# shanjiayao/PTT

Hardware: AMD Instinct MI355X
Metric: tracklet frames/sec (hot path: PointNet++ SA stack + Point-Track-Transformer blocks) (higher is better)
Workload: dtype f32

## Files before the change

include/ptt_hip.h:

```cpp
#ifndef PTT_HIP_H
#define PTT_HIP_H

#include <stddef.h>
#include <stdint.h>

#ifdef __cplusplus
extern "C" {
#endif

#define PTT_ABI_VERSION 31

enum {
    PTT_OK = 0,
    PTT_EINVAL = -1,
    PTT_EUNSUPPORTED = -2,
    PTT_ELAUNCH = -3,
    PTT_EWORKSPACE = -4
};

typedef void* ptt_stream_t;

int ptt_version(void);
const char* ptt_error_name(int code);
const char* ptt_last_error_string(void);

int ptt_fps_f32(const float* xyz, int B, int N, int npoint, int32_t* idx_out,
                ptt_stream_t stream);
int ptt_fps_ws_f32(const float* xyz, int B, int N, int npoint, int32_t* idx_out, float* workspace,
                   size_t workspace_elems, ptt_stream_t stream);

int ptt_ffps_f32(const float* xyz, const float* feat, int64_t feat_sb, int64_t feat_sc, int64_t feat_sn,
                 int B, int N, int C, int npoint, int32_t* idx_out, ptt_stream_t stream);

int ptt_gather_f32(const float* feat, const int32_t* idx, int B, int C, int N, int M,
                   float* out, ptt_stream_t stream);
int ptt_gather_grad_f32(const float* grad_out, const int32_t* idx, int B, int C, int N,
                        int M, float* grad_feat, ptt_stream_t stream);

int ptt_select_centres_f32(const float* xyz, const int32_t* idx, int B, int N, int M, float* new_xyz,
                           int64_t* idx64_out, ptt_stream_t stream);

int ptt_ball_query_f32(const float* new_xyz, const float* xyz, int B, int M, int N,
                       float radius, int nsample, int32_t* idx_out, ptt_stream_t stream);

int ptt_centres_ball_query_f32(const float* xyz, const int32_t* sel, int B, int N, int M, float radius, int nsample,
                               float* new_xyz, int64_t* idx64_out, int32_t* idx_out, ptt_stream_t stream);

int ptt_group_f32(const float* feat, const int32_t* idx, int B, int C, int N, int M,
                  int ns, float* out, ptt_stream_t stream);
int ptt_group_grad_f32(const float* grad_out, const int32_t* idx, int B, int C, int N,
                       int M, int ns, float* grad_feat, ptt_stream_t stream);

size_t ptt_scatter_add_det_workspace(int B, int N, int E);
int ptt_scatter_add_det_f32(const float* src, const int32_t* idx, int B, int C, int N, int E, float* out,
                            void* workspace, size_t workspace_bytes, ptt_stream_t stream);

int ptt_knn_f32(const float* xyz, int B, int N, int k, int32_t* idx_out,
                ptt_stream_t stream);
int ptt_knn_rel_f32(const float* xyz, int B, int N, int k, int32_t* idx_out, float* rel_out,
                    ptt_stream_t stream);

size_t ptt_packed_weight_elems(int Cout, int K);
int ptt_pack_weight_f32(const float* W, int Cout, int K, float* packed,
                        ptt_stream_t stream);
int ptt_pack_weight_rot_f32(const float* W, int Cout, int K, int rot, float* packed,
                            ptt_stream_t stream);

int ptt_linear_f32(const float* X, int rows, int K, int ldx, const float* Wpacked, int Cout,
                   const float* scale, const float* shift, int relu, const float* residual,
                   int ldr, float* out, int ldo, ptt_stream_t stream);

#define PTT_SA_MAX_LAYERS 4

typedef struct ptt_sa_layer {
    const float* Wpacked;
    const float* scale;
    const float* shift;
    int Cin;
    int Cout;
    int relu;
} ptt_sa_layer;

int ptt_rows_mlp_f32(const float* X, int rows, int K, int ldx, const ptt_sa_layer* layers, int n_layers,
                     const float* residual, int ldr, float* out, int ldo, ptt_stream_t stream);

size_t ptt_ball_query_grid_workspace(int B, int N);
int ptt_ball_query_grid_f32(const float* new_xyz, const float* xyz, int B, int M, int N, float radius, int nsample,
                            int32_t* idx_out, void* workspace, size_t workspace_bytes, ptt_stream_t stream);
int ptt_centres_ball_query_grid_f32(const float* xyz, const int32_t* sel, int B, int N, int M, float radius, int nsample,
                                    float* new_xyz, int64_t* idx64_out, int32_t* idx_out, void* workspace, size_t workspace_bytes,
                                    ptt_stream_t stream);
int ptt_fps_ball_knn_f32(const float* xyz, int B, int N, int M, float radius, int nsample, int k, int32_t* inds,
                         int64_t* inds64, float* new_xyz, int32_t* idx, int32_t* knn, float* rel, ptt_stream_t stream);
#define PTT_POINT_JOBS_MAX 4
typedef struct ptt_point_job {
    const float* xyz; const int32_t* centre_sel; const int32_t* point_sel;
    float* new_xyz; int64_t* idx64_out; int32_t* idx_out; float* rel_out;
    int32_t kind, sel_ld, B, Nraw, Npts, M, nsample;
    float radius;
} ptt_point_job;
int ptt_point_jobs_f32(const ptt_point_job* jobs, int n_jobs, ptt_stream_t stream);

#define PTT_ROW_JOBS_MAX 4
typedef struct ptt_row_job {
    const float* X; const float* X2;
    const float* Xmax;
    const float* Wpacked; const float* scale; const float* shift;
    const float* res; const float* res2;
    float* out; float* out2; float* raw;
    const float* rel; const float* w1;
    const float* qkv; const int32_t* knn; const float* pos;
    int32_t rows, K, K1, ldx, ldx2, Cout;
    int32_t act, res_split, ldr, ldr2, out_split, out_col0, ldo, ldo2, ldraw;
    int32_t prologue, epilogue, ldq, q_off, k_off, v_off, ldp, N;
    float sm_scale;
    int32_t col_tiles;
    const int32_t* idx; const float* xyz; const float* centres; const float* wx;
    float radius;
    int32_t ns, M, normalize_xyz, pro_relu;
} ptt_row_job;
int ptt_row_jobs_f32(const ptt_row_job* jobs, int n_jobs, ptt_stream_t stream);

typedef struct ptt_sa_desc {
    const float* xyz;
    const float* new_xyz;
    const int32_t* idx;
    const float* feat;
    int64_t feat_sb, feat_sc, feat_sn;
    float* out;
    int64_t out_sb, out_sc, out_sm;
    int B, N, M, nsample, C;
    float radius;
    int use_xyz;
    int normalize_xyz;
    int n_layers;
    ptt_sa_layer layers[PTT_SA_MAX_LAYERS];
    const float* l0_point_term;
    const float* l0_xyz_weight;
    int l0_channels;
    int l0_relu;
    void* compact_ws;
    size_t compact_ws_bytes;
} ptt_sa_desc;

int ptt_sa_fused_fwd_f32(const ptt_sa_desc* d, ptt_stream_t stream);
size_t ptt_sa_compact_workspace(int B, int M);

typedef struct ptt_xcorr_desc {
    const float* cos_t;
    const float* P;
    const float* w_sim;
    const float* scale0;
    const float* shift0;
    float* out;
    int64_t out_sb, out_sc, out_sn;
    float* sim_out;
    int B, Ns, Nt, C0;
    int n_layers;
    ptt_sa_layer layers[PTT_SA_MAX_LAYERS];
    int32_t split; int64_t out_sh;
    const float* search_feat; const float* templ_feat;
    int64_t s_sb, s_sn, t_sb, t_sn;
    int C; float eps;
} ptt_xcorr_desc;

int ptt_xcorr_fused_fwd_f32(const ptt_xcorr_desc* d, ptt_stream_t stream);

int ptt_cosine_map_f32(const float* search_feat, int64_t s_sb, int64_t s_sn, int64_t s_sc, const float* templ_feat,
                       int64_t t_sb, int64_t t_sn, int64_t t_sc, int B, int Ns, int Nt, int C, float eps,
                       float* cos_t, ptt_stream_t stream);

typedef struct ptt_attn_desc {
    const float* xyz;
    const float* rel;
    const int32_t* knn;
    const float* qkv;
    const float* Wd1p;
    const float* Wd2p;
    const float* bd2;
    const float* Wg1p;
    const float* bg1;
    const float* Wg2p;
    const float* bg2;
    float* res;
    float* attn;
    int B, N, k, D;
    const int32_t* order;
    int heads;
} ptt_attn_desc;

int ptt_pt_attn_pair_f32(const ptt_attn_desc* d, ptt_stream_t stream);
int ptt_spatial_order_f32(const float* xyz, int B, int N, int32_t* order, ptt_stream_t stream);

typedef struct ptt_crop_job {
    const float* points;
    int64_t ld;
    double lo1[3], hi1[3];
    double trans[3];
    double rot[9];
    double lo2[3], hi2[3];
    float* out;
    int32_t* count;
    int32_t n_points;
    int32_t capacity;
    uint8_t* label_out;
    double ltrans[3];
    double lrot[9];
    double llo[3], lhi[3];
    int32_t append;
    int32_t reserved;
} ptt_crop_job;

int ptt_crop_compact_f32(const ptt_crop_job* jobs_device, int n_jobs, ptt_stream_t stream);
#define PTT_CROP_JOBS_BY_VALUE_MAX 8
int ptt_crop_compact_host_f32(const ptt_crop_job* jobs_host, int n_jobs, ptt_stream_t stream);

#define PTT_SCAN_CROP_CHUNK 1024
size_t ptt_crop_scan_workspace(int n_jobs, int max_points);
int ptt_crop_scan_f32(const ptt_crop_job* jobs_device, int n_jobs, int max_points, void* ws, size_t ws_bytes, ptt_stream_t stream);

#define PTT_MAX_SEGMENTS 4
typedef struct ptt_regularize_job {
    const float* seg[PTT_MAX_SEGMENTS];
    const int32_t* seg_count[PTT_MAX_SEGMENTS];
    int32_t seg_capacity[PTT_MAX_SEGMENTS];
// ... 301 lines not shown
```

ptt_amd/_lib.py:

```python
import ctypes
import os
import re
from ctypes import Structure, c_char_p, c_double, c_float, c_int, c_int32, c_int64, c_longlong, c_size_t, c_uint32, c_void_p

from .build import HEADER as HEADER_PATH, LIB as LIB_PATH


def _strip_comments(text):
    return re.sub(r"/\*.*?\*/|//[^\n]*", " ", text, flags=re.S)


def parse_defines(text):
    return {n: int(v) for n, v in re.findall(r"^[ \t]*#[ \t]*define[ \t]+(PTT_\w+)[ \t]+(-?\d+)[ \t]*$", _strip_comments(text), re.M)}


CTYPES = {"int": c_int, "int32_t": c_int32, "uint32_t": c_uint32, "int64_t": c_int64, "long long": c_longlong, "size_t": c_size_t,
          "float": c_float, "double": c_double, "ptt_stream_t": c_void_p}


def _ctype(decl, name, is_return=False):
    words = decl.replace("*", " * ").split()
    if not is_return and len(words) > 1 and words[-1] != "*":
        words.pop()
    if "*" in words:
# ... 67 lines not shown
                ("reg", c_float * 4), ("index", c_uint32), ("epoch", c_uint32), ("capacity", c_int32), ("reserved", c_int32)]


class TrainBatchDesc(Structure):
    _fields_ = [("search_points", c_void_p), ("template_points", c_void_p), ("cls_label", c_void_p), ("reg_label", c_void_p),
                ("src_out", c_void_p), ("idx_search_out", c_void_p), ("idx_template_out", c_void_p), ("info", c_void_p), ("totals", c_void_p),
                ("B", c_int32), ("n_cand", c_int32), ("search_size", c_int32), ("template_size", c_int32), ("min_points", c_int32),
                ("seed_lo", c_uint32), ("seed_hi", c_uint32), ("reserved", c_int32)]


class BnTrainTail(Structure):
    _fields_ = [("gamma", c_void_p), ("beta", c_void_p), ("act_a", c_void_p), ("act_b", c_void_p),
                ("running_mean", c_void_p), ("running_var", c_void_p), ("num_batches_tracked", c_void_p), ("momentum", c_float)]


class BnBwdInput(Structure):
    _fields_ = [("g", c_void_p), ("ldg", c_int), ("arg", c_void_p), ("ns", c_int), ("z", c_void_p), ("ldz", c_int),
                ("k1", c_void_p), ("c0", c_void_p), ("c1", c_void_p), ("mean", c_void_p), ("act_a", c_void_p), ("act_b", c_void_p),
                ("dz_out", c_void_p), ("ldd", c_int)]


class PackJob(Structure):
    _fields_ = [("W", c_void_p), ("out_offset", c_int64), ("stride_out", c_int64), ("stride_k", c_int64),
                ("Cout", c_int32), ("K", c_int32)]


class RowJob(Structure):
    _fields_ = [("X", c_void_p), ("X2", c_void_p), ("Xmax", c_void_p), ("Wpacked", c_void_p), ("scale", c_void_p), ("shift", c_void_p),
                ("res", c_void_p), ("res2", c_void_p), ("out", c_void_p), ("out2", c_void_p), ("raw", c_void_p),
                ("rel", c_void_p), ("w1", c_void_p), ("qkv", c_void_p), ("knn", c_void_p), ("pos", c_void_p),
                ("rows", c_int32), ("K", c_int32), ("K1", c_int32), ("ldx", c_int32), ("ldx2", c_int32), ("Cout", c_int32),
                ("act", c_int32), ("res_split", c_int32), ("ldr", c_int32), ("ldr2", c_int32), ("out_split", c_int32),
                ("out_col0", c_int32), ("ldo", c_int32), ("ldo2", c_int32), ("ldraw", c_int32),
                ("prologue", c_int32), ("epilogue", c_int32), ("ldq", c_int32), ("q_off", c_int32), ("k_off", c_int32),
                ("v_off", c_int32), ("ldp", c_int32), ("N", c_int32), ("sm_scale", c_float), ("col_tiles", c_int32),
                ("idx", c_void_p), ("xyz", c_void_p), ("centres", c_void_p), ("wx", c_void_p), ("radius", c_float),
                ("ns", c_int32), ("M", c_int32), ("normalize_xyz", c_int32), ("pro_relu", c_int32)]


class PointJob(Structure):
    _fields_ = [("xyz", c_void_p), ("centre_sel", c_void_p), ("point_sel", c_void_p), ("new_xyz", c_void_p), ("idx64_out", c_void_p),
                ("idx_out", c_void_p), ("rel_out", c_void_p), ("kind", c_int32), ("sel_ld", c_int32), ("B", c_int32),
                ("Nraw", c_int32), ("Npts", c_int32), ("M", c_int32), ("nsample", c_int32), ("radius", c_float)]


class TrackLossDesc(Structure):
    _fields_ = [("seed_cls", c_void_p), ("cls_label", c_void_p), ("search_inds", c_void_p), ("votes", c_void_p), ("reg_label", c_void_p),
                ("box_data", c_void_p), ("centres", c_void_p), ("pos_weight_seed", c_void_p), ("pos_weight_box", c_void_p),
                ("B", c_int32), ("N", c_int32), ("Ns", c_int32), ("M", c_int32), ("ld_reg", c_int32),
                ("w_seed_cls", c_float), ("w_seed_reg", c_float), ("w_box_cls", c_float), ("w_box_reg", c_float)]


class AdamTensor(Structure):
    _fields_ = [("param", c_void_p), ("grad", c_void_p), ("exp_avg", c_void_p), ("exp_avg_sq", c_void_p), ("n", c_int64)]


class GradJob(Structure):
    _fields_ = [("partial", c_void_p), ("nchunks", c_int32), ("reserved", c_int32)]


class GradSegment(Structure):
    _fields_ = [("dst", c_int64), ("n", c_int32), ("cols", c_int32), ("ld", c_int32), ("job0", c_int32), ("njobs", c_int32), ("out", c_int32),
                ("vec", c_int32), ("reserved", c_int32)]


class AdamHyper(Structure):
    _fields_ = [("beta1", c_float), ("beta2", c_float), ("one_minus_beta1", c_float), ("one_minus_beta2", c_float), ("eps", c_float), ("step_size", c_float), ("bias2_sqrt", c_float),
                ("weight_decay", c_float), ("max_norm", c_float), ("write_clipped", c_int32)]


class SaLayer(Structure):
    _fields_ = [("Wpacked", c_void_p), ("scale", c_void_p), ("shift", c_void_p),
                ("Cin", c_int), ("Cout", c_int), ("relu", c_int)]


class SaDesc(Structure):
    _fields_ = [("xyz", c_void_p), ("new_xyz", c_void_p), ("idx", c_void_p), ("feat", c_void_p),
                ("feat_sb", c_int64), ("feat_sc", c_int64), ("feat_sn", c_int64),
                ("out", c_void_p), ("out_sb", c_int64), ("out_sc", c_int64), ("out_sm", c_int64),
                ("B", c_int), ("N", c_int), ("M", c_int), ("nsample", c_int), ("C", c_int),
                ("radius", c_float), ("use_xyz", c_int), ("normalize_xyz", c_int), ("n_layers", c_int),
                ("layers", SaLayer * PTT_SA_MAX_LAYERS),
                ("l0_point_term", c_void_p), ("l0_xyz_weight", c_void_p), ("l0_channels", c_int), ("l0_relu", c_int),
                ("compact_ws", c_void_p), ("compact_ws_bytes", c_size_t)]


class XcorrDesc(Structure):
    _fields_ = [("cos_t", c_void_p), ("P", c_void_p), ("w_sim", c_void_p), ("scale0", c_void_p), ("shift0", c_void_p),
                ("out", c_void_p), ("out_sb", c_int64), ("out_sc", c_int64), ("out_sn", c_int64),
                ("sim_out", c_void_p),
                ("B", c_int), ("Ns", c_int), ("Nt", c_int), ("C0", c_int),
                ("n_layers", c_int), ("layers", SaLayer * PTT_SA_MAX_LAYERS),
                ("split", c_int32), ("out_sh", c_int64), ("search_feat", c_void_p), ("templ_feat", c_void_p),
                ("s_sb", c_int64), ("s_sn", c_int64), ("t_sb", c_int64), ("t_sn", c_int64), ("C", c_int), ("eps", c_float)]


class AttnDesc(Structure):
    _fields_ = [("xyz", c_void_p), ("rel", c_void_p), ("knn", c_void_p), ("qkv", c_void_p),
                ("Wd1p", c_void_p), ("Wd2p", c_void_p), ("bd2", c_void_p),
                ("Wg1p", c_void_p), ("bg1", c_void_p), ("Wg2p", c_void_p), ("bg2", c_void_p),
                ("res", c_void_p), ("attn", c_void_p),
                ("B", c_int), ("N", c_int), ("k", c_int), ("D", c_int), ("order", c_void_p), ("heads", c_int)]


_lib = None


def lib():
    global _lib
    if _lib is None:
        if not os.path.exists(LIB_PATH):
            raise RuntimeError(
                "ptt_amd: %s is missing — build it with `python -m ptt_amd.build` "
                "(hipcc --offload-arch=gfx950); there is no CPU fallback" % LIB_PATH)
        import torch
        try:
            loaded = ctypes.CDLL(LIB_PATH)
        except OSError as e:
            raise RuntimeError("ptt_amd: cannot load %s: %s" % (LIB_PATH, e))
        for name, (restype, argtypes) in PROTOTYPES.items():
            fn = getattr(loaded, name)
            fn.restype, fn.argtypes = restype, argtypes
        if loaded.ptt_version() != ABI_VERSION:
            raise RuntimeError("ptt_amd: %s has ABI version %d, this package expects %d — rebuild it with "
                               "`python -m ptt_amd.build`" % (LIB_PATH, loaded.ptt_version(), ABI_VERSION))
        _lib = loaded
    return _lib


def check(rc, what):
    if rc != 0:
        l = lib()
        raise RuntimeError("%s failed: %s (%s)" % (what, l.ptt_error_name(rc).decode(),
                                                   l.ptt_last_error_string().decode()))
```

ptt_amd/csrc/common.h:

```cpp
#pragma once
#include <hip/hip_runtime.h>
#include <stdint.h>
#include <stdio.h>
#include "../../include/ptt_hip.h"

namespace ptt {

char* last_error_buf();
int fail(int code, const char* fmt, ...);
int check_launch(const char* what);

static inline hipStream_t as_stream(ptt_stream_t s) { return reinterpret_cast<hipStream_t>(s); }

struct DevSwitches {
    int linear_rt = 1, linear_ct = 1;
    int linear_small = 1;
    int sa_gather1 = 0;
    int sa_stagger = 0;
    int sa_wave = 1;
    int sa_rt = 2;
    int sa_lds = 1;
    int sa_stream = 1;
    int sa_chunk = 2;
    int pair_stagger = 0;
    int pair_lds_pad = 0;
    int sa_lds_chunk = 2;
    int fps_plain = 0;
    int ball_cpw = 0;
    int fps_t = 0;
    int ffps_stream = 0;
    int group_grad_global = 0;
    long long* stamps = nullptr;
};
const DevSwitches& dev_switches();

int set_lds_limit(const void* fn, int bytes);

bool wgrad_stream_ok(int R, int Cout, int Cin, int ldz, int ldx);
int wgrad_stream_rows(int R);
int launch_wgrad_stream(const float* dZ, int ldz, const float* X, int ldx, int R, int Cout, int Cin, int rows, float* partial,
                        const float* x_scale, const float* x_shift, hipStream_t s);

template <int CTRL, int ROW_MASK>
__device__ __forceinline__ int dpp_i32(int v) {
    return __builtin_amdgcn_update_dpp(v, v, CTRL, ROW_MASK, 0xF, false);
}
template <int CTRL, int ROW_MASK>
__device__ __forceinline__ float dpp_f32(float v) {
    return __builtin_bit_cast(float, dpp_i32<CTRL, ROW_MASK>(__builtin_bit_cast(int, v)));
}

__device__ __forceinline__ float wave_max_f32(float v) {
    v = fmaxf(v, dpp_f32<0xB1, 0xF>(v));
    v = fmaxf(v, dpp_f32<0x4E, 0xF>(v));
    v = fmaxf(v, dpp_f32<0x141, 0xF>(v));
    v = fmaxf(v, dpp_f32<0x140, 0xF>(v));
    v = fmaxf(v, dpp_f32<0x142, 0xA>(v));
    v = fmaxf(v, dpp_f32<0x143, 0xC>(v));
    return __builtin_bit_cast(float, __builtin_amdgcn_readlane(__builtin_bit_cast(int, v), 63));
}
__device__ __forceinline__ float wave_max_f32_fused(float v) {
    asm volatile(
        "s_nop 1\n\tv_max_f32_dpp %0, %0, %0 quad_perm:[1,0,3,2] row_mask:0xf bank_mask:0xf\n\t"
        "s_nop 1\n\tv_max_f32_dpp %0, %0, %0 quad_perm:[2,3,0,1] row_mask:0xf bank_mask:0xf\n\t"
        "s_nop 1\n\tv_max_f32_dpp %0, %0, %0 row_half_mirror row_mask:0xf bank_mask:0xf\n\t"
        "s_nop 1\n\tv_max_f32_dpp %0, %0, %0 row_mirror row_mask:0xf bank_mask:0xf\n\t"
        "s_nop 1\n\tv_max_f32_dpp %0, %0, %0 row_bcast:15 row_mask:0xa bank_mask:0xf\n\t"
        "s_nop 1\n\tv_max_f32_dpp %0, %0, %0 row_bcast:31 row_mask:0xc bank_mask:0xf\n\t"
        "s_nop 1"
        : "+v"(v));
    return __builtin_bit_cast(float, __builtin_amdgcn_readlane(__builtin_bit_cast(int, v), 63));
}

__device__ __forceinline__ float wave_min_f32(float v) {
    v = fminf(v, dpp_f32<0xB1, 0xF>(v));
    v = fminf(v, dpp_f32<0x4E, 0xF>(v));
    v = fminf(v, dpp_f32<0x141, 0xF>(v));
    v = fminf(v, dpp_f32<0x140, 0xF>(v));
    v = fminf(v, dpp_f32<0x142, 0xA>(v));
    v = fminf(v, dpp_f32<0x143, 0xC>(v));
    return __builtin_bit_cast(float, __builtin_amdgcn_readlane(__builtin_bit_cast(int, v), 63));
}
__device__ __forceinline__ int wave_min_i32(int v) {
    v = min(v, dpp_i32<0xB1, 0xF>(v));
    v = min(v, dpp_i32<0x4E, 0xF>(v));
    v = min(v, dpp_i32<0x141, 0xF>(v));
    v = min(v, dpp_i32<0x140, 0xF>(v));
    v = min(v, dpp_i32<0x142, 0xA>(v));
    v = min(v, dpp_i32<0x143, 0xC>(v));
    return __builtin_amdgcn_readlane(v, 63);
}

}
```

ptt_amd/csrc/errors.hip:

```cpp
#include <stdarg.h>
#include <stdlib.h>
#include <string.h>
#include <map>
#include <mutex>
#include <utility>
#include "common.h"

namespace ptt {

static thread_local char g_err[512] = "";

char* last_error_buf() { return g_err; }

int fail(int code, const char* fmt, ...) {
    va_list ap;
    va_start(ap, fmt);
    vsnprintf(g_err, sizeof(g_err), fmt, ap);
    va_end(ap);
    return code;
}

int check_launch(const char* what) {
    const hipError_t e = hipGetLastError();
    if (e == hipSuccess) return PTT_OK;
    return fail(PTT_ELAUNCH, "%s: %s", what, hipGetErrorString(e));
}

#ifdef PTT_DEV
static DevSwitches read_switches() {
    DevSwitches d;
    if (const char* e = getenv("PTT_LINEAR_TILE")) { d.linear_rt = (e[0] == '2') ? 2 : 1; d.linear_ct = (e[0] && e[1] == '2') ? 2 : 1; }
    if (getenv("PTT_SA_GATHER1")) d.sa_gather1 = 1;
    if (const char* e = getenv("PTT_SA_STAGGER")) d.sa_stagger = atoi(e);
    if (const char* e = getenv("PTT_SA_WAVE")) d.sa_wave = atoi(e) != 0;
    if (const char* e = getenv("PTT_SA_RT")) d.sa_rt = (atoi(e) == 1) ? 1 : 2;
    if (const char* e = getenv("PTT_SA_STREAM")) d.sa_stream = atoi(e) != 0;
    if (const char* e = getenv("PTT_SA_LDS")) d.sa_lds = atoi(e) != 0;
    if (const char* e = getenv("PTT_SA_CHUNK")) d.sa_chunk = atoi(e);
    if (const char* e = getenv("PTT_PAIR_STAGGER")) d.pair_stagger = atoi(e);
    if (const char* e = getenv("PTT_PAIR_LDS_PAD")) d.pair_lds_pad = atoi(e);
    if (const char* e = getenv("PTT_LINEAR_SMALL")) d.linear_small = atoi(e);
    if (const char* e = getenv("PTT_BALL_CPW")) d.ball_cpw = atoi(e);
    if (const char* e = getenv("PTT_FPS_PLAIN")) d.fps_plain = atoi(e);
    if (const char* e = getenv("PTT_SA_LDS_CHUNK")) d.sa_lds_chunk = atoi(e);
    if (const char* e = getenv("PTT_FPS_T")) d.fps_t = atoi(e);
    if (const char* e = getenv("PTT_FFPS_STREAM")) d.ffps_stream = atoi(e);
    if (getenv("PTT_GROUP_GRAD_GLOBAL")) d.group_grad_global = 1;
    if (const char* e = getenv("PTT_DEBUG_STAMPS")) d.stamps = reinterpret_cast<long long*>(strtoull(e, nullptr, 16));
    return d;
}
const DevSwitches& dev_switches() {
    static thread_local DevSwitches d;
    d = read_switches();
    return d;
}
#else
const DevSwitches& dev_switches() {
    static const DevSwitches d;
    return d;
}
#endif

int set_lds_limit(const void* fn, int bytes) {
    if (bytes <= 48 * 1024) return PTT_OK;
    static std::map<std::pair<const void*, int>, int> table;
    static std::mutex mu;
    int dev = 0;
    if (hipGetDevice(&dev) != hipSuccess) return check_launch("hipGetDevice");
    std::lock_guard<std::mutex> g(mu);
    const auto key = std::make_pair(fn, dev);
    const auto it = table.find(key);
    if (it != table.end() && it->second >= bytes) return PTT_OK;
    if (hipFuncSetAttribute(fn, hipFuncAttributeMaxDynamicSharedMemorySize, bytes) != hipSuccess)
        return check_launch("hipFuncSetAttribute(MaxDynamicSharedMemorySize)");
    table[key] = bytes;
    return PTT_OK;
}

}

extern "C" int ptt_version(void) { return PTT_ABI_VERSION; }

extern "C" const char* ptt_last_error_string(void) { return ptt::last_error_buf(); }

extern "C" const char* ptt_error_name(int code) {
    switch (code) {
        case PTT_OK: return "PTT_OK";
        case PTT_EINVAL: return "PTT_EINVAL";
        case PTT_EUNSUPPORTED: return "PTT_EUNSUPPORTED";
        case PTT_ELAUNCH: return "PTT_ELAUNCH";
        case PTT_EWORKSPACE: return "PTT_EWORKSPACE";
        default: return "PTT_E?";
    }
}
```

ptt_amd/csrc/mfma_ops.hip:

```cpp
#include <math.h>
#include <stdlib.h>
#include <string.h>
#include "common.h"
#include "mfma_common.h"

#ifndef PTT_PAIR_PF
#define PTT_PAIR_PF 1
#endif
#ifndef PTT_GATHER_BATCH
#define PTT_GATHER_BATCH 16
#endif
#ifndef PTT_SA_WAVES
#define PTT_SA_WAVES 2
#endif

namespace ptt {

#ifdef PTT_DEV
#define PTT_STAMP(i) do { if (p.dbg && threadIdx.x == 0 && blockIdx.x < 4096) p.dbg[blockIdx.x * 8 + (i)] = __builtin_readcyclecounter(); } while (0)
#else
#define PTT_STAMP(i) do { } while (0)
#endif

__device__ __forceinline__ void stagger_second_slot(int first_wave_blocks, int quanta) {
// ... 340 lines not shown
                if (gr >= p.rows) continue;
                float y = acc[rt][u][r] * sc + sh;
                if (p.relu) y = fmaxf(y, 0.f);
                if (p.residual) y += p.residual[(size_t)gr * p.ldr + col];
                p.out[(size_t)gr * p.ldo + col] = y;
            }
    }
}

constexpr int LS_PD = 8;
__global__ __launch_bounds__(512, 1) void linear_small_kernel(LinearParams p) {
    extern __shared__ __attribute__((aligned(16))) float smem[];
    const int t = threadIdx.x, lane = t & 63, half = lane >> 5;
    const int w = __builtin_amdgcn_readfirstlane(t >> 6), ks = w >> 2, cw = w & 3;
    const int row0 = blockIdx.x * 32;
    const int ct = blockIdx.y * 4 + cw;
    const bool has_ct = ct < p.NT;
    const int hb = ((p.nkb + 1) / 2 + LS_PD - 1) / LS_PD * LS_PD;
    const int ldk = 2 * hb * 8 + 4;
    float* Xs = smem;
    float* Rs = smem + 32 * ldk;
    {
        const int qpr = 2 * hb * 2;
        for (int e = t; e < 32 * qpr; e += 512) {
            const int r = e / qpr, c = (e - r * qpr) << 2;
            f32x4 v = {0.f, 0.f, 0.f, 0.f};
            if (row0 + r < p.rows && c < p.K) v = *reinterpret_cast<const f32x4*>(p.X + (size_t)(row0 + r) * p.ldx + c);
            *reinterpret_cast<f32x4*>(Xs + r * ldk + c) = v;
        }
    }
    const __amdgpu_buffer_rsrc_t wr = weight_rsrc(p.Wp);
    const int wvoff = ((has_ct ? ct : 0) * 64 + lane) * 16;
    const int wkstep = p.NT * 1024;
    const int kb0 = ks * hb, last = p.nkb - 1;
    f32x4 b[LS_PD];
#pragma unroll
    for (int i = 0; i < LS_PD; ++i) b[i] = weight_load(wr, wvoff, min(kb0 + i, last) * wkstep);
    f32x16 acc;
#pragma unroll
    for (int r = 0; r < 16; ++r) acc[r] = 0.f;
    __syncthreads();
    const float* arow = Xs + (lane & 31) * ldk + 4 * half + kb0 * 8;
    for (int k = 0; k < hb; k += LS_PD) {
#pragma unroll
        for (int i = 0; i < LS_PD; ++i) {
            const f32x4 a = *reinterpret_cast<const f32x4*>(arow + (k + i) * 8);
#pragma unroll
            for (int j = 0; j < 4; ++j) acc = __builtin_amdgcn_mfma_f32_32x32x2f32(a[j], b[i][j], acc, 0, 0, 0);
            b[i] = weight_load(wr, wvoff, min(kb0 + k + i + LS_PD, last) * wkstep);
        }
    }
    if (ks == 1) {
#pragma unroll
        for (int r = 0; r < 16; ++r) Rs[(cw * 16 + r) * 64 + lane] = acc[r];
    }
    __syncthreads();
    if (ks == 1 || !has_ct) return;
    const int col = ct * 32 + (lane & 31);
    if (col >= p.Cout) return;
    const float sc = p.scale ? p.scale[col] : 1.f;
    const float sh = p.shift ? p.shift[col] : 0.f;
#pragma unroll
    for (int r = 0; r < 16; ++r) {
        const int gr = row0 + tile_row(r, half);
        if (gr >= p.rows) continue;
        float y = (acc[r] + Rs[(cw * 16 + r) * 64 + lane]) * sc + sh;
        if (p.relu) y = fmaxf(y, 0.f);
        if (p.residual) y += p.residual[(size_t)gr * p.ldr + col];
        p.out[(size_t)gr * p.ldo + col] = y;
    }
}

struct SaLayerDev { const float* Wp; const float* scale; const float* shift; int Cin, Cout, relu, nkb, NT; };
struct SaParams {
    const float* xyz; const float* new_xyz; const int32_t* idx; const float* feat; float* out;
    long long fsb, fsc, fsn, osb, osc, osm;
    int B, N, M, C, use_xyz, normalize, n_layers, ldk, K0, first_wave, stagger, vec_gather;
    int tiles, chunk;
    int hoist, l0_relu;
    const float* wx;
    float radius;
    long long* dbg;
    int32_t* cws;
    SaLayerDev L[PTT_SA_MAX_LAYERS];
};

struct RowsMlpParams {
    const float* X; const float* residual; float* out;
    int rows, K0, ldx, ldr, ldo, n_layers, ldk, vec_in;
    SaLayerDev L[PTT_SA_MAX_LAYERS];
};

__global__ __launch_bounds__(256, 2) void rows_mlp_kernel(RowsMlpParams p) {
    extern __shared__ __attribute__((aligned(16))) float smem[];
    float* Xs = smem;
    const int t = threadIdx.x, lane = t & 63, w = t >> 6, half = lane >> 5;
    const int row0 = blockIdx.x * 32;
    f32x4 pw[3];
    float psh[3];
    auto prefetch = [&](const SaLayerDev& L) {
        const f32x4* bp = reinterpret_cast<const f32x4*>(L.Wp) + (size_t)w * 64 + lane;
#pragma unroll
        for (int u = 0; u < 3; ++u) {
            psh[u] = 0.f;
            if (w + 4 * u < L.NT) {
                pw[u] = bp[(size_t)u * 4 * 64];
                const int col = (w + 4 * u) * 32 + (lane & 31);
                if (L.shift && !L.scale && col < L.Cout) psh[u] = L.shift[col];
            }
        }
    };
    prefetch(p.L[0]);
    {
        const int Kpad = p.L[0].nkb * 8;
        if (p.vec_in) {
            const int nq = Kpad >> 2;
            for (int e = t; e < 32 * nq; e += 256) {
                const int r = e / nq, c4 = (e - r * nq) * 4;
                f32x4 v = {0.f, 0.f, 0.f, 0.f};
                if (row0 + r < p.rows && c4 < p.K0) v = *reinterpret_cast<const f32x4*>(p.X + (size_t)(row0 + r) * p.ldx + c4);
                *reinterpret_cast<f32x4*>(Xs + r * p.ldk + c4) = v;
            }
        } else {
            for (int e = t; e < 32 * Kpad; e += 256) {
                const int r = e / Kpad, c = e - r * Kpad;
                Xs[r * p.ldk + c] = (row0 + r < p.rows && c < p.K0) ? p.X[(size_t)(row0 + r) * p.ldx + c] : 0.f;
            }
        }
    }
    lds_barrier();
    for (int l = 0; l < p.n_layers; ++l) {
        const SaLayerDev& L = p.L[l];
        const bool last = l == p.n_layers - 1, affine = L.scale != nullptr;
        f32x16 acc[1][3];
#pragma unroll
        for (int u = 0; u < 3; ++u)
#pragma unroll
            for (int r = 0; r < 16; ++r) acc[0][u][r] = psh[u];
        int nvalid = 0;
#pragma unroll
        for (int u = 0; u < 3; ++u)
            if (w + 4 * u < L.NT) nvalid = u + 1;
        if (nvalid) gemm_tiles<1, 3, 0>(Xs, p.ldk, L.nkb, reinterpret_cast<const f32x4*>(L.Wp), L.NT, w, nvalid, lane, acc, pw);
        if (!last) { prefetch(p.L[l + 1]); lds_barrier(); }
#pragma unroll
        for (int u = 0; u < 3; ++u) {
            if (u >= nvalid) break;
            const int col = (w + 4 * u) * 32 + (lane & 31);
            float sc = 1.f, sh = 0.f;
            if (affine && col < L.Cout) { sc = L.scale[col]; sh = L.shift ? L.shift[col] : 0.f; }
#pragma unroll
            for (int r = 0; r < 16; ++r) {
                float y = affine ? acc[0][u][r] * sc + sh : acc[0][u][r];
                if (L.relu) y = fmaxf(y, 0.f);
                const int row = tile_row(r, half);
                if (!last) {
                    Xs[row * p.ldk + col] = (col < L.Cout) ? y : 0.f;
                } else if (col < L.Cout && row0 + row < p.rows) {
                    if (p.residual) y += p.residual[(size_t)(row0 + row) * p.ldr + col];
                    p.out[(size_t)(row0 + row) * p.ldo + col] = y;
                }
            }
        }
        if (!last) lds_barrier();
    }
}
// ... 172 lines not shown
                if (L.relu) m = fmaxf(m, 0.f);
                const int c = centre0 + rt;
                if (half == 0 && rt < ncentres) {
                    const int b = c / p.M, mm = c - b * p.M;
                    p.out[b * p.osb + col * p.osc + mm * p.osm] = m;
                }
            } else {
                float m0 = y[0], m1 = y[8];
#pragma unroll
                for (int r = 1; r < 8; ++r) { m0 = fmaxf(m0, y[r]); m1 = fmaxf(m1, y[8 + r]); }
                m0 = max_halves(m0);
                m1 = max_halves(m1);
                if (L.relu) { m0 = fmaxf(m0, 0.f); m1 = fmaxf(m1, 0.f); }
                if (half == 0) {
                    const int ca = rt * 2, cb = rt * 2 + 1;
                    if (ca < ncentres) {
                        const int c = centre0 + ca; const int b = c / p.M, mm = c - b * p.M;
                        p.out[b * p.osb + col * p.osc + mm * p.osm] = m0;
                    }
                    if (cb < ncentres) {
                        const int c = centre0 + cb; const int b = c / p.M, mm = c - b * p.M;
                        p.out[b * p.osb + col * p.osc + mm * p.osm] = m1;
                    }
                }
            }
        }
    }
    if (!last) lds_barrier();
}

template <int NS, int RT>
__global__ __launch_bounds__(256, PTT_SA_WAVES) void sa_fused_kernel(SaParams p) {
    extern __shared__ __attribute__((aligned(16))) float smem[];
    float* Xs = smem;
    constexpr int CPW = 32 * RT / NS;
    const int t = threadIdx.x, lane = t & 63, w = t >> 6;
    const int total_centres = p.B * p.M;
    const int centre0 = logical_block() * CPW;
    const int ncentres = min(CPW, total_centres - centre0);
    stagger_second_slot(p.first_wave, p.stagger);
    PTT_STAMP(0);

    SaPre pre;
    pre.w[0] = pre.w[1] = f32x4{0.f, 0.f, 0.f, 0.f};
    prefetch_first_block(p.L[0].Wp, p.L[0].scale, p.L[0].shift, p.L[0].NT, w, lane, pre);

    sa_gather_rows<NS, 8 * RT>(p, Xs, w * 8 * RT, centre0, lane);
    lds_barrier();

    PTT_STAMP(1);
    for (int l = 0; l < p.n_layers; ++l) {
        const SaLayerDev& L = p.L[l];
        const bool last = (l == p.n_layers - 1);
        const int ctw = (L.NT + 3) >> 2;
        const SaLayerDev* Ln = last ? nullptr : &p.L[l + 1];
        if (ctw <= 1) sa_layer<NS, 1, RT>(p, L, last, Xs, lane, w, centre0, ncentres, pre, Ln);
        else sa_layer<NS, 2, RT>(p, L, last, Xs, lane, w, centre0, ncentres, pre, Ln);
        PTT_STAMP(2 + l);
    }
}

constexpr int SAS_LDK = 132;
constexpr int SAS_TILE = 64 * SAS_LDK;

__device__ __forceinline__ f32x4 sas_pair_load(const float* meta, __amdgpu_buffer_rsrc_t rf, int w, int i, int sub, int q,
                                               f32x4& m) {
    m = *reinterpret_cast<const f32x4*>(meta + (w * 16 + 2 * i + sub) * 4);
    return weight_load(rf, __builtin_bit_cast(int, m[0]) + q * 16, 0);
}
__device__ __forceinline__ void sas_pair_store(float* X, int w, int i, int sub, int q, f32x4 v, const f32x4& m, const f32x4& wx0,
                                               const f32x4& wx1, const f32x4& wx2, float floor) {
#pragma unroll
    for (int j = 0; j < 4; ++j) {
        float y = __builtin_fmaf(wx0[j], m[1], v[j]);
        y = __builtin_fmaf(wx1[j], m[2], y);
        y = __builtin_fmaf(wx2[j], m[3], y);
        v[j] = fmaxf(y, floor);
    }
    *reinterpret_cast<f32x4*>(X + (16 * w + 2 * i + sub) * SAS_LDK + q * 4) = v;
}

struct SasCentre {
    int c, b, m;
    __device__ __forceinline__ void advance(int k, int M) {
        c += k; m += k;
        while (m >= M) { m -= M; ++b; }
    }
};

__device__ __forceinline__ float sas_pool(const f32x16& a, float sh, int relu) {
    float mx = a[0];
#pragma unroll
    for (int r = 1; r < 16; ++r) mx = fmaxf(mx, a[r]);
    mx = max_halves(mx) + sh;
    return relu ? fmaxf(mx, 0.f) : mx;
}

#ifndef PTT_SAS_INTERLEAVE
#define PTT_SAS_INTERLEAVE 0
#endif
#ifndef PTT_SAS_EXP
#define PTT_SAS_EXP 0
#endif
template <int NS>
__global__ __launch_bounds__(256, 2) void sa_stream_kernel(SaParams p) {
    static_assert(NS == 32, "one centre per 32-row tile");
    extern __shared__ __attribute__((aligned(16))) float smem[];
    float* const P = smem;
    float* const Q = smem + SAS_TILE;
    float* const meta = smem + 2 * SAS_TILE;
    const int t = threadIdx.x, lane = t & 63, half = lane >> 5, sub = half, q = lane & 31;
    const int w = __builtin_amdgcn_readfirstlane(t >> 6);
    const int tile0 = logical_block() * p.chunk;
    const int ntiles = min(p.chunk, p.tiles - tile0);
    if (ntiles <= 0) return;
    stagger_second_slot(p.first_wave, p.stagger);
    const SaLayerDev& L1 = p.L[0];
    const SaLayerDev& L2 = p.L[1];
    const __amdgpu_buffer_rsrc_t rf = weight_rsrc(p.feat);
    const __amdgpu_buffer_rsrc_t wr1 = weight_rsrc(L1.Wp), wr2 = weight_rsrc(L2.Wp);
    const int wvoff = (w * 64 + lane) * 16;
    constexpr int WK1 = 4 * 1024, WK2 = 8 * 1024;
    const f32x4 wx0 = *reinterpret_cast<const f32x4*>(p.wx + q * 4);
    const f32x4 wx1 = *reinterpret_cast<const f32x4*>(p.wx + 128 + q * 4);
    const f32x4 wx2 = *reinterpret_cast<const f32x4*>(p.wx + 256 + q * 4);
    const int col = lane & 31;
    const float sh1 = L1.shift ? L1.shift[w * 32 + col] : 0.f;
    const float sh2a = L2.shift ? L2.shift[w * 32 + col] : 0.f;
    const float sh2b = L2.shift ? L2.shift[(w + 4) * 32 + col] : 0.f;
    f32x16 sh1v;
#pragma unroll
    for (int r = 0; r < 16; ++r) sh1v[r] = sh1;
    const int total_centres = p.B * p.M;
    const float floor0 = p.l0_relu ? 0.f : -__builtin_inff();
    const float rdiv = p.normalize ? p.radius : 1.0f;
    const int M = p.M, N = p.N;
    const int osb = (int)p.osb, osm = (int)p.osm;
    const int ocol0 = (w * 32 + col) * (int)p.osc, ocol1 = ((w + 4) * 32 + col) * (int)p.osc;

    SasCentre own, first;
    {
        const int c0 = tile0 * 2;
        first.c = c0; first.b = c0 / M; first.m = c0 - first.b * M;
        own = first;
        own.advance(w >> 1, M);
    }
    auto meta_index = [&](const SasCentre& ce) -> int {
        const int c = ce.c < total_centres ? ce.c : total_centres - 1;
        return p.idx[(size_t)c * 32 + 16 * (w & 1) + (lane & 15)];
    };
    struct MetaXyz { float x, y, z, cx, cy, cz; int flat; };
    auto meta_fetch = [&](const SasCentre& ce, int n) -> MetaXyz {
        const bool in = ce.c < total_centres;
        const int c = in ? ce.c : total_centres - 1;
        const int b = in ? ce.b : p.B - 1;
        MetaXyz r;
        r.flat = b * N + n;
        r.x = p.xyz[(size_t)r.flat * 3 + 0]; r.y = p.xyz[(size_t)r.flat * 3 + 1]; r.z = p.xyz[(size_t)r.flat * 3 + 2];
        r.cx = p.new_xyz[(size_t)c * 3 + 0]; r.cy = p.new_xyz[(size_t)c * 3 + 1]; r.cz = p.new_xyz[(size_t)c * 3 + 2];
        return r;
    };
    auto meta_store = [&](const MetaXyz& r) {
        const float dx = (r.x - r.cx) / rdiv, dy = (r.y - r.cy) / rdiv, dz = (r.z - r.cz) / rdiv;
        const int off = r.flat * (128 * (int)sizeof(float));
        *reinterpret_cast<f32x4*>(meta + (w * 16 + (lane & 15)) * 4) = f32x4{__builtin_bit_cast(float, off), dx, dy, dz};
    };

    f32x4 pre1[2] = {weight_load(wr1, wvoff, 0), weight_load(wr1, wvoff, WK1)};
    {
        const int n = meta_index(own);
        meta_store(meta_fetch(own, n));
#pragma unroll
        for (int i = 0; i < 8; ++i) {
            f32x4 m;
            const f32x4 v = sas_pair_load(meta, rf, w, i, sub, q, m);
            sas_pair_store(P, w, i, sub, q, v, m, wx0, wx1, wx2, floor0);
        }
    }

    f32x16 acc[2][2];
#pragma unroll
    for (int rt = 0; rt < 2; ++rt)
#pragma unroll
        for (int u = 0; u < 2; ++u)
#pragma unroll
            for (int r = 0; r < 16; ++r) acc[rt][u][r] = 0.f;
    float pv[2][2] = {{0.f, 0.f}, {0.f, 0.f}};
    SasCentre prev = first;
    const f32x16 zero16 = {0.f, 0.f, 0.f, 0.f, 0.f, 0.f, 0.f, 0.f, 0.f, 0.f, 0.f, 0.f, 0.f, 0.f, 0.f, 0.f};

    auto store_pooled = [&](const SasCentre& f) {
        SasCentre c1 = f;
        c1.advance(1, M);
        if (half == 0) {
            if (f.c < total_centres) {
                float* o = p.out + (f.b * osb + f.m * osm);
                o[ocol0] = pv[0][0]; o[ocol1] = pv[0][1];
            }
            if (c1.c < total_centres) {
                float* o = p.out + (c1.b * osb + c1.m * osm);
                o[ocol0] = pv[1][0]; o[ocol1] = pv[1][1];
            }
        }
    };

    for (int it = 0; it < ntiles; ++it) {
        const bool more = it + 1 < ntiles;
        SasCentre own_next = own;
        if (more) own_next.advance(2, M);
        if (!(PTT_SAS_EXP & 1)) lds_barrier();
        const int nn = meta_index(own_next);
        MetaXyz mx;

        f32x16 acc1[2];
        {
            const float* arow = P + (lane & 31) * SAS_LDK + 4 * half;
            f32x4 a0[2], a1[2], bc[2], bn[2];
#define SAS_A1(A, KB)                                                                           \
            {                                                                                   \
                A[0] = *reinterpret_cast<const f32x4*>(arow + (KB) * 8);                        \
                A[1] = *reinterpret_cast<const f32x4*>(arow + 32 * SAS_LDK + (KB) * 8);         \
            }
            bc[0] = pre1[0]; bc[1] = pre1[1];
            SAS_A1(a0, 0)
#pragma unroll
            for (int i = 0; i < 8; ++i) {
                if (i < 7) { bn[0] = weight_load(wr1, wvoff, (2 * i + 2) * WK1); bn[1] = weight_load(wr1, wvoff, (2 * i + 3) * WK1); }
                SAS_A1(a1, 2 * i + 1)
                if (i == 4 && !(PTT_SAS_EXP & 16)) mx = meta_fetch(own_next, nn);
                __builtin_amdgcn_sched_barrier(0);
                if (i == 0) {
#pragma unroll
                    for (int rt = 0; rt < 2; ++rt) acc1[rt] = __builtin_amdgcn_mfma_f32_32x32x2f32(a0[rt][0], bc[0][0], sh1v, 0, 0, 0);
#pragma unroll
                    for (int j = 1; j < 4; ++j)
#pragma unroll
                        for (int rt = 0; rt < 2; ++rt)
                            acc1[rt] = __builtin_amdgcn_mfma_f32_32x32x2f32(a0[rt][j], bc[0][j], acc1[rt], 0, 0, 0);
                } else {
#pragma unroll
                    for (int j = 0; j < 4; ++j)
#pragma unroll
                        for (int rt = 0; rt < 2; ++rt)
                            acc1[rt] = __builtin_amdgcn_mfma_f32_32x32x2f32(a0[rt][j], bc[0][j], acc1[rt], 0, 0, 0);
                }
                __builtin_amdgcn_sched_barrier(0);
                if (i < 7) SAS_A1(a0, 2 * i + 2)
                __builtin_amdgcn_sched_barrier(0);
#pragma unroll
                for (int j = 0; j < 4; ++j)
#pragma unroll
                    for (int rt = 0; rt < 2; ++rt)
                        acc1[rt] = __builtin_amdgcn_mfma_f32_32x32x2f32(a1[rt][j], bc[1][j], acc1[rt], 0, 0, 0);
                __builtin_amdgcn_sched_barrier(0);
                if (i < 4 && !(PTT_SAS_EXP & 8)) pv[i >> 1][i & 1] = sas_pool(acc[i >> 1][i & 1], (i & 1) ? sh2b : sh2a, L2.relu);
                if (i == 6 && !(PTT_SAS_EXP & 16)) meta_store(mx);
                __builtin_amdgcn_sched_barrier(0);
                bc[0] = bn[0]; bc[1] = bn[1];
            }
#undef SAS_A1
        }
        f32x4 pre2[2][2];
#pragma unroll
        for (int k = 0; k < 2; ++k) {
            pre2[k][0] = weight_load(wr2, wvoff, k * WK2);
            pre2[k][1] = weight_load(wr2, wvoff, k * WK2 + 4 * 1024);
        }
#pragma unroll
        for (int rt = 0; rt < 2; ++rt)
#pragma unroll
            for (int r = (PTT_SAS_EXP & 4) ? 15 : 0; r < 16; ++r)
                Q[(rt * 32 + tile_row(r, half)) * SAS_LDK + w * 32 + col] = fmaxf(acc1[rt][r], 0.f);
        if (it > 0) store_pooled(prev);
        if (!(PTT_SAS_EXP & 1)) lds_barrier();

        {
            const float* arow = Q + (lane & 31) * SAS_LDK + 4 * half;
            f32x4 a0[2], a1[2], bc[2][2], bn[2][2];
#define SAS_A2(A, KB)                                                                           \
            {                                                                                   \
                A[0] = *reinterpret_cast<const f32x4*>(arow + (KB) * 8);                        \
                A[1] = *reinterpret_cast<const f32x4*>(arow + 32 * SAS_LDK + (KB) * 8);         \
            }
#pragma unroll
            for (int k = 0; k < 2; ++k) { bc[k][0] = pre2[k][0]; bc[k][1] = pre2[k][1]; }
            SAS_A2(a0, 0)
            f32x4 mc = *reinterpret_cast<const f32x4*>(meta + (w * 16 + sub) * 4), mn = mc;
#pragma unroll
            for (int i = 0; i < 8; ++i) {
                if (i < 7) {
#pragma unroll
                    for (int k = 0; k < 2; ++k) {
                        bn[k][0] = weight_load(wr2, wvoff, (2 * i + 2 + k) * WK2);
                        bn[k][1] = weight_load(wr2, wvoff, (2 * i + 2 + k) * WK2 + 4 * 1024);
                    }
                } else {
                    pre1[0] = weight_load(wr1, wvoff, 0);
                    pre1[1] = weight_load(wr1, wvoff, WK1);
                }
                SAS_A2(a1, 2 * i + 1)
                f32x4 v = wx0;
                if (!(PTT_SAS_EXP & 2)) v = weight_load(rf, __builtin_bit_cast(int, mc[0]) + q * 16, 0);
                __builtin_amdgcn_sched_barrier(0);
                if (i == 0) {
#pragma unroll
                    for (int u = 0; u < 2; ++u)
#pragma unroll
                        for (int rt = 0; rt < 2; ++rt)
                            acc[rt][u] = __builtin_amdgcn_mfma_f32_32x32x2f32(a0[rt][0], bc[0][u][0], zero16, 0, 0, 0);
#pragma unroll
                    for (int j = 1; j < 4; ++j)
#pragma unroll
                        for (int u = 0; u < 2; ++u)
#pragma unroll
                            for (int rt = 0; rt < 2; ++rt)
                                acc[rt][u] = __builtin_amdgcn_mfma_f32_32x32x2f32(a0[rt][j], bc[0][u][j], acc[rt][u], 0, 0, 0);
                } else {
                    gemm_mfma_block<2, 2, 2>(a0, bc[0], acc);
                }
                __builtin_amdgcn_sched_barrier(0);
                if (i < 7) {
                    SAS_A2(a0, 2 * i + 2)
                    mn = *reinterpret_cast<const f32x4*>(meta + (w * 16 + 2 * (i + 1) + sub) * 4);
                }
                __builtin_amdgcn_sched_barrier(0);
                gemm_mfma_block<2, 2, 2>(a1, bc[1], acc);
                if (!(PTT_SAS_EXP & 2)) sas_pair_store(P, w, i, sub, q, v, mc, wx0, wx1, wx2, floor0);
#if PTT_SAS_INTERLEAVE
#pragma unroll
                for (int k = 0; k < 16; ++k) {
                    __builtin_amdgcn_sched_group_barrier(0x008, 1, 0);
                    __builtin_amdgcn_sched_group_barrier(0x002, 1, 0);
                }
                __builtin_amdgcn_sched_group_barrier(0x200, 1, 0);
#endif
                __builtin_amdgcn_sched_barrier(0);
                mc = mn;
#pragma unroll
                for (int k = 0; k < 2; ++k) { bc[k][0] = bn[k][0]; bc[k][1] = bn[k][1]; }
            }
#undef SAS_A2
        }
        prev = first;
        if (more) { first.advance(2, M); own = own_next; }
    }
#pragma unroll
    for (int i = 0; i < 4; ++i) pv[i >> 1][i & 1] = sas_pool(acc[i >> 1][i & 1], (i & 1) ? sh2b : sh2a, L2.relu);
    store_pooled(prev);
}

struct XcorrParams {
    const float* P; const float* wsim; const float* scale0; const float* shift0;
    float* sim_out;
    const float* cos_t;
    int C0, Nt;
    SaParams sa;
    const float* sfeat; const float* tfeat; long long s_sb, s_sn, t_sb, t_sn; int C; float eps;
    long long out_sh;
};

struct CosParams {
    const float* sfeat; const float* tfeat; float* cos_t;
    long long s_sb, s_sn, s_sc, t_sb, t_sn, t_sc;
    int B, Ns, Nt, C;
    float eps;
};
__global__ __launch_bounds__(256) void cos_map_kernel(CosParams q) {
    const int lane = threadIdx.x & 63;
    const int j = blockIdx.x * 4 + (threadIdx.x >> 6);
    if (j >= q.B * q.Ns) return;
    const int b = j / q.Ns, jj = j - b * q.Ns;
    const float* s = q.sfeat + (long long)b * q.s_sb + (long long)jj * q.s_sn;
    for (int i0 = 0; i0 < q.Nt; i0 += 64) {
        const int i = i0 + lane;
        const float* a = q.tfeat + (long long)b * q.t_sb + (long long)(i < q.Nt ? i : q.Nt - 1) * q.t_sn;
        float dot = 0.f, na = 0.f, ns = 0.f;
        if (q.t_sc == 1 && q.s_sc == 1 && (q.C & 3) == 0 && ((q.t_sn | q.t_sb | q.s_sn | q.s_sb) & 3) == 0 &&
            ((reinterpret_cast<uintptr_t>(q.tfeat) | reinterpret_cast<uintptr_t>(q.sfeat)) & 15) == 0) {
            for (int c = 0; c < q.C; c += 4) {
                const f32x4 av = *reinterpret_cast<const f32x4*>(a + c), sv = *reinterpret_cast<const f32x4*>(s + c);
#pragma unroll
                for (int k = 0; k < 4; ++k) { dot += av[k] * sv[k]; na += av[k] * av[k]; ns += sv[k] * sv[k]; }
            }
        } else {
            for (int c = 0; c < q.C; ++c) {
                const float av = a[(long long)c * q.t_sc], sv = s[(long long)c * q.s_sc];
                dot += av * sv; na += av * av; ns += sv * sv;
            }
        }
        if (i < q.Nt) q.cos_t[((long long)b * q.Ns + jj) * q.Nt + i] = dot / (fmaxf(sqrtf(na), q.eps) * fmaxf(sqrtf(ns), q.eps));
    }
}

template <int RT, bool SPLIT>
__global__ __launch_bounds__(256, 2) void xcorr_fused_kernel(XcorrParams q) {
    constexpr int ROWS = 32 * RT;
    extern __shared__ __attribute__((aligned(16))) float smem[];
    const SaParams& p = q.sa;
    float* Xs = smem;
    float* simv = smem + ROWS * p.ldk;
    const int t = threadIdx.x, lane = t & 63, w = t >> 6, half = lane >> 5;
    const int npts = p.B * p.M;
    const int j = SPLIT ? (int)blockIdx.x % npts : logical_block();
    const int hsel = SPLIT ? (int)blockIdx.x / npts : 0;
    const int b = j / p.M, jj = j - b * p.M;
    stagger_second_slot(p.first_wave, p.stagger);
    SaPre pre;
    pre.w[0] = pre.w[1] = f32x4{0.f, 0.f, 0.f, 0.f};
    float run[2] = {-__builtin_inff(), -__builtin_inff()};
    const int nlast = p.n_layers - 1;
    const SaLayerDev& LL = p.L[nlast];

    const int ibeg = SPLIT ? hsel * (q.Nt >> 1) : 0, iend = SPLIT ? ibeg + (q.Nt >> 1) : q.Nt;
    for (int i0 = ibeg; i0 < iend; i0 += ROWS) {
        prefetch_first_block(p.L[0].Wp, p.L[0].scale, p.L[0].shift, p.L[0].NT, w, lane, pre);
        if (i0 != ibeg) __syncthreads();
        if constexpr (SPLIT) {
            const int i = t >> 3, sub = t & 7;
            const float* a = q.tfeat + (long long)b * q.t_sb + (long long)(i0 + i) * q.t_sn;
            const float* sv_ = q.sfeat + (long long)b * q.s_sb + (long long)jj * q.s_sn;
            float dot = 0.f, na = 0.f, ns = 0.f;
            for (int c = sub * 4; c < q.C; c += 32) {
                const f32x4 av = *reinterpret_cast<const f32x4*>(a + c), sv = *reinterpret_cast<const f32x4*>(sv_ + c);
#pragma unroll
                for (int k = 0; k < 4; ++k) { dot += av[k] * sv[k]; na += av[k] * av[k]; ns += sv[k] * sv[k]; }
            }
#pragma unroll
            for (int m = 1; m < 8; m <<= 1) { dot += __shfl_xor(dot, m, 64); na += __shfl_xor(na, m, 64); ns += __shfl_xor(ns, m, 64); }
            if (sub == 0) simv[i] = dot / (fmaxf(sqrtf(na), q.eps) * fmaxf(sqrtf(ns), q.eps));
        } else {
            if (t < ROWS) {
// ... 76 lines not shown
            p.out[(SPLIT ? hsel * q.out_sh : 0) + b * p.osb + col * p.osc + jj * p.osm] = LL.relu ? fmaxf(run[u], 0.f) : run[u];
        }
    }
}

template <int NS, int CT, bool AFFINE, int RT>
__device__ __forceinline__ void sa_wave_layer(const SaParams& p, const SaLayerDev& L, bool last, float* Xw, int lane,
                                              int centre0, int ncentres) {
    f32x16 acc[RT][CT];
#pragma unroll
    for (int u = 0; u < CT; ++u) {
        const float s0 = (!AFFINE && L.shift) ? L.shift[u * 32 + (lane & 31)] : 0.f;
#pragma unroll
        for (int rt = 0; rt < RT; ++rt)
#pragma unroll
            for (int r = 0; r < 16; ++r) acc[rt][u][r] = s0;
    }
    gemm_core<RT, CT, CT, 1>(Xw, p.ldk, L.nkb, reinterpret_cast<const f32x4*>(L.Wp), L.NT, 0, lane, acc);
    __builtin_amdgcn_wave_barrier();
    const int half = lane >> 5;
#pragma unroll
    for (int u = 0; u < CT; ++u) {
        const int col = u * 32 + (lane & 31);
        float sc = 1.f, sv = 0.f;
        if constexpr (AFFINE) { sc = L.scale[col]; sv = L.shift ? L.shift[col] : 0.f; }
#pragma unroll
        for (int rt = 0; rt < RT; ++rt) {
            float y[16];
#pragma unroll
            for (int r = 0; r < 16; ++r) y[r] = AFFINE ? acc[rt][u][r] * sc + sv : acc[rt][u][r];
            if (!last) {
#pragma unroll
                for (int r = 0; r < 16; ++r)
                    Xw[(rt * 32 + tile_row(r, half)) * p.ldk + col] = L.relu ? fmaxf(y[r], 0.f) : y[r];
            } else if (NS == 32) {
                float m = y[0];
#pragma unroll
                for (int r = 1; r < 16; ++r) m = fmaxf(m, y[r]);
                m = max_halves(m);
                if (L.relu) m = fmaxf(m, 0.f);
                if (half == 0 && rt < ncentres) {
                    const int c = centre0 + rt; const int b = c / p.M, mm = c - b * p.M;
                    p.out[b * p.osb + col * p.osc + mm * p.osm] = m;
                }
            } else {
                float m0 = y[0], m1 = y[8];
#pragma unroll
                for (int r = 1; r < 8; ++r) { m0 = fmaxf(m0, y[r]); m1 = fmaxf(m1, y[8 + r]); }
                m0 = max_halves(m0);
                m1 = max_halves(m1);
                if (L.relu) { m0 = fmaxf(m0, 0.f); m1 = fmaxf(m1, 0.f); }
                if (half == 0) {
                    if (2 * rt < ncentres) {
                        const int c = centre0 + 2 * rt; const int b = c / p.M, mm = c - b * p.M;
                        p.out[b * p.osb + col * p.osc + mm * p.osm] = m0;
                    }
                    if (2 * rt + 1 < ncentres) {
                        const int c = centre0 + 2 * rt + 1; const int b = c / p.M, mm = c - b * p.M;
                        p.out[b * p.osb + col * p.osc + mm * p.osm] = m1;
                    }
                }
            }
        }
    }
    __builtin_amdgcn_wave_barrier();
}

constexpr int SAC_HDR = 16;
struct SacTable {
    int32_t* ws; int T;
    __host__ __device__ int32_t* ndist() const { return ws + SAC_HDR; }
    __host__ __device__ int32_t* list(int k) const { return ws + SAC_HDR + (size_t)(1 + k) * T; }
    __host__ __device__ int32_t* rows(int k) const { return ws + SAC_HDR + 5 * (size_t)T + (size_t)((4 << k) - 4) * T; }
    static size_t words(size_t T) { return SAC_HDR + 65 * T; }
};
constexpr int SAC_PASSES = 4;

__global__ __launch_bounds__(64) void sa_compact_zero_kernel(int32_t* ws) {
    if (threadIdx.x < 4) ws[threadIdx.x] = 0;
}

template <bool XYZ>
__global__ __launch_bounds__(256) void sa_compact_kernel(const float* __restrict__ xyz, const int32_t* __restrict__ idx, int N, int M,
                                                         SacTable tab) {
    __shared__ int s_cnt[4], s_base[4], s_cls[32], s_pos[32], s_nd[32];
    __shared__ int s_row[32][32];
    const int t = threadIdx.x, lane = t & 63, half = lane >> 5, s = lane & 31, w = t >> 6;
    const int g0 = blockIdx.x * 32, T = tab.T;
    if (t < 4) s_cnt[t] = 0;
    __syncthreads();
    int iv[SAC_PASSES];
    uint32_t x[SAC_PASSES], y[SAC_PASSES], z[SAC_PASSES];
#pragma unroll
    for (int q = 0; q < SAC_PASSES; ++q) iv[q] = idx[(size_t)min(g0 + q * 8 + w * 2 + half, T - 1) * 32 + s];
    if constexpr (XYZ) {
#pragma unroll
        for (int q = 0; q < SAC_PASSES; ++q) {
            const int b = min(g0 + q * 8 + w * 2 + half, T - 1) / M;
            const uint32_t* pt = reinterpret_cast<const uint32_t*>(xyz) + ((size_t)b * N + iv[q]) * 3;
            x[q] = pt[0]; y[q] = pt[1]; z[q] = pt[2];
        }
    }
#pragma unroll
    for (int q = 0; q < SAC_PASSES; ++q) {
        const int lc = q * 8 + w * 2 + half;
        const int i0a = __builtin_amdgcn_readlane(iv[q], 0), i0b = __builtin_amdgcn_readlane(iv[q], 32);
        const int i0 = half ? i0b : i0a;
        const bool real = s == 0 || iv[q] != i0;
        int dup = 0;
        if constexpr (XYZ) {
            const unsigned long long rm = __ballot(real);
            const int J = 31 - __builtin_clz((uint32_t)rm | (uint32_t)(rm >> 32));
            for (int j = 0; j < J; ++j) {
                const uint32_t xa = __builtin_amdgcn_readlane(x[q], j), xb = __builtin_amdgcn_readlane(x[q], 32 + j);
                const uint32_t ya = __builtin_amdgcn_readlane(y[q], j), yb = __builtin_amdgcn_readlane(y[q], 32 + j);
                const uint32_t za = __builtin_amdgcn_readlane(z[q], j), zb = __builtin_amdgcn_readlane(z[q], 32 + j);
                dup |= (int)(j < s) & (int)(x[q] == (half ? xb : xa)) & (int)(y[q] == (half ? yb : ya)) & (int)(z[q] == (half ? zb : za));
            }
        }
        const bool keep = real && !dup;
        const unsigned long long km = __ballot(keep);
        const uint32_t m = half ? (uint32_t)(km >> 32) : (uint32_t)km;
        const int nd = __popc(m);
        if (keep) s_row[lc][__popc(m & ((1u << s) - 1u))] = iv[q];
        if (s == 0) {
            const int k = nd <= 4 ? 0 : nd <= 8 ? 1 : nd <= 16 ? 2 : 3;
            const bool valid = g0 + lc < T;
            s_cls[lc] = valid ? k : -1;
            s_nd[lc] = nd;
            s_pos[lc] = valid ? atomicAdd(&s_cnt[k], 1) : 0;
            if (valid) tab.ndist()[g0 + lc] = nd;
        }
    }
    __syncthreads();
    if (t < 4) s_base[t] = s_cnt[t] ? atomicAdd(&tab.ws[t], s_cnt[t]) : 0;
    __syncthreads();
    for (int e = t; e < 32 * 32; e += 256) {
        const int lc = e >> 5, j = e & 31, k = s_cls[lc];
        if (k < 0 || j >= (4 << k)) continue;
        const int q = s_base[k] + s_pos[lc];
        tab.rows(k)[(size_t)q * (4 << k) + j] = s_row[lc][j < s_nd[lc] ? j : 0];
        if (j == 0) tab.list(k)[q] = g0 + lc;
    }
}

#ifndef PTT_SAL_WGS
#define PTT_SAL_WGS 1
#endif
#ifndef PTT_SAL_WAVES
#define PTT_SAL_WAVES 12
#endif

template <int ROWS>
struct SacTileT {
    static constexpr int LG = ROWS == 32 ? 3 : 4;
    static_assert(ROWS == 32 || ROWS == 64, "32- or 64-row tiles");
    int k, first, n;
    __device__ __forceinline__ static void count(const int32_t* ws, int total, int (&cnt)[4], int (&tiles)[4]) {
#pragma unroll
        for (int k = 0; k < 4; ++k) {
            cnt[k] = min(max(ws[k], 0), total);
            tiles[k] = (k ? tiles[k - 1] : 0) + ((cnt[k] + ((1 << LG) >> k) - 1) >> (LG - k));
        }
    }
    __device__ __forceinline__ void at(int j, const int (&tiles)[4], const int (&cnt)[4]) {
        k = j < tiles[0] ? 0 : j < tiles[1] ? 1 : j < tiles[2] ? 2 : 3;
        const int j0 = k == 0 ? 0 : k == 1 ? tiles[0] : k == 2 ? tiles[1] : tiles[2];
        const int nk = k == 0 ? cnt[0] : k == 1 ? cnt[1] : k == 2 ? cnt[2] : cnt[3];
        first = (j - j0) << (LG - k);
        n = min((1 << LG) >> k, nk - first);
    }
    __device__ __forceinline__ void row(const SacTable& tab, int s, int& n_out, int& ball) const {
        const int cl = s >> (2 + k), inb = cl < n;
        n_out = tab.rows(k)[(size_t)first * (4 << k) + (inb ? s : (s & ((4 << k) - 1)))];
        ball = tab.list(k)[first + (inb ? cl : 0)];
    }
};
using SacTile = SacTileT<32>;

template <int NU>
__device__ __forceinline__ void sac_store(int k, int n, int ball, int M, const f32x16 (&acc)[NU], const float (&sh)[NU],
                                          float* const (&o)[NU], int relu, int half, int osb, int osm) {
    int ob[8];
#pragma unroll
    for (int g = 0; g < 8; ++g) {
        if (g >= (8 >> k)) break;
        const int id = __builtin_amdgcn_readlane(ball, g << (2 + k)), b = id / M;
        ob[g] = b * osb + (id - b * M) * osm;
    }
#pragma unroll
    for (int u = 0; u < NU; ++u) {
        const f32x16& a = acc[u];
        if (k == 3) {
            const float mx = sas_pool(a, sh[u], relu);
            if (half == 0) o[u][ob[0]] = mx;
        } else if (k == 2) {
            float m0 = a[0], m1 = a[8];
#pragma unroll
            for (int r = 1; r < 8; ++r) { m0 = fmaxf(m0, a[r]); m1 = fmaxf(m1, a[8 + r]); }
            m0 = max_halves(m0) + sh[u]; m1 = max_halves(m1) + sh[u];
            if (relu) { m0 = fmaxf(m0, 0.f); m1 = fmaxf(m1, 0.f); }
            if (half < n) o[u][half ? ob[1] : ob[0]] = half ? m1 : m0;
        } else {
            float m[4];
#pragma unroll
            for (int q = 0; q < 4; ++q) m[q] = fmaxf(fmaxf(a[4 * q], a[4 * q + 1]), fmaxf(a[4 * q + 2], a[4 * q + 3]));
            if (k == 1) {
#pragma unroll
                for (int q = 0; q < 4; ++q) m[q] = max_halves(m[q]) + sh[u];
#pragma unroll
                for (int i = 0; i < 2; ++i) {
                    const int g = 2 * half + i;
                    float v = half ? m[2 + i] : m[i];
                    if (relu) v = fmaxf(v, 0.f);
                    if (g < n) o[u][half ? ob[2 + i] : ob[i]] = v;
                }
            } else {
#pragma unroll
                for (int q = 0; q < 4; ++q) {
                    const int g = 2 * q + half;
                    float v = m[q] + sh[u];
                    if (relu) v = fmaxf(v, 0.f);
                    if (g < n) o[u][half ? ob[2 * q + 1] : ob[2 * q]] = v;
                }
            }
        }
    }
}

template <bool COMPACT>
__global__ __launch_bounds__(64 * PTT_SAL_WAVES) __attribute__((amdgpu_waves_per_eu(PTT_SAL_WAVES * PTT_SAL_WGS / 4)))
void sa_lds_kernel(SaParams p) {
    extern __shared__ __attribute__((aligned(16))) float smem[];
    float* W1 = smem;
    float* W2 = smem + 4096;
    const int t = threadIdx.x, lane = t & 63, half = lane >> 5, col = lane & 31;
    const int w = __builtin_amdgcn_readfirstlane(t >> 6);
    const int total = p.B * p.M, M = p.M, N = p.N;
    const int nw = (int)blockDim.x >> 6;
    SacTable tab{p.cws, total};
    int cnt[4], tiles[4];
    if constexpr (COMPACT) {
        SacTile::count(p.cws, total, cnt, tiles);
        if (logical_block() >= tiles[3]) return;
    }
    {
        const f32x4* g1 = reinterpret_cast<const f32x4*>(p.L[1].Wp);
        const f32x4* g2 = reinterpret_cast<const f32x4*>(p.L[2].Wp);
        f32x4* s1 = reinterpret_cast<f32x4*>(W1);
        f32x4* s2 = reinterpret_cast<f32x4*>(W2);
        const int nthr = (int)blockDim.x;
        for (int i = t; i < 1024; i += nthr) s1[i] = g1[i];
        for (int i = t; i < 2048; i += nthr) s2[i] = g2[i];
    }
    float* cst = smem + 4096 + 8192 + w * 640 + lane;
#pragma unroll
    for (int u = 0; u < 2; ++u) {
        const f32x4 f = reinterpret_cast<const f32x4*>(p.L[0].Wp)[u * 64 + col];
        const float s0 = p.L[0].shift ? p.L[0].shift[u * 32 + col] : 0.f;
        cst[(0 + u) * 64] = half ? f[1] : f[0];
        cst[(2 + u) * 64] = half ? s0 : f[2];
        cst[(4 + u) * 64] = p.L[1].shift ? p.L[1].shift[u * 32 + col] : 0.f;
    }
#pragma unroll
    for (int u = 0; u < 4; ++u) cst[(6 + u) * 64] = p.L[2].shift ? p.L[2].shift[u * 32 + col] : 0.f;
    const float one_zero = half ? 0.f : 1.f, one_hi = 1.f;
    __syncthreads();
    int c0, c1, cstep;
    if constexpr (COMPACT) {
        c0 = logical_block() + (int)gridDim.x * w; c1 = tiles[3]; cstep = (int)gridDim.x * nw;
    } else {
        const int gw = logical_block() * nw + w;
        c0 = gw * p.chunk; c1 = min(total, c0 + p.chunk); cstep = 1;
    }
    if (c0 >= c1) return;
    const float rdiv = p.normalize ? p.radius : 1.0f;
    const int osb = (int)p.osb, osm = (int)p.osm, osc = (int)p.osc;
    const f32x16 zero16 = {0.f, 0.f, 0.f, 0.f, 0.f, 0.f, 0.f, 0.f, 0.f, 0.f, 0.f, 0.f, 0.f, 0.f, 0.f, 0.f};
    const float* a1p = W1 + lane * 4;
    const float* b2p = W2 + lane * 4;
    const __amdgpu_buffer_rsrc_t rx = weight_rsrc(p.xyz);

    SasCentre ce{0, 0, 0};
    SacTile tc{0, 0, 0};
    float px, py, pz, cx, cy, cz;
    int g_cur = 0;
    if constexpr (COMPACT) {
        tc.at(c0, tiles, cnt);
        int n_cur;
        tc.row(tab, col, n_cur, g_cur);
        const size_t flat = (size_t)(g_cur / M) * N + n_cur;
        px = p.xyz[flat * 3]; py = p.xyz[flat * 3 + 1]; pz = p.xyz[flat * 3 + 2];
        cx = p.new_xyz[(size_t)g_cur * 3]; cy = p.new_xyz[(size_t)g_cur * 3 + 1]; cz = p.new_xyz[(size_t)g_cur * 3 + 2];
    } else {
        ce.c = c0; ce.b = c0 / M; ce.m = c0 - ce.b * M;
        const int n_cur = p.idx[(size_t)c0 * 32 + col];
        const size_t flat = (size_t)ce.b * N + n_cur;
        px = p.xyz[flat * 3]; py = p.xyz[flat * 3 + 1]; pz = p.xyz[flat * 3 + 2];
        cx = p.new_xyz[(size_t)c0 * 3]; cy = p.new_xyz[(size_t)c0 * 3 + 1]; cz = p.new_xyz[(size_t)c0 * 3 + 2];
    }
    for (int c = c0; c < c1; c += cstep) {
        SasCentre nx = ce;
        SacTile tx = tc;
        int n_next, g_next;
        if constexpr (COMPACT) {
            if (c + cstep < c1) tx.at(c + cstep, tiles, cnt);
            tx.row(tab, col, n_next, g_next);
        } else {
            if (c + 1 < c1) nx.advance(1, M);
            n_next = p.idx[(size_t)nx.c * 32 + col];
        }
        f32x4 wa[2], wn[2];
#pragma unroll
        for (int u = 0; u < 2; ++u) wa[u] = *reinterpret_cast<const f32x4*>(a1p + u * 256);
        const float dx = (px - cx) / rdiv, dy = (py - cy) / rdiv, dz = (pz - cz) / rdiv;
        __builtin_amdgcn_sched_barrier(0);
        f32x16 h0[2];
        {
            const float k0 = half ? dy : dx, k1 = half ? one_hi : dz;
#pragma unroll
            for (int u = 0; u < 2; ++u) h0[u] = __builtin_amdgcn_mfma_f32_32x32x2f32(cst[(0 + u) * 64], k0, zero16, 0, 0, 0);
#pragma unroll
            for (int u = 0; u < 2; ++u) h0[u] = __builtin_amdgcn_mfma_f32_32x32x2f32(cst[(2 + u) * 64], k1, h0[u], 0, 0, 0);
#pragma unroll
            for (int u = 0; u < 2; ++u)
#pragma unroll
                for (int r = 0; r < 16; ++r) h0[u][r] = fmaxf(h0[u][r], 0.f);
        }
        f32x16 h1[2];
        f32x4 wb[4], wm[4];
        {
#pragma unroll
            for (int u = 0; u < 2; ++u) h1[u] = __builtin_amdgcn_mfma_f32_32x32x2f32(cst[(4 + u) * 64], one_zero, zero16, 0, 0, 0);
#pragma unroll
            for (int kb = 0; kb < 8; ++kb) {
                if (kb < 7) {
#pragma unroll
                    for (int u = 0; u < 2; ++u) wn[u] = *reinterpret_cast<const f32x4*>(a1p + ((kb + 1) * 2 + u) * 256);
                } else {
#pragma unroll
                    for (int u = 0; u < 4; ++u) wb[u] = *reinterpret_cast<const f32x4*>(b2p + u * 256);
                }
                __builtin_amdgcn_sched_barrier(0);
#pragma unroll
                for (int j = 0; j < 4; ++j)
#pragma unroll
                    for (int u = 0; u < 2; ++u)
                        h1[u] = __builtin_amdgcn_mfma_f32_32x32x2f32(wa[u][j], h0[kb >> 2][(kb & 3) * 4 + j], h1[u], 0, 0, 0);
                __builtin_amdgcn_sched_barrier(0);
#pragma unroll
                for (int u = 0; u < 2; ++u) wa[u] = wn[u];
            }
#pragma unroll
            for (int u = 0; u < 2; ++u)
#pragma unroll
                for (int r = 0; r < 16; ++r) h1[u][r] = fmaxf(h1[u][r], 0.f);
        }
        {
            const int g = COMPACT ? g_next : nx.c;
            const int off = ((COMPACT ? g_next / M : nx.b) * N + n_next) * 12;
            px = __builtin_bit_cast(float, __builtin_amdgcn_raw_buffer_load_b32(rx, off, 0, 0));
            py = __builtin_bit_cast(float, __builtin_amdgcn_raw_buffer_load_b32(rx, off + 4, 0, 0));
            pz = __builtin_bit_cast(float, __builtin_amdgcn_raw_buffer_load_b32(rx, off + 8, 0, 0));
            cx = p.new_xyz[(size_t)g * 3]; cy = p.new_xyz[(size_t)g * 3 + 1]; cz = p.new_xyz[(size_t)g * 3 + 2];
        }
        __builtin_amdgcn_sched_barrier(0);
// ... 457 lines not shown
        if (L.nkb * 8 > maxk) maxk = L.nkb * 8;
        if (!last && L.NT * 32 > maxk) maxk = L.NT * 32;
        cin = s.Cout;
    }
    if (ldo < cin || (residual && ldr < cin)) return fail(PTT_EINVAL, "ptt_rows_mlp_f32: ldo=%d ldr=%d Cout=%d", ldo, ldr, cin);
    p.ldk = maxk + 4;
    p.vec_in = ((K & 3) == 0 && (ldx & 3) == 0 && (reinterpret_cast<uintptr_t>(X) & 15) == 0) ? 1 : 0;
    const int lds = 32 * p.ldk * (int)sizeof(float);
    int rc = set_lds_limit(reinterpret_cast<const void*>(rows_mlp_kernel), lds);
    if (rc) return rc;
    hipLaunchKernelGGL(rows_mlp_kernel, dim3((rows + 31) / 32), dim3(256), lds, as_stream(stream), p);
    return check_launch("rows_mlp_kernel");
}

extern "C" size_t ptt_sa_compact_workspace(int B, int M) {
    const long long T = (long long)(B > 0 ? B : 0) * (M > 0 ? M : 0);
    return SacTable::words((size_t)T) * sizeof(int32_t);
}

extern "C" int ptt_sa_fused_fwd_f32(const ptt_sa_desc* d, ptt_stream_t stream) {
    if (!d) return fail(PTT_EINVAL, "ptt_sa_fused_fwd_f32: null descriptor");
    if (d->B < 0 || d->N <= 0 || d->M < 0 || d->C < 0 || d->n_layers < 1 || d->n_layers > PTT_SA_MAX_LAYERS)
        return fail(PTT_EINVAL, "ptt_sa_fused_fwd_f32: B=%d N=%d M=%d C=%d layers=%d", d->B, d->N, d->M, d->C,
                    d->n_layers);
    if (d->nsample != 16 && d->nsample != 32 && d->nsample != 64)
        return fail(PTT_EUNSUPPORTED, "ptt_sa_fused_fwd_f32: nsample=%d (16, 32 and 64 are instantiated)", d->nsample);
    if (d->B == 0 || d->M == 0) return PTT_OK;
    const bool hoist = d->l0_point_term != nullptr;
    if (!d->xyz || !d->new_xyz || !d->idx || !d->out || (!hoist && d->C > 0 && !d->feat))
        return fail(PTT_EINVAL, "ptt_sa_fused_fwd_f32: null pointer");
    if (!d->use_xyz && d->C == 0) return fail(PTT_EINVAL, "ptt_sa_fused_fwd_f32: no xyz and no features");
    if (hoist) {
        const int c0 = d->l0_channels;
        if (!d->use_xyz || !d->l0_xyz_weight || c0 <= 0 || (c0 % 32) != 0 || c0 > 256 ||
            (reinterpret_cast<uintptr_t>(d->l0_point_term) & 15) != 0 ||
            (reinterpret_cast<uintptr_t>(d->l0_xyz_weight) & 15) != 0)
            return fail(PTT_EINVAL, "ptt_sa_fused_fwd_f32: hoisted layer 0 needs use_xyz, 16-byte aligned (B,N,C0) and "
                        "(3,C0) arrays and C0 a multiple of 32 <= 256 (C0=%d)", c0);
    }

    SaParams p;
    p.xyz = d->xyz; p.new_xyz = d->new_xyz; p.idx = d->idx; p.feat = d->feat; p.out = d->out;
    p.fsb = d->feat_sb; p.fsc = d->feat_sc; p.fsn = d->feat_sn;
    p.osb = d->out_sb; p.osc = d->out_sc; p.osm = d->out_sm;
    p.B = d->B; p.N = d->N; p.M = d->M; p.C = d->C; p.use_xyz = d->use_xyz ? 1 : 0;
    p.normalize = d->normalize_xyz ? 1 : 0; p.n_layers = d->n_layers; p.radius = d->radius;
    p.K0 = (d->use_xyz ? 3 : 0) + d->C;
    p.hoist = hoist ? 1 : 0; p.l0_relu = d->l0_relu ? 1 : 0; p.wx = d->l0_xyz_weight;
    if (hoist && d->l0_channels == 128 && (unsigned long long)d->B * d->N * 128ull * sizeof(float) < 0x7fffffffull &&
        !dev_switches().sa_gather1)
        p.hoist = 2;
    if (hoist) {
        p.feat = d->l0_point_term; p.C = d->l0_channels; p.K0 = p.C;
        p.fsc = 1; p.fsn = p.C; p.fsb = (long long)d->N * p.C;
    }
    int maxk = 0, cin = p.K0;
    for (int l = 0; l < d->n_layers; ++l) {
        const ptt_sa_layer& s = d->layers[l];
        if (s.Cin != cin) return fail(PTT_EINVAL, "ptt_sa_fused_fwd_f32: layer %d Cin=%d, expected %d", l, s.Cin, cin);
        if (s.Cout <= 0 || (s.Cout % 32) != 0 || s.Cout > 256)
            return fail(PTT_EUNSUPPORTED, "ptt_sa_fused_fwd_f32: layer %d Cout=%d must be a multiple of 32 <= 256", l,
                        s.Cout);
        if (!s.Wpacked) return fail(PTT_EINVAL, "ptt_sa_fused_fwd_f32: layer %d has no weights", l);
        SaLayerDev& L = p.L[l];
        L.Wp = s.Wpacked; L.scale = s.scale; L.shift = s.shift; L.Cin = s.Cin; L.Cout = s.Cout; L.relu = s.relu;
        L.nkb = (s.Cin + 7) / 8; L.NT = s.Cout / 32;
        if (L.nkb * 8 > maxk) maxk = L.nkb * 8;
        if (l + 1 < d->n_layers && s.Cout > maxk) maxk = s.Cout;
        cin = s.Cout;
    }
    {
        const unsigned long long lim = 0x7fffffffull, B = (unsigned long long)d->B;
        if (B * d->N * 12ull >= lim || B * d->M * d->nsample * 4ull >= lim || B * d->M * (unsigned long long)cin * 4ull >= lim ||
            B * d->N * (unsigned long long)(p.C > 0 ? p.C : 1) * 4ull >= lim)
            return fail(PTT_EUNSUPPORTED, "ptt_sa_fused_fwd_f32: B=%d N=%d M=%d: an array of this launch exceeds 2 GiB "
                        "(32-bit offsets) — split the batch", d->B, d->N, d->M);
    }
    p.ldk = maxk + 4;
    p.vec_gather = (p.C > 0 && p.fsc == 1 && (p.C & 3) == 0 && p.C <= 256 && (p.fsn & 3) == 0 &&
                    (p.fsb & 3) == 0 && (reinterpret_cast<uintptr_t>(p.feat) & 15) == 0) ? 1 : 0;
    p.first_wave = 1024; p.stagger = dev_switches().sa_stagger;
    p.dbg = dev_switches().stamps;
    p.cws = nullptr;
    const int total_centres = d->B * d->M;
    hipStream_t s = as_stream(stream);
    int rc;
    if (d->C == 0 && d->use_xyz && !hoist && d->nsample == 32 && d->n_layers == 3 && p.L[0].Cout == 64 && p.L[1].Cout == 64 &&
        p.L[2].Cout == 128 && !p.L[0].scale && !p.L[1].scale && !p.L[2].scale && p.L[0].relu && p.L[1].relu &&
        dev_switches().sa_lds) {
        const int waves = 256 * PTT_SAL_WAVES * PTT_SAL_WGS;
        p.chunk = (total_centres + waves - 1) / waves;
        if (dev_switches().sa_lds_chunk > 0 && p.chunk > dev_switches().sa_lds_chunk) p.chunk = dev_switches().sa_lds_chunk;
        const int nw = total_centres * 3 <= 256 * PTT_SAL_WAVES ? 4 : PTT_SAL_WAVES;
        int wgs = (total_centres + p.chunk * nw - 1) / (p.chunk * nw);
        const int lds = (4096 + 8192 + PTT_SAL_WAVES * 640) * (int)sizeof(float);
        if (d->compact_ws) {
            if (d->compact_ws_bytes < ptt_sa_compact_workspace(d->B, d->M) || (reinterpret_cast<uintptr_t>(d->compact_ws) & 15))
                return fail(PTT_EWORKSPACE, "ptt_sa_fused_fwd_f32: compact_ws needs %zu bytes, 16-byte aligned (got %zu)",
                            ptt_sa_compact_workspace(d->B, d->M), d->compact_ws_bytes);
            p.cws = static_cast<int32_t*>(d->compact_ws);
            hipLaunchKernelGGL(sa_compact_zero_kernel, dim3(1), dim3(64), 0, s, p.cws);
            if ((rc = check_launch("sa_compact_zero_kernel"))) return rc;
            hipLaunchKernelGGL(sa_compact_kernel<true>, dim3((total_centres + 31) / 32), dim3(256), 0, s, d->xyz, d->idx, d->N, d->M,
                               SacTable{p.cws, total_centres});
            if ((rc = check_launch("sa_compact_kernel"))) return rc;
            if (wgs > 256 * PTT_SAL_WGS) wgs = 256 * PTT_SAL_WGS;
            if ((rc = set_lds_limit(reinterpret_cast<const void*>(sa_lds_kernel<true>), lds))) return rc;
            hipLaunchKernelGGL(sa_lds_kernel<true>, dim3(wgs), dim3(64 * nw), lds, s, p);
            return check_launch("sa_lds_kernel");
        }
        if ((rc = set_lds_limit(reinterpret_cast<const void*>(sa_lds_kernel<false>), lds))) return rc;
        hipLaunchKernelGGL(sa_lds_kernel<false>, dim3(wgs), dim3(64 * nw), lds, s, p);
        return check_launch("sa_lds_kernel");
    }
    size_t wbytes = 0;
    bool wave_ok = true;
    for (int l = 0; l < d->n_layers; ++l) {
        wbytes += (size_t)d->layers[l].Cin * d->layers[l].Cout * sizeof(float);
        const int nt = d->layers[l].Cout / 32;
        if (!(nt == 1 || nt == 2 || nt == 4)) wave_ok = false;
    }
    wave_ok = wave_ok && dev_switches().sa_wave;
    if (wave_ok && wbytes <= 64 * 1024 && d->nsample <= 32) {
        const int lds = 4 * 32 * p.ldk * (int)sizeof(float);
        const int cpw = 32 / d->nsample, per_wg = 4 * cpw;
        const dim3 grid((total_centres + per_wg - 1) / per_wg);
        if (d->nsample == 32) {
            if ((rc = set_lds_limit(reinterpret_cast<const void*>(sa_wave_kernel<32, 1>), lds))) return rc;
            hipLaunchKernelGGL((sa_wave_kernel<32, 1>), grid, dim3(256), lds, s, p);
        } else {
            if ((rc = set_lds_limit(reinterpret_cast<const void*>(sa_wave_kernel<16, 1>), lds))) return rc;
            hipLaunchKernelGGL((sa_wave_kernel<16, 1>), grid, dim3(256), lds, s, p);
        }
        return check_launch("sa_wave_kernel");
    }
    if (p.hoist == 2 && d->nsample == 32 && d->n_layers == 2 && p.L[0].Cin == 128 && p.L[0].Cout == 128 &&
        p.L[1].Cout == 256 && !p.L[0].scale && !p.L[1].scale && p.L[0].relu && dev_switches().sa_stream) {
        p.tiles = (total_centres + 1) / 2;
        int wgs = p.tiles < 512 ? p.tiles : 512;
        p.chunk = (p.tiles + wgs - 1) / wgs;
        if (dev_switches().sa_chunk > 0 && p.chunk > dev_switches().sa_chunk) p.chunk = dev_switches().sa_chunk;
        wgs = (p.tiles + p.chunk - 1) / p.chunk;
        if (d->compact_ws) {
            if (d->compact_ws_bytes < ptt_sa_compact_workspace(d->B, d->M) || (reinterpret_cast<uintptr_t>(d->compact_ws) & 15))
                return fail(PTT_EWORKSPACE, "ptt_sa_fused_fwd_f32: compact_ws needs %zu bytes, 16-byte aligned (got %zu)",
                            ptt_sa_compact_workspace(d->B, d->M), d->compact_ws_bytes);
            p.cws = static_cast<int32_t*>(d->compact_ws);
            hipLaunchKernelGGL(sa_compact_zero_kernel, dim3(1), dim3(64), 0, s, p.cws);
            if ((rc = check_launch("sa_compact_zero_kernel"))) return rc;
            hipLaunchKernelGGL(sa_compact_kernel<false>, dim3((total_centres + 31) / 32), dim3(256), 0, s, d->xyz, d->idx, d->N, d->M,
                               SacTable{p.cws, total_centres});
            if ((rc = check_launch("sa_compact_kernel"))) return rc;
            const int lds = (2 * SAS_TILE + 64 * 4 + 64) * (int)sizeof(float);
            if ((rc = set_lds_limit(reinterpret_cast<const void*>(sa_stream_compact_kernel), lds))) return rc;
            hipLaunchKernelGGL(sa_stream_compact_kernel, dim3(p.tiles < 512 ? p.tiles : 512), dim3(256), lds, s, p);
            return check_launch("sa_stream_compact_kernel");
        }
        const int lds = (2 * SAS_TILE + 4 * 16 * 4) * (int)sizeof(float);
        if ((rc = set_lds_limit(reinterpret_cast<const void*>(sa_stream_kernel<32>), lds))) return rc;
        hipLaunchKernelGGL((sa_stream_kernel<32>), dim3(wgs), dim3(256), lds, s, p);
        return check_launch("sa_stream_kernel");
    }
    int RT = dev_switches().sa_rt;
    if (d->nsample == 64) RT = 2;
    const int lds = 32 * RT * p.ldk * (int)sizeof(float);
    if (lds > 160 * 1024) return fail(PTT_EUNSUPPORTED, "ptt_sa_fused_fwd_f32: %d B of LDS per workgroup", lds);
    const int cpw = 32 * RT / d->nsample;
    const dim3 grid((total_centres + cpw - 1) / cpw);
#define PTT_SA_CASE(NSV, RTV)                                                                                   \
    if (d->nsample == NSV && RT == RTV) {                                                                       \
        if ((rc = set_lds_limit(reinterpret_cast<const void*>(sa_fused_kernel<NSV, RTV>), lds))) return rc;     \
        hipLaunchKernelGGL((sa_fused_kernel<NSV, RTV>), grid, dim3(256), lds, s, p);                            \
    }
    PTT_SA_CASE(32, 2) PTT_SA_CASE(32, 1) PTT_SA_CASE(16, 2) PTT_SA_CASE(16, 1) PTT_SA_CASE(64, 2)
#undef PTT_SA_CASE
    return check_launch("sa_fused_kernel");
}

extern "C" int ptt_xcorr_fused_fwd_f32(const ptt_xcorr_desc* d, ptt_stream_t stream) {
    if (!d) return fail(PTT_EINVAL, "ptt_xcorr_fused_fwd_f32: null descriptor");
    if (d->B < 0 || d->Ns <= 0 || d->C0 <= 0 || d->n_layers < 1 || d->n_layers > PTT_SA_MAX_LAYERS)
        return fail(PTT_EINVAL, "ptt_xcorr_fused_fwd_f32: B=%d Ns=%d C0=%d layers=%d", d->B, d->Ns, d->C0, d->n_layers);
    if (d->Nt <= 0 || (d->Nt % 64) != 0)
        return fail(PTT_EUNSUPPORTED, "ptt_xcorr_fused_fwd_f32: Nt=%d (the template seeds are walked in chunks of 64)", d->Nt);
    if (d->n_layers < 2) return fail(PTT_EUNSUPPORTED, "ptt_xcorr_fused_fwd_f32: needs at least two MFMA layers after layer 0");
    if ((d->C0 % 8) != 0 || d->C0 > 256) return fail(PTT_EUNSUPPORTED, "ptt_xcorr_fused_fwd_f32: C0=%d", d->C0);
    if (d->B == 0) return PTT_OK;
    if (!d->P || !d->w_sim || !d->out) return fail(PTT_EINVAL, "ptt_xcorr_fused_fwd_f32: null pointer");
    if ((unsigned long long)d->B * d->Ns * d->Nt >= 0x7fffffffull || (unsigned long long)d->B * d->Nt * d->C0 >= 0x7fffffffull)
        return fail(PTT_EUNSUPPORTED, "ptt_xcorr_fused_fwd_f32: B=%d Ns=%d Nt=%d: 32-bit element offsets — split the batch",
                    d->B, d->Ns, d->Nt);
    XcorrParams q;
    q.P = d->P; q.wsim = d->w_sim; q.scale0 = d->scale0;
    q.shift0 = d->shift0; q.sim_out = d->sim_out; q.cos_t = d->cos_t;
    q.C0 = d->C0; q.Nt = d->Nt;
    q.sfeat = q.tfeat = nullptr; q.s_sb = q.s_sn = q.t_sb = q.t_sn = 0; q.C = 0; q.eps = 0.f; q.out_sh = 0;
    SaParams& p = q.sa;
    memset(&p, 0, sizeof(p));
    p.out = d->out; p.osb = d->out_sb; p.osc = d->out_sc; p.osm = d->out_sn;
    p.B = d->B; p.M = d->Ns; p.n_layers = d->n_layers;
    int maxk = d->C0, cin = d->C0;
    for (int l = 0; l < d->n_layers; ++l) {
        const ptt_sa_layer& s = d->layers[l];
        if (s.Cin != cin) return fail(PTT_EINVAL, "ptt_xcorr_fused_fwd_f32: layer %d Cin=%d, expected %d", l, s.Cin, cin);
        if (s.Cout <= 0 || (s.Cout % 32) != 0 || s.Cout > 256)
            return fail(PTT_EUNSUPPORTED, "ptt_xcorr_fused_fwd_f32: layer %d Cout=%d", l, s.Cout);
        if (!s.Wpacked) return fail(PTT_EINVAL, "ptt_xcorr_fused_fwd_f32: layer %d has no weights", l);
        SaLayerDev& L = p.L[l];
        L.Wp = s.Wpacked; L.scale = s.scale; L.shift = s.shift; L.Cin = s.Cin; L.Cout = s.Cout; L.relu = s.relu;
        L.nkb = (s.Cin + 7) / 8; L.NT = s.Cout / 32;
        if (l + 1 < d->n_layers && s.Cout > maxk) maxk = s.Cout;
        cin = s.Cout;
    }
    p.ldk = ((maxk + 7) / 8) * 8 + 4;
    p.first_wave = 1024; p.stagger = 2;
    if (d->split) {
        if (!d->search_feat || !d->templ_feat || d->sim_out || (d->C & 3) || (d->s_sb & 3) || (d->s_sn & 3) ||
            (d->t_sb & 3) || (d->t_sn & 3) || ((reinterpret_cast<uintptr_t>(d->search_feat) | reinterpret_cast<uintptr_t>(d->templ_feat)) & 15) ||
            ((d->B * d->Ns) & 7) || d->C <= 0)
            return fail(PTT_EINVAL, "ptt_xcorr_fused_fwd_f32: the split form needs the features (unit channel stride, C %% 4 == 0, 16-byte "
                                    "aligned rows), B * Ns %% 8 == 0 and no sim_out");
        q.sfeat = d->search_feat; q.tfeat = d->templ_feat; q.s_sb = d->s_sb; q.s_sn = d->s_sn; q.t_sb = d->t_sb; q.t_sn = d->t_sn;
        q.C = d->C; q.eps = d->eps; q.out_sh = d->out_sh;
        const int lds = (32 * p.ldk + 32) * (int)sizeof(float);
        int rc = set_lds_limit(reinterpret_cast<const void*>(xcorr_fused_kernel<1, true>), lds);
        if (rc) return rc;
        hipLaunchKernelGGL((xcorr_fused_kernel<1, true>), dim3(2 * d->B * d->Ns), dim3(256), lds, as_stream(stream), q);
        return check_launch("xcorr_fused_kernel");
    }
    if (!d->cos_t) return fail(PTT_EINVAL, "ptt_xcorr_fused_fwd_f32: null pointer (cos_t comes from ptt_cosine_map_f32)");
    const int lds = (64 * p.ldk + 64) * (int)sizeof(float);
    int rc = set_lds_limit(reinterpret_cast<const void*>(xcorr_fused_kernel<2, false>), lds);
    if (rc) return rc;
    hipLaunchKernelGGL((xcorr_fused_kernel<2, false>), dim3(d->B * d->Ns), dim3(256), lds, as_stream(stream), q);
    return check_launch("xcorr_fused_kernel");
}

extern "C" int ptt_cosine_map_f32(const float* search_feat, int64_t s_sb, int64_t s_sn, int64_t s_sc, const float* templ_feat,
                                  int64_t t_sb, int64_t t_sn, int64_t t_sc, int B, int Ns, int Nt, int C, float eps,
                                  float* cos_t, ptt_stream_t stream) {
    if (B < 0 || Ns <= 0 || Nt <= 0 || C <= 0) return fail(PTT_EINVAL, "ptt_cosine_map_f32: B=%d Ns=%d Nt=%d C=%d", B, Ns, Nt, C);
    if (B == 0) return PTT_OK;
    if (!search_feat || !templ_feat || !cos_t) return fail(PTT_EINVAL, "ptt_cosine_map_f32: null pointer");
    CosParams q;
// ... 63 lines not shown
```

ptt_amd/csrc/point_ops.hip:

```cpp
#pragma clang fp contract(off)

#include <limits.h>
#include <stdlib.h>
#include "common.h"

namespace ptt {

__device__ __forceinline__ float sqdist3(float ax, float ay, float az, float bx, float by, float bz) {
    const float dx = ax - bx, dy = ay - by, dz = az - bz;
    return (dx * dx + dy * dy) + dz * dz;
}

__device__ __forceinline__ float knn_dist(float ax, float ay, float az, float bx, float by, float bz) {
    const float d = sqdist3(ax, ay, az, bx, by, bz);
    return d < __builtin_inff() ? d : 3.402823466e+38f;
}

__device__ __forceinline__ float lane_bcast(float v, int src_lane) {
    return __builtin_bit_cast(float, __builtin_amdgcn_readlane(__builtin_bit_cast(int, v), src_lane));
}

typedef float fps_f2 __attribute__((ext_vector_type(2)));


template <int T, int P, bool LX, int ABL = 0>
__global__ __launch_bounds__(T) void fps_kernel(const float* __restrict__ xyz, int N, int npoint,
                                               int32_t* __restrict__ idx_out) {
    constexpr int W = T / 64;
    const int b = blockIdx.x;
    const float* __restrict__ pts = xyz + (size_t)b * N * 3;
    int32_t* __restrict__ out = idx_out + (size_t)b * npoint;
    const int t = threadIdx.x;
    const int lane = t & 63;
    const int wv = t >> 6;

    extern __shared__ int sel_lds[];
    float* xyz_lds = reinterpret_cast<float*>(sel_lds + ((npoint + 3) & ~3));

    float px[P], py[P], pz[P], md[P];
#pragma unroll
    for (int i = 0; i < P; ++i) {
        const int k = t * P + i;
        float x = 0.f, y = 0.f, z = 0.f, m = -1.0f;
        if (k < N) {
            x = pts[3 * k + 0];
            y = pts[3 * k + 1];
            z = pts[3 * k + 2];
            const float mag = (x * x + y * y) + z * z;
            m = (mag > 1e-3f) ? 1e10f : -1.0f;
            if (LX) { xyz_lds[3 * k + 0] = x; xyz_lds[3 * k + 1] = y; xyz_lds[3 * k + 2] = z; }
        }
        px[i] = x; py[i] = y; pz[i] = z; md[i] = m;
    }

    __shared__ __attribute__((aligned(16))) float slots[2][W > 1 ? W : 1][8];

    float lx = pts[0], ly = pts[1], lz = pts[2];
    if (t == 0 && npoint > 0) sel_lds[0] = 0;
    if (LX) __syncthreads();

    for (int j = 1; j < npoint; ++j) {
        float best = -1.0f, bx = 0.f, by = 0.f, bz = 0.f;
        int besti = 0;
        if constexpr ((P % 2) == 0) {
            const fps_f2 lxv = {lx, lx}, lyv = {ly, ly}, lzv = {lz, lz};
#pragma unroll
            for (int i = 0; i < ((ABL & 32) ? 2 : P); i += 2) {
                const fps_f2 dx = fps_f2{px[i], px[i + 1]} - lxv, dy = fps_f2{py[i], py[i + 1]} - lyv,
                             dz = fps_f2{pz[i], pz[i + 1]} - lzv;
                const fps_f2 d = (dx * dx + dy * dy) + dz * dz;
#pragma unroll
                for (int h = 0; h < 2; ++h) {
                    const float m = fminf(md[i + h], d[h]);
                    md[i + h] = m;
                    const bool take = m > best;
                    best = take ? m : best;
                    besti = take ? t * P + i + h : besti;
                    if (!LX) {
                        bx = take ? px[i + h] : bx;
                        by = take ? py[i + h] : by;
                        bz = take ? pz[i + h] : bz;
                    }
                }
            }
        } else {
#pragma unroll
            for (int i = 0; i < P; ++i) {
                const float d = sqdist3(px[i], py[i], pz[i], lx, ly, lz);
                const float m = fminf(md[i], d);
                md[i] = m;
                const bool take = m > best;
                best = take ? m : best;
                besti = take ? t * P + i : besti;
                if (!LX) {
                    bx = take ? px[i] : bx;
                    by = take ? py[i] : by;
                    bz = take ? pz[i] : bz;
                }
            }
        }
        float wmax;
        if constexpr (ABL & 1) wmax = __builtin_amdgcn_readfirstlane(best); else wmax = wave_max_f32_fused(best);
        int src;
        if constexpr (ABL & 2) {
            src = (int)(__builtin_bit_cast(unsigned, wmax) & 63u);
        } else {
            const unsigned long long winners = __ballot(best == wmax);
            src = __ffsll((long long)winners) - 1;
            if constexpr (ABL & 1) src &= 63;
        }
        if constexpr (W == 1) {
            int widx = __builtin_amdgcn_readlane(besti, src);
            if (wmax < 0.f) widx = 0;
            if constexpr ((ABL & 8) != 0) {
                lx = (float)widx * 1e-3f; ly = lx; lz = lx;
            } else if constexpr (LX) {
                lx = xyz_lds[3 * widx + 0]; ly = xyz_lds[3 * widx + 1]; lz = xyz_lds[3 * widx + 2];
            } else if (wmax < 0.f) {
                lx = pts[0]; ly = pts[1]; lz = pts[2];
            } else {
                lx = lane_bcast(bx, src); ly = lane_bcast(by, src); lz = lane_bcast(bz, src);
            }
            if (lane == 0) sel_lds[j] = widx;
        } else if constexpr ((ABL & 4) != 0) {
            int gi = __builtin_amdgcn_readlane(besti, src);
            if (wmax < 0.f) gi = 0;
            if constexpr ((ABL & 8) != 0) { lx = (float)gi * 1e-3f; ly = lx; lz = lx; }
            else { lx = xyz_lds[3 * gi + 0]; ly = xyz_lds[3 * gi + 1]; lz = xyz_lds[3 * gi + 2]; }
            if (lane == 0 && wv == 0) sel_lds[j] = gi;
        } else {
            const int par = j & 1;
            if (lane == src) {
                if constexpr (LX) {
                    *reinterpret_cast<float2*>(slots[par][wv]) = make_float2(best, __builtin_bit_cast(float, besti));
                } else {
                    float4* s4 = reinterpret_cast<float4*>(slots[par][wv]);
                    s4[0] = make_float4(best, __builtin_bit_cast(float, besti), bx, by);
                    slots[par][wv][4] = bz;
                }
            }
            if constexpr ((ABL & 16) == 0) __syncthreads();
            float gd, gx = 0.f, gy = 0.f, gz = 0.f;
            int gi;
            if constexpr (W <= 4) {
                gd = -1.0f; gi = 0;
#pragma unroll
                for (int w = 0; w < W; ++w) {
                    if constexpr (LX) {
                        const float2 s2 = *reinterpret_cast<const float2*>(slots[par][w]);
                        const bool take = s2.x > gd;
                        gd = take ? s2.x : gd;
                        gi = take ? __builtin_bit_cast(int, s2.y) : gi;
                    } else {
                        const float4 s4 = *reinterpret_cast<const float4*>(slots[par][w]);
                        const float sz = slots[par][w][4];
                        const bool take = s4.x > gd;
                        gd = take ? s4.x : gd;
                        gi = take ? __builtin_bit_cast(int, s4.y) : gi;
                        gx = take ? s4.z : gx;
                        gy = take ? s4.w : gy;
                        gz = take ? sz : gz;
                    }
                }
            } else {
                if constexpr (LX) {
                    float2 s2 = make_float2(-1.0f, 0.f);
                    if (lane < W) s2 = *reinterpret_cast<const float2*>(slots[par][lane]);
                    gd = wave_max_f32_fused(s2.x);
                    const int sl = __ffsll((long long)__ballot(s2.x == gd)) - 1;
                    gi = __builtin_amdgcn_readlane(__builtin_bit_cast(int, s2.y), sl);
                } else {
                    float4 s4 = make_float4(-1.0f, 0.f, 0.f, 0.f);
                    float sz = 0.f;
                    if (lane < W) { s4 = *reinterpret_cast<const float4*>(slots[par][lane]); sz = slots[par][lane][4]; }
                    gd = wave_max_f32_fused(s4.x);
                    const int sl = __ffsll((long long)__ballot(s4.x == gd)) - 1;
                    gi = __builtin_amdgcn_readlane(__builtin_bit_cast(int, s4.y), sl);
                    gx = lane_bcast(s4.z, sl); gy = lane_bcast(s4.w, sl); gz = lane_bcast(sz, sl);
                }
            }
            if (gd < 0.f) gi = 0;
            if constexpr ((ABL & 16) != 0) gi &= 1023;
            if constexpr ((ABL & 8) != 0) {
                lx = (float)gi * 1e-3f; ly = lx; lz = lx;
            } else if constexpr (LX) {
                lx = xyz_lds[3 * gi + 0]; ly = xyz_lds[3 * gi + 1]; lz = xyz_lds[3 * gi + 2];
            } else {
                if (gd < 0.f) { gx = pts[0]; gy = pts[1]; gz = pts[2]; }
                lx = gx; ly = gy; lz = gz;
            }
            if (t == 0) sel_lds[j] = gi;
        }
    }
    __syncthreads();
    for (int j = t; j < npoint; j += T) out[j] = sel_lds[j];
}

template <int T, int P>
static int launch_fps(const float* xyz, int B, int N, int npoint, int32_t* idx, hipStream_t s) {
    const size_t sel_bytes = (size_t)((npoint + 3) & ~3) * sizeof(int);
    if (sel_bytes + (size_t)N * 12 + 1024 <= 65536 && !dev_switches().fps_plain) {
#ifdef PTT_DEV
        if (const char* e = getenv("PTT_FPS_ABL")) {
            const int abl = atoi(e);
#define PTT_FPS_ABL_CASE(A) if (abl == A) { hipLaunchKernelGGL((fps_kernel<T, P, true, A>), dim3(B), dim3(T), sel_bytes + (size_t)N * 12, s, xyz, N, npoint, idx); return check_launch("fps_kernel(abl)"); }
            PTT_FPS_ABL_CASE(1) PTT_FPS_ABL_CASE(2) PTT_FPS_ABL_CASE(3) PTT_FPS_ABL_CASE(4) PTT_FPS_ABL_CASE(8) PTT_FPS_ABL_CASE(12) PTT_FPS_ABL_CASE(15)
            PTT_FPS_ABL_CASE(16) PTT_FPS_ABL_CASE(32) PTT_FPS_ABL_CASE(47) PTT_FPS_ABL_CASE(7) PTT_FPS_ABL_CASE(24) PTT_FPS_ABL_CASE(40)
#undef PTT_FPS_ABL_CASE
        }
#endif
        hipLaunchKernelGGL((fps_kernel<T, P, true>), dim3(B), dim3(T), sel_bytes + (size_t)N * 12, s, xyz, N, npoint, idx);
        return check_launch("fps_kernel");
    }
    hipLaunchKernelGGL((fps_kernel<T, P, false>), dim3(B), dim3(T), sel_bytes, s, xyz, N, npoint, idx);
    return check_launch("fps_kernel");
}

template <int CPW>
__device__ __forceinline__ void ball_sweep(const float* __restrict__ pts, int N, float r2, int ns, const float (&cx)[CPW],
                                           const float (&cy)[CPW], const float (&cz)[CPW], int ncentres,
                                           int32_t* __restrict__ out0, int lane) {
    int cnt[CPW], first[CPW];
#pragma unroll
    for (int c = 0; c < CPW; ++c) { cnt[c] = (c < ncentres) ? 0 : ns; first[c] = 0; }
    for (int base = 0; base < N; base += 64) {
        const int k = base + lane;
        const bool in = k < N;
        float px = 0.f, py = 0.f, pz = 0.f;
        if (in) { px = pts[3 * k + 0]; py = pts[3 * k + 1]; pz = pts[3 * k + 2]; }
        bool active = false;
#pragma unroll
        for (int c = 0; c < CPW; ++c) {
            if (cnt[c] >= ns) continue;
            const float d = sqdist3(cx[c], cy[c], cz[c], px, py, pz);
            const bool hit = in && d < r2;
            const unsigned long long mask = __ballot(hit);
            if (mask != 0ull) {
                if (cnt[c] == 0) first[c] = base + (__ffsll((long long)mask) - 1);
                const int pos = cnt[c] + __popcll(mask & ((1ull << lane) - 1ull));
                if (hit && pos < ns) out0[(size_t)c * ns + pos] = k;
                cnt[c] += __popcll(mask);
            }
            active = active || cnt[c] < ns;
        }
        if (!active) break;
    }
#pragma unroll
    for (int c = 0; c < CPW; ++c) {
        if (c >= ncentres) break;
        const int fill = (cnt[c] > 0) ? first[c] : 0;
        for (int s = cnt[c] + lane; s < ns; s += 64) out0[(size_t)c * ns + s] = fill;
    }
}

template <int CPW>
__global__ __launch_bounds__(256) void ball_query_kernel(const float* __restrict__ new_xyz,
                                                         const float* __restrict__ xyz, int BM, int M, int N,
                                                         float r2, int ns, int32_t* __restrict__ idx_out) {
    const int centre = (blockIdx.x * 4 + (threadIdx.x >> 6)) * CPW;
    if (centre >= BM) return;
    const int lane = threadIdx.x & 63;
    const int b = centre / M;
    float cx[CPW], cy[CPW], cz[CPW];
    const int nc = min(CPW, BM - centre);
#pragma unroll
    for (int c = 0; c < CPW; ++c) {
        const int cc = centre + (c < nc ? c : 0);
        cx[c] = new_xyz[(size_t)cc * 3 + 0]; cy[c] = new_xyz[(size_t)cc * 3 + 1]; cz[c] = new_xyz[(size_t)cc * 3 + 2];
    }
    ball_sweep<CPW>(xyz + (size_t)b * N * 3, N, r2, ns, cx, cy, cz, nc, idx_out + (size_t)centre * ns, lane);
}

template <int CPW>
__global__ __launch_bounds__(256) void centres_ball_query_kernel(const float* __restrict__ xyz, const int32_t* __restrict__ sel,
                                                                 int BM, int M, int N, float r2, int ns,
                                                                 float* __restrict__ new_xyz, long long* __restrict__ idx64,
                                                                 int32_t* __restrict__ idx_out) {
    const int centre = (blockIdx.x * 4 + (threadIdx.x >> 6)) * CPW;
    if (centre >= BM) return;
    const int lane = threadIdx.x & 63;
    const int b = centre / M;
    const float* __restrict__ pts = xyz + (size_t)b * N * 3;
    float cx[CPW], cy[CPW], cz[CPW];
    const int nc = min(CPW, BM - centre);
#pragma unroll
    for (int c = 0; c < CPW; ++c) {
        const int cc = centre + (c < nc ? c : 0);
        const int n = sel ? sel[cc] : cc - b * M;
        cx[c] = pts[3 * n + 0]; cy[c] = pts[3 * n + 1]; cz[c] = pts[3 * n + 2];
        if (lane == 0 && c < nc) {
            new_xyz[(size_t)cc * 3 + 0] = cx[c]; new_xyz[(size_t)cc * 3 + 1] = cy[c]; new_xyz[(size_t)cc * 3 + 2] = cz[c];
            if (idx64) idx64[cc] = n;
        }
    }
    ball_sweep<CPW>(pts, N, r2, ns, cx, cy, cz, nc, idx_out + (size_t)centre * ns, lane);
}

// ... 774 lines not shown
__global__ __launch_bounds__(256) void ball_query_grid_kernel(const float* __restrict__ xyz, const float* __restrict__ centres,
                                                              const int32_t* __restrict__ sel, int sel_mode, int BM, int M, int N,
                                                              float r2, int ns, const int32_t* __restrict__ ws,
                                                              float* __restrict__ new_xyz_out, long long* __restrict__ idx64,
                                                              int32_t* __restrict__ idx_out) {
    extern __shared__ unsigned bq_bits[];
    const int lane = threadIdx.x & 63, wv = threadIdx.x >> 6;
    const int centre = blockIdx.x * 4 + wv;
    if (centre >= BM) return;
    const int words = (N + 31) >> 5;
    unsigned* __restrict__ bits = bq_bits + (size_t)wv * words;
    const int b = centre / M;
    const float* __restrict__ pts = xyz + (size_t)b * N * 3;
    const int32_t* __restrict__ slice = ws + (size_t)b * grid_slice_ints(N);
    const GridHead g = *reinterpret_cast<const GridHead*>(slice);
    const int32_t* __restrict__ cstart = slice + 8;
    const int32_t* __restrict__ cpts = slice + 8 + GRID_MAX_CELLS + 1;
    float cx, cy, cz;
    if (sel_mode) {
        const int n = sel ? sel[centre] : centre - b * M;
        cx = pts[3 * n]; cy = pts[3 * n + 1]; cz = pts[3 * n + 2];
        if (lane == 0) {
            new_xyz_out[(size_t)centre * 3] = cx; new_xyz_out[(size_t)centre * 3 + 1] = cy; new_xyz_out[(size_t)centre * 3 + 2] = cz;
            if (idx64) idx64[centre] = n;
        }
    } else {
        cx = centres[(size_t)centre * 3]; cy = centres[(size_t)centre * 3 + 1]; cz = centres[(size_t)centre * 3 + 2];
    }
    for (int w = lane; w < words; w += 64) bits[w] = 0u;
    __builtin_amdgcn_wave_barrier();
    const int ix = grid_cell_coord(cx, g.ox, g.inv, g.nx), iy = grid_cell_coord(cy, g.oy, g.inv, g.ny), iz = grid_cell_coord(cz, g.oz, g.inv, g.nz);
    for (int dz = -1; dz <= 1; ++dz) {
        const int z = iz + dz;
        if (z < 0 || z >= g.nz) continue;
        for (int dy = -1; dy <= 1; ++dy) {
            const int y = iy + dy;
            if (y < 0 || y >= g.ny) continue;
            const int x0 = ix > 0 ? ix - 1 : 0, x1 = ix + 1 < g.nx ? ix + 1 : g.nx - 1;
            const int c0 = (z * g.ny + y) * g.nx + x0;
            const int s0 = cstart[c0], s1 = cstart[c0 + (x1 - x0) + 1];
            for (int e = s0 + lane; e < s1; e += 64) {
                const int k = cpts[e];
                const float d = sqdist3(cx, cy, cz, pts[3 * k], pts[3 * k + 1], pts[3 * k + 2]);
                if (d < r2) atomicOr(&bits[k >> 5], 1u << (k & 31));
            }
        }
    }
    __builtin_amdgcn_wave_barrier();
    asm volatile("s_waitcnt lgkmcnt(0)" ::: "memory");
    int32_t* __restrict__ out = idx_out + (size_t)centre * ns;
    int cnt = 0, first = 0;
    for (int w0 = 0; w0 < words && cnt < ns; w0 += 64) {
        const int w = w0 + lane;
        unsigned v = w < words ? bits[w] : 0u;
        const int mine = __popc(v);
        int incl = mine;
#pragma unroll
        for (int off = 1; off < 64; off <<= 1) { const int u = __shfl_up(incl, off, 64); if (lane >= off) incl += u; }
        const int total = __shfl(incl, 63, 64);
        if (total == 0) continue;
        if (cnt == 0) {
            const unsigned long long any = __ballot(mine > 0);
            const int fl = __ffsll((long long)any) - 1;
            const unsigned fv = __shfl(v, fl, 64);
            first = ((w0 + fl) << 5) + (__ffs(fv) - 1);
        }
        int pos = cnt + incl - mine;
        while (v != 0u && pos < ns) {
            const int bit = __ffs(v) - 1;
            out[pos++] = (w << 5) + bit;
            v &= v - 1u;
        }
        cnt += total;
    }
    const int have = cnt < ns ? cnt : ns;
    const int fill = cnt > 0 ? first : 0;
    for (int s2 = have + lane; s2 < ns; s2 += 64) out[s2] = fill;
}

}

using namespace ptt;

extern "C" int ptt_fps_f32(const float* xyz, int B, int N, int npoint, int32_t* idx_out, ptt_stream_t stream) {
    if (B < 0 || N <= 0 || npoint < 0) return fail(PTT_EINVAL, "ptt_fps_f32: B=%d N=%d npoint=%d", B, N, npoint);
    if (B == 0 || npoint == 0) return PTT_OK;
    if (!xyz || !idx_out) return fail(PTT_EINVAL, "ptt_fps_f32: null pointer");
    if (npoint > 15360) return fail(PTT_EUNSUPPORTED, "ptt_fps_f32: npoint=%d exceeds the LDS index buffer (15360)", npoint);
    hipStream_t s = as_stream(stream);
    if (N <= 64) return launch_fps<64, 1>(xyz, B, N, npoint, idx_out, s);
    if (N <= 128) return launch_fps<64, 2>(xyz, B, N, npoint, idx_out, s);
    if (N <= 256) return launch_fps<64, 4>(xyz, B, N, npoint, idx_out, s);
    if (N <= 512) {
        if (const int T = dev_switches().fps_t) {
            if (T == 256) return launch_fps<256, 2>(xyz, B, N, npoint, idx_out, s);
            if (T == 128) return launch_fps<128, 4>(xyz, B, N, npoint, idx_out, s);
            if (T == 512) return launch_fps<512, 1>(xyz, B, N, npoint, idx_out, s);
        }
        return launch_fps<64, 8>(xyz, B, N, npoint, idx_out, s);
    }
    if (N <= 1024) {
        if (const int T = dev_switches().fps_t) {
            if (T == 64) return launch_fps<64, 16>(xyz, B, N, npoint, idx_out, s);
            if (T == 128) return launch_fps<128, 8>(xyz, B, N, npoint, idx_out, s);
            if (T == 512) return launch_fps<512, 2>(xyz, B, N, npoint, idx_out, s);
        }
        return launch_fps<256, 4>(xyz, B, N, npoint, idx_out, s);
    }
    if (N <= 2048) {
        if (const int T = dev_switches().fps_t) {
            if (T == 512) return launch_fps<512, 4>(xyz, B, N, npoint, idx_out, s);
            if (T == 1024) return launch_fps<1024, 2>(xyz, B, N, npoint, idx_out, s);
            if (T == 128) return launch_fps<128, 16>(xyz, B, N, npoint, idx_out, s);
        }
        return launch_fps<256, 8>(xyz, B, N, npoint, idx_out, s);
    }
    if (N <= 4096) return launch_fps<512, 8>(xyz, B, N, npoint, idx_out, s);
    if (N <= 8192) return launch_fps<1024, 8>(xyz, B, N, npoint, idx_out, s);
    if (N <= 16384) return launch_fps<1024, 16>(xyz, B, N, npoint, idx_out, s);
    return fail(PTT_EUNSUPPORTED, "ptt_fps_f32: N=%d exceeds the register-resident limit 16384 (use ptt_fps_ws_f32)", N);
}

extern "C" int ptt_spatial_order_f32(const float* xyz, int B, int N, int32_t* order, ptt_stream_t stream) {
    if (B < 0 || N <= 0) return fail(PTT_EINVAL, "ptt_spatial_order_f32: B=%d N=%d", B, N);
    if (B == 0) return PTT_OK;
    if (!xyz || !order) return fail(PTT_EINVAL, "ptt_spatial_order_f32: null pointer");
    if (N > 8192 || (long long)B * N > INT_MAX) return fail(PTT_EUNSUPPORTED, "ptt_spatial_order_f32: N=%d (at most 8192 points per cloud are sorted in LDS)", N);
    int P = 2;
    while (P < N) P <<= 1;
    const int lds = P * (int)sizeof(unsigned long long);
    if (int rc = set_lds_limit(reinterpret_cast<const void*>(spatial_order_kernel), lds)) return rc;
    hipLaunchKernelGGL(spatial_order_kernel, dim3(B), dim3(1024), lds, as_stream(stream), xyz, N, P, order);
    return check_launch("spatial_order_kernel");
}

extern "C" int ptt_fps_ws_f32(const float* xyz, int B, int N, int npoint, int32_t* idx_out, float* workspace, size_t workspace_elems,
                              ptt_stream_t stream) {
    if (B < 0 || N <= 0 || npoint < 0) return fail(PTT_EINVAL, "ptt_fps_ws_f32: B=%d N=%d npoint=%d", B, N, npoint);
    if (B == 0 || npoint == 0) return PTT_OK;
    if (!xyz || !idx_out) return fail(PTT_EINVAL, "ptt_fps_ws_f32: null pointer");
    if ((long long)N * 3 > INT_MAX) return fail(PTT_EUNSUPPORTED, "ptt_fps_ws_f32: N=%d", N);
    if (!workspace || workspace_elems < (size_t)B * N)
        return fail(PTT_EWORKSPACE, "ptt_fps_ws_f32: %zu floats of workspace needed", (size_t)B * N);
    hipLaunchKernelGGL(fps_ws_kernel, dim3(B), dim3(1024), 0, as_stream(stream), xyz, N, npoint, workspace, idx_out);
    return check_launch("fps_ws_kernel");
}

extern "C" int ptt_ffps_f32(const float* xyz, const float* feat, int64_t feat_sb, int64_t feat_sc, int64_t feat_sn, int B, int N, int C,
                            int npoint, int32_t* idx_out, ptt_stream_t stream) {
    if (B < 1 || N < 1 || npoint < 1 || C < 0) return fail(PTT_EINVAL, "ptt_ffps_f32: B=%d N=%d C=%d npoint=%d", B, N, C, npoint);
    if (!xyz || !idx_out || (C > 0 && !feat)) return fail(PTT_EINVAL, "ptt_ffps_f32: null pointer");
    if (N > FFPS_MAX_N || C > FFPS_MAX_C || npoint > FFPS_MAX_NPOINT)
        return fail(PTT_EUNSUPPORTED, "ptt_ffps_f32: N=%d C=%d npoint=%d exceed the limits N <= %d, C <= %d, npoint <= %d", N, C, npoint,
                    FFPS_MAX_N, FFPS_MAX_C, FFPS_MAX_NPOINT);
    if (C > 0 && (long long)(N - 1) * llabs((long long)feat_sn) + (long long)(C - 1) * llabs((long long)feat_sc) > INT_MAX)
        return fail(PTT_EUNSUPPORTED, "ptt_ffps_f32: one cloud's features span more than 2^31 elements (strides %lld, %lld)",
                    (long long)feat_sc, (long long)feat_sn);
    hipStream_t s = as_stream(stream);
    if (C == 0) { feat = xyz; feat_sb = feat_sc = feat_sn = 0; }
    if (!dev_switches().ffps_stream) {
        int rc = -1;
        if (C == 128) rc = launch_ffps_resident<128>(xyz, feat, feat_sb, feat_sc, feat_sn, B, N, npoint, idx_out, s);
        else if (C == 256) rc = launch_ffps_resident<256>(xyz, feat, feat_sb, feat_sc, feat_sn, B, N, npoint, idx_out, s);
        else if (C == 257) rc = launch_ffps_resident<257>(xyz, feat, feat_sb, feat_sc, feat_sn, B, N, npoint, idx_out, s);
        if (rc != -1) return rc;
    }
#define PTT_FFPS_CASE(T, P) return launch_ffps<T, P>(xyz, feat, feat_sb, feat_sc, feat_sn, B, N, C, npoint, idx_out, s)
    if (N <= 64) PTT_FFPS_CASE(64, 1);
    if (N <= 128) PTT_FFPS_CASE(128, 1);
    if (N <= 256) PTT_FFPS_CASE(256, 1);
    if (N <= 512) PTT_FFPS_CASE(512, 1);
    if (N <= 1024) PTT_FFPS_CASE(1024, 1);
    if (N <= 2048) PTT_FFPS_CASE(1024, 2);
    if (N <= 4096) PTT_FFPS_CASE(1024, 4);
    if (N <= 8192) PTT_FFPS_CASE(1024, 8);
    PTT_FFPS_CASE(1024, 16);
#undef PTT_FFPS_CASE
}

static int ball_cpw(int BM, int M) {
    const int force = dev_switches().ball_cpw;
    if (force == 1 || (M & 3) != 0) return 1;
    if (force == 8 && (M & 7) == 0) return 8;
    if (force == 4) return 4;
    return BM >= 4 * 256 * 8 ? 4 : 1;
}

extern "C" int ptt_ball_query_f32(const float* new_xyz, const float* xyz, int B, int M, int N, float radius,
                                  int nsample, int32_t* idx_out, ptt_stream_t stream) {
    if (B < 0 || M < 0 || N <= 0 || nsample <= 0)
        return fail(PTT_EINVAL, "ptt_ball_query_f32: B=%d M=%d N=%d nsample=%d", B, M, N, nsample);
    if (B == 0 || M == 0) return PTT_OK;
    if (!new_xyz || !xyz || !idx_out) return fail(PTT_EINVAL, "ptt_ball_query_f32: null pointer");
    const float r2 = radius * radius;
    const int BM = B * M;
    const int cpw = ball_cpw(BM, M);
    if (cpw == 8)
        hipLaunchKernelGGL((ball_query_kernel<8>), dim3((BM / 8 + 3) / 4), dim3(256), 0, as_stream(stream), new_xyz, xyz, BM, M,
                           N, r2, nsample, idx_out);
    else if (cpw == 4)
        hipLaunchKernelGGL((ball_query_kernel<4>), dim3((BM / 4 + 3) / 4), dim3(256), 0, as_stream(stream), new_xyz, xyz, BM, M,
                           N, r2, nsample, idx_out);
    else
// ... 250 lines not shown
```

ptt_amd/models/backbones_3d/pointnet2/pointnet2_modules.py:

```python
import os
from typing import List

import torch
import torch.nn as nn
import torch.nn.functional as F

from .... import ops, train_ops
from ....param_cache import (DropsCachesOnModeChange, FoldedLayer, ParamCache, conv_bn_tensors, fold_conv_bn,
                             index_table)
from . import pointnet2_utils
from . import pytorch_utils as pt_utils

STREAM_COMPACT_MIN_BALLS = 2048
STREAM_COMPACT_MAX_POINTS = 1024


class PointnetSAModuleVotes(DropsCachesOnModeChange, nn.Module):
    def __init__(self, *, mlp: List[int], radius: float = None, nsample: int = None, bn: bool = True,
                 use_xyz: bool = True, normalize_xyz: bool = False, sample_uniformly: bool = False,
                 sample_method='fps'):
        super().__init__()
        self.radius = radius
        self.nsample = nsample
        self.mlp_module = None
        self.use_xyz = use_xyz
        self.normalize_xyz = normalize_xyz
        self.sample_uniformly = sample_uniformly
        self.grouper = pointnet2_utils.QueryAndGroup(radius, nsample, use_xyz=use_xyz, ret_grouped_xyz=True,
                                                     normalize_xyz=normalize_xyz, sample_uniformly=sample_uniformly,
                                                     ret_unique_cnt=False)
        mlp_spec = mlp
        if use_xyz and len(mlp_spec) > 0:
            mlp_spec[0] += 3
        self.mlp_module = pt_utils.SharedMLP(mlp_spec, bn=bn)
        self.sample_method = sample_method
        self._fused_cache = ParamCache()
        self.centres_knn_k = 0
        self.centres_knn = None

    def _sample(self, xyz, features, npoint):
        if self.sample_method == 'fps':
            return pointnet2_utils.furthest_point_sample(xyz, npoint)
        if self.sample_method in ('rs', 'sequence'):
            return index_table(xyz.size(0), npoint, xyz.device, torch.int32)
        if self.sample_method == 'ffps':
            if features is None:
                raise ValueError("sample_method 'ffps': a level without point features cannot sample in feature space "
                                 "(use 'fps' for it)")
            return ops.feature_fps(xyz.contiguous(), features.detach(), npoint)
        raise NotImplementedError(self.sample_method)

    def _fusable(self, xyz, features):
        if self.training or not xyz.is_cuda:
            return False
        name = 'PointnetSAModuleVotes(nsample=%s, mlp=%s)' % (self.nsample, [u.conv.weight.shape[0] for u in self.mlp_module
                                                                              if hasattr(u, 'conv')])
        if ops.autograd_recording(self, xyz, features):
            return ops.note_unfused(name, 'autograd is recording (wrap inference in torch.no_grad())')
        if self.sample_uniformly or self.nsample not in (16, 32, 64):
            return ops.note_unfused(name, 'nsample must be 16, 32 or 64 and sample_uniformly off')
        if xyz.dtype != torch.float32 or (features is not None and features.dtype != torch.float32):
            return ops.note_unfused(name, 'inputs must be float32')
        if len(self.mlp_module) > 4:
            return ops.note_unfused(name, 'more than 4 SharedMLP layers')
        for unit in self.mlp_module:
            conv = getattr(unit, 'conv', None)
            if conv is None or conv.kernel_size != (1, 1) or conv.weight.shape[0] % 32 != 0 or conv.weight.shape[0] > 256:
                return ops.note_unfused(name, 'layer widths must be multiples of 32, at most 256, 1x1 convolutions')
            if list(unit._modules.keys())[0] != 'conv':
                return ops.note_unfused(name, 'pre-activation units')
        return True

    def _fused_params(self, device):
        return self._fused_cache.get(conv_bn_tensors(self.mlp_module), device, self._fold)

    def _fold(self):
        layers, scale0 = [], None
        for li, unit in enumerate(self.mlp_module):
            w = unit.conv.weight
            cout, cin = w.shape[0], w.shape[1]
            rot = 3 if (li == 0 and self.use_xyz and cin > 3) else 0
            scale, shift = fold_conv_bn(unit)
            scale0 = scale if li == 0 else scale0
            wq = w if scale is None else w * scale.view(-1, 1, 1, 1)
            layers.append(FoldedLayer(ops.pack_weight(wq, rot), None, shift, cin, cout, hasattr(unit, 'activation')))
        hoist = None
        w0 = self.mlp_module[0].conv.weight
        if (self.use_xyz and len(layers) >= 2 and w0.shape[1] > 3 and layers[0].cout <= 256
                and os.environ.get('PTT_SA_HOIST', '1') != '0'):
            w2 = w0.reshape(w0.shape[0], w0.shape[1]).float()
            wx = w2[:, 0:3] if scale0 is None else w2[:, 0:3] * scale0[:, None]
            wf = w2[:, 3:] if scale0 is None else w2[:, 3:] * scale0[:, None]
            hoist = (ops.pack_weight(wf.contiguous()), wx.t().contiguous(), layers[0].cout, layers[0].relu)
        return layers, hoist

    def forward(self, xyz: torch.Tensor, features: torch.Tensor, npoint: int, inds: torch.Tensor = None, pre=None,
                compact: bool = False):
        self.centres_knn = None
        if self._fusable(xyz, features):
            return self._forward_fused(xyz, features, npoint, inds, pre, compact)
        return self._forward_train(xyz, features, npoint, inds)

    def _forward_fused(self, xyz, features, npoint, inds, pre, compact):
        if (pre is None and inds is None and self.sample_method == 'fps' and xyz.shape[1] <= 256 and npoint <= 128
                and xyz.shape[0] * npoint * self.nsample <= ops.ONE_FRAME_MAX_SA_ROWS and self.centres_knn_k <= npoint):
            xyz = xyz.contiguous()
            inds, inds64, new_xyz, idx, self.centres_knn = ops.fps_ball_knn(xyz, npoint, self.radius, self.nsample, self.centres_knn_k)
            pre = (new_xyz, idx, inds64)
        prefix = inds is None and self.sample_method in ('rs', 'sequence')
        if pre is not None:
            pass
        elif prefix:
            inds64 = index_table(xyz.size(0), npoint, xyz.device, torch.int64)
        elif inds is None:
            inds = self._sample(xyz, features, npoint)
        else:
            assert inds.shape[1] == npoint
            inds = inds.to(torch.int32)

        xyz = xyz.contiguous()
        if pre is not None:
            new_xyz, idx, inds64 = pre
        elif prefix:
            new_xyz, _, idx = ops.centres_ball_query(xyz, None, npoint, self.radius, self.nsample)
        else:
            new_xyz, inds64, idx = ops.centres_ball_query(xyz, inds.contiguous(), npoint, self.radius, self.nsample)
        layers, hoist = self._fused_params(xyz.device)
        if hoist is not None and features is not None:
            wf_packed, wx, c0, relu0 = hoist
            rows = features.transpose(1, 2)
            uniform = rows.stride(2) == 1 and rows.stride(0) == rows.shape[1] * rows.stride(1)
            term = ops.linear(rows if uniform else rows.contiguous(), wf_packed, c0, None, layers[0].shift, relu=False)
            B, M, ns = xyz.shape[0], npoint, self.nsample
            if (B * M * ns <= ops.ONE_FRAME_MAX_SA_ROWS and ns in (16, 32) and len(layers) == 3 and c0 % 4 == 0 and c0 >= 192):
                L1, L2 = layers[1], layers[2]
                h = torch.empty((B * M * ns, L1.cout), dtype=torch.float32, device=xyz.device)
                ops.row_jobs([pt_utils.layer_job(L1, prologue=3, x=term, idx=idx, xyz=xyz, centres=new_xyz, wx=wx,
                                                 radius=self.radius, ns=ns, M=M, N=xyz.shape[1], normalize_xyz=self.normalize_xyz,
                                                 pro_relu=relu0, out=h)])
                pooled = torch.empty((B, M, L2.cout), dtype=torch.float32, device=xyz.device)
                ops.row_jobs([pt_utils.layer_job(L2, x=h, epilogue=2, ns=ns, M=M, out=pooled)])
                return new_xyz, pooled.transpose(1, 2), inds64
            new_features = ops.sa_fused_forward(xyz, new_xyz, idx, None, layers[1:], self.radius, True,
                                                self.normalize_xyz, point_major_out=True, l0=(term, wx, relu0),
                                                compact=(bool(compact) and B * M >= STREAM_COMPACT_MIN_BALLS
                                                         and xyz.shape[1] <= STREAM_COMPACT_MAX_POINTS))
        else:
            new_features = ops.sa_fused_forward(xyz, new_xyz, idx, features, layers, self.radius,
                                                self.use_xyz, self.normalize_xyz, point_major_out=True,
                                                compact=features is None)
        return new_xyz, new_features, inds64

    def _forward_train(self, xyz, features, npoint, inds):
        if inds is None:
            inds = self._sample(xyz, features, npoint)
        else:
            assert inds.shape[1] == npoint
            inds = inds.to(torch.int32)
        hoist = (self.use_xyz and not self.sample_uniformly and self.nsample * npoint <= 16384
                 and train_ops.usable(self.mlp_module, xyz if features is None else features)
                 and self.mlp_module[0].conv.weight.shape[0] % 4 == 0)
        if hoist and not xyz.requires_grad and inds.dtype == torch.int32:
            new_xyz, inds64, idx = ops.centres_ball_query(xyz.contiguous(), inds.contiguous(), npoint, self.radius, self.nsample)
            y = train_ops.sa_level_hoisted(xyz, new_xyz, features, idx, self.mlp_module, self.radius, self.normalize_xyz)
            return new_xyz, y, inds64
        xyz_flipped = xyz.transpose(1, 2).contiguous()
        new_xyz = pointnet2_utils.gather_operation(xyz_flipped, inds).transpose(1, 2).contiguous()
        if hoist and features is not None:
            idx = pointnet2_utils.ball_query(self.radius, self.nsample, xyz, new_xyz)
            y = train_ops.sa_level_hoisted(xyz, new_xyz, features, idx, self.mlp_module, self.radius, self.normalize_xyz)
            return new_xyz, y, inds.to(torch.int64)
        grouped_features, grouped_xyz = self.grouper(xyz, new_xyz, features)
        if train_ops.usable(self.mlp_module, grouped_features):
            return new_xyz, train_ops.shared_mlp_pool(grouped_features, self.mlp_module, pool_dim=3), inds.to(torch.int64)
        y = self.mlp_module(grouped_features)
        y = y.max(dim=3)[0]
        return new_xyz, y, inds.to(torch.int64)
```

ptt_amd/models/backbones_3d/pointnet2_backbone.py:

```python
from typing import List

import torch
import torch.nn as nn

from ... import graph_policy, ops, train_ops
from ...param_cache import ParamCache, index_table
from .pointnet2 import pointnet2_modules


class PointNet2BackboneLight(nn.Module):
    def __init__(self, model_cfg, input_channels, **kwargs):
        super().__init__()
        self.model_cfg = model_cfg
        input_channels -= 3
        self.num_points_each_layer = []
        self.SA_modules = nn.ModuleList()
        sa = self.model_cfg.SA_CONFIG
        for k in range(len(sa.RADIUS)):
            mlps = list(sa.MLPS[k])
            if k == 0:
                mlps[0] = input_channels
            self.SA_modules.append(pointnet2_modules.PointnetSAModuleVotes(
                radius=sa.RADIUS[k], nsample=sa.NSAMPLE[k], mlp=mlps,
                use_xyz=sa.get('USE_XYZ', True), normalize_xyz=sa.get('NORMALIZE_XYZ', True),
                sample_method=sa.SAMPLE_METHOD[k]))
        self.cov_final = nn.Conv1d(256, 256, kernel_size=1)
        self.num_point_features = sa.MLPS[-1][-1]
        self._cov_cache = ParamCache()
        self.seed_knn = 16
        self.overlap_branches = True
        self._side_stream = None

    @staticmethod
    def _break_up_pc(pc):
        xyz = pc[..., 0:3].contiguous()
        features = pc[..., 3:].contiguous() if pc.size(-1) > 3 else None
        return xyz, features

    def _cov_final(self, features):
        if not features.is_cuda:
            return self.cov_final(features)
        if self.training:
            if features.dtype != torch.float32:
                return self.cov_final(features)
            return train_ops.rows_linear(self.cov_final, features.transpose(1, 2)).transpose(1, 2)
        if ops.autograd_recording(self.cov_final, features) or features.dtype != torch.float32:
            ops.note_unfused('PointNet2BackboneLight.cov_final', 'autograd is recording or input is not float32')
            return self.cov_final(features)
        w, b = self.cov_final.weight, self.cov_final.bias
        wpacked, bias = self._cov_cache.get([w, b], w.device, lambda: (ops.pack_weight(w), b.detach().float().contiguous()))
        rows = features.transpose(1, 2)
        out = ops.linear(rows, wpacked, w.shape[0], None, bias)
        return out.transpose(1, 2)

    def branch_forward(self, pts, npoints: List, inds0=None, want_knn=0, compact_levels=()):
        xyz, features = self._break_up_pc(pts)
        sa = self.model_cfg.SA_CONFIG
        one_frame = (not self.training and xyz.is_cuda and features is None and len(self.SA_modules) == 3
                     and xyz.shape[0] * npoints[0] <= 4 * ops.ONE_FRAME_MAX_POINTS
                     and self.SA_modules[0].sample_method == 'fps'
                     and all(m.sample_method in ('rs', 'sequence') for m in self.SA_modules[1:])
                     and npoints[0] >= npoints[1] >= npoints[2] and (not want_knn or npoints[2] <= 128)
                     and all(m._fusable(xyz, None) for m in self.SA_modules[:1]))
        knn = None
        if one_frame:
            from .pointnet2 import pointnet2_utils
            xyz = xyz.contiguous()
            if inds0 is None:
                inds0 = pointnet2_utils.furthest_point_sample(xyz, npoints[0])
            inds0 = inds0.to(torch.int32).contiguous()
            levels, inds64, knn = ops.sa_levels_point_jobs(xyz, inds0, list(npoints), list(sa.RADIUS), list(sa.NSAMPLE),
                                                           knn_k=want_knn)
            seq = [None] + [index_table(xyz.size(0), n, xyz.device, torch.int64) for n in npoints[1:3]]
            xyz, features, inds0 = self.SA_modules[0](xyz=xyz, features=features, npoint=npoints[0], inds=inds0,
                                                      pre=(levels[0][0], levels[0][1], inds64))
            xyz, features, inds1 = self.SA_modules[1](xyz=xyz, features=features, npoint=npoints[1],
                                                      pre=(levels[1][0], levels[1][1], seq[1]))
            xyz, features, inds2 = self.SA_modules[2](xyz=xyz, features=features, npoint=npoints[2],
                                                      pre=(levels[2][0], levels[2][1], seq[2]))
        else:
            xyz, features, inds0 = self.SA_modules[0](xyz=xyz, features=features, npoint=npoints[0], inds=inds0)
            xyz, features, inds1 = self.SA_modules[1](xyz=xyz, features=features, npoint=npoints[1], compact=1 in compact_levels)
            xyz, features, inds2 = self.SA_modules[2](xyz=xyz, features=features, npoint=npoints[2], compact=2 in compact_levels)
        point_features = self._cov_final(features)
        assert inds1.dtype == inds2.dtype == torch.int64, 'index type must be int64, not {}'.format(inds2.dtype)
        if all(m.sample_method in ('rs', 'sequence') for m in self.SA_modules[1:]) and inds0.shape[1] >= npoints[2]:
            inds = inds0[:, :npoints[2]]
        else:
            inds = inds0.gather(1, inds1).gather(1, inds2)
        if want_knn:
            return xyz, point_features, inds, knn
        return xyz, point_features, inds

    def sample(self, search_points, template_points):
        from .pointnet2 import pointnet2_utils
        sa = self.model_cfg.SA_CONFIG
        assert sa.SAMPLE_METHOD[0] == 'fps'
        return (pointnet2_utils.furthest_point_sample(search_points[..., 0:3].contiguous(), sa.NPOINTS_SEARCH[0]),
                pointnet2_utils.furthest_point_sample(template_points[..., 0:3].contiguous(), sa.NPOINTS_TEMPLATE[0]))

    def forward_branches(self, search_points, template_points, inds=None):
        sa = self.model_cfg.SA_CONFIG
        i_s, i_t = inds if inds is not None else (None, None)
        last = (len(self.SA_modules) - 1,) if (search_points.is_cuda and not self.training) else ()
        if not (self.overlap_branches and search_points.is_cuda and not self.training):
            r = self.branch_forward(search_points, sa.NPOINTS_SEARCH, i_s, want_knn=self.seed_knn, compact_levels=last)
            t_seeds, t_feats, t_inds = self.branch_forward(template_points, sa.NPOINTS_TEMPLATE, i_t)
        else:
            if self._side_stream is None or self._side_stream.device != search_points.device:
                self._side_stream = torch.cuda.Stream(device=search_points.device)
            main = torch.cuda.current_stream(search_points.device)
            side = graph_policy.branch(main, self._side_stream)
            with torch.cuda.stream(side):
                t_seeds, t_feats, t_inds = self.branch_forward(template_points, sa.NPOINTS_TEMPLATE, i_t)
            r = self.branch_forward(search_points, sa.NPOINTS_SEARCH, i_s, want_knn=self.seed_knn, compact_levels=last)
            graph_policy.join(main, side)
            if side is not main:
                for t in (t_seeds, t_feats, t_inds, template_points):
                    t.record_stream(main)
        s_seeds, s_feats, s_inds = r[:3]
        s_knn = r[3] if len(r) > 3 else None
        out = {'search_seeds': s_seeds, 'search_feats': s_feats, 'search_inds': s_inds,
               'template_seeds': t_seeds, 'template_feats': t_feats, 'template_inds': t_inds}
        if s_knn is not None:
            out['search_seeds_knn'] = s_knn
        return out

    def forward(self, batch_dict):
        batch_dict.update(self.forward_branches(batch_dict['search_points'], batch_dict['template_points'],
                                                batch_dict.pop('fps_inds', None)))
        batch_dict.pop('search_points')
        batch_dict.pop('template_points')
        return batch_dict
```

ptt_amd/ops.py:

```python
import contextlib
import ctypes
import os

import torch

from . import _lib
from ._lib import AttnDesc, SaDesc, SaLayer, XcorrDesc


def _stream():
    return ctypes.c_void_p(torch.cuda.current_stream().cuda_stream)


_timing = None


def start_kernel_timing(names):
    global _timing
    _timing = {n: [] for n in names}


def stop_kernel_timing():
    global _timing
    t, _timing = _timing, None
# ... 52 lines not shown


def drop_params():
    global param_generation
    param_generation += 1


class StateWatch(object):

    def __init__(self, module):
        self.tensors = list(module.parameters()) + list(module.buffers())
        self.mark()

    def _key(self):
        return list(map(torch.Tensor.data_ptr, self.tensors)), [t._version for t in self.tensors]

    def mark(self):
        self.generation, self.key = param_generation, self._key()

    def changed(self):
        return param_generation != self.generation or self._key() != self.key


def require_finite(*tensors):
    bad = [k for k, t in enumerate(tensors) if t is not None and t.is_floating_point() and not bool(torch.isfinite(t).all())]
    if bad:
        raise ValueError("non-finite values in tensor(s) %s" % ", ".join("#%d %s" % (k, tuple(tensors[k].shape)) for k in bad))


def _chk(t, name, dtype, ndim=None):
    if not isinstance(t, torch.Tensor):
        raise TypeError("%s must be a torch.Tensor" % name)
    if not t.is_cuda:
        raise RuntimeError("%s must be a device (HIP) tensor — CPU tensors are not supported" % name)
    if t.dtype != dtype:
        raise RuntimeError("%s must be %s, got %s" % (name, dtype, t.dtype))
    if not t.is_contiguous():
        raise RuntimeError("%s must be contiguous" % name)
    if ndim is not None and t.dim() != ndim:
        raise RuntimeError("%s must have %d dimensions, got %s" % (name, ndim, tuple(t.shape)))
    return t


def _ptr(t):
    return ctypes.c_void_p(t.data_ptr()) if t is not None else ctypes.c_void_p(0)


_UNTIMED = contextlib.nullcontext()


def _launch(name, device, *args, timed=None):
    with torch.cuda.device(device), (_timed(timed) if timed else _UNTIMED):
        rc = getattr(_lib.lib(), name)(*args, _stream())
    if rc:
        _lib.check(rc, name)


def _host(name, *args):
    return getattr(_lib.lib(), name)(*args)


def _host_checked(name, *args):
    _lib.check(_host(name, *args), name)


def _workspace(query, device, *dims):
    ws = _ws(_host(query, *dims), device)
    return ws, (_ptr(ws), ws.numel() * 8)


FPS_RESIDENT_MAX_N, FPS_RESIDENT_MAX_NPOINT = 16384, 15360


def furthest_point_sampling(xyz, npoint):
    _chk(xyz, "xyz", torch.float32, 3)
    B, N, _ = xyz.shape
    out = torch.empty((B, int(npoint)), dtype=torch.int32, device=xyz.device)
    if N <= FPS_RESIDENT_MAX_N and int(npoint) <= FPS_RESIDENT_MAX_NPOINT:
        _launch("ptt_fps_f32", xyz.device, _ptr(xyz), B, N, int(npoint), _ptr(out), timed='ptt_fps_f32')
    else:
        ws = torch.empty((B * N,), dtype=torch.float32, device=xyz.device)
        _launch("ptt_fps_ws_f32", xyz.device, _ptr(xyz), B, N, int(npoint), _ptr(out), _ptr(ws), ws.numel(), timed='ptt_fps_f32')
    return out


FFPS_MAX_N, FFPS_MAX_C, FFPS_MAX_NPOINT = 16384, 1024, 15360


def feature_fps(xyz, features, npoint):
    _chk(xyz, "xyz", torch.float32, 3)
    B, N, _ = xyz.shape
    C = 0
    if features is not None:
        if not isinstance(features, torch.Tensor):
            raise TypeError("features must be a torch.Tensor")
        if not features.is_cuda:
            raise RuntimeError("features must be a device (HIP) tensor — CPU tensors are not supported")
        if features.dtype != torch.float32:
            raise RuntimeError("features must be torch.float32, got %s" % features.dtype)
        if features.dim() != 3 or features.shape[0] != B or features.shape[2] != N:
            raise RuntimeError("features must be (B,C,N) = (%d,C,%d), got %s" % (B, N, tuple(features.shape)))
        C = features.shape[1]
    npoint = int(npoint)
    if N > FFPS_MAX_N or C > FFPS_MAX_C or npoint > FFPS_MAX_NPOINT:
        raise ValueError("feature_fps: N=%d, C=%d, npoint=%d exceed the kernel's limits N <= %d, C <= %d, npoint <= %d"
                         % (N, C, npoint, FFPS_MAX_N, FFPS_MAX_C, FFPS_MAX_NPOINT))
    if N < 1 or npoint < 1:
        raise ValueError("feature_fps: N=%d and npoint=%d must be at least 1" % (N, npoint))
    out = torch.empty((B, npoint), dtype=torch.int32, device=xyz.device)
    if B == 0:
        return out
    sb, sc, sn = features.stride() if C else (0, 0, 0)
    if C and (N - 1) * abs(sn) + (C - 1) * abs(sc) > 2 ** 31 - 1:
        raise ValueError("feature_fps: one cloud's features span more than 2^31 - 1 elements (strides %d, %d)" % (sc, sn))
    _launch("ptt_ffps_f32", xyz.device, _ptr(xyz), _ptr(features if C else None), sb, sc, sn, B, N, C, npoint, _ptr(out),
            timed='ptt_ffps_f32')
    return out


def gather_points(features, idx):
    _chk(features, "features", torch.float32, 3)
    _chk(idx, "idx", torch.int32, 2)
    B, C, N = features.shape
    M = idx.shape[1]
    out = torch.empty((B, C, M), dtype=torch.float32, device=features.device)
    _launch("ptt_gather_f32", features.device, _ptr(features), _ptr(idx), B, C, N, M, _ptr(out))
    return out


def scatter_add_det(src, idx, N):
    B, C, E = src.shape
    out = torch.empty((B, C, int(N)), dtype=torch.float32, device=src.device)
    nbytes = _host("ptt_scatter_add_det_workspace", B, int(N), E)
    ws = torch.empty((max(1, (nbytes + 3) // 4),), dtype=torch.int32, device=src.device)
    _launch("ptt_scatter_add_det_f32", src.device, _ptr(src), _ptr(idx), B, C, int(N), E, _ptr(out), _ptr(ws), ws.numel() * 4)
    return out


_ATOMIC_GRADS = os.environ.get("PTT_ATOMIC_GRADS", "0")


def set_atomic_grads(on):
    global _ATOMIC_GRADS
    prev = _ATOMIC_GRADS == "1"
    _ATOMIC_GRADS = "1" if on else "0"
    return prev


def _det_grads(entries, N):
    if int(N) * 16384 > 0xffffffff:
        return False
    return entries <= 16384 and _ATOMIC_GRADS != "1"


def gather_points_grad(grad_out, idx, N):
    _chk(grad_out, "grad_out", torch.float32, 3)
    _chk(idx, "idx", torch.int32, 2)
    B, C, M = grad_out.shape
    if M > 0 and _det_grads(M, N):
        return scatter_add_det(grad_out, idx, N)
    out = torch.empty((B, C, int(N)), dtype=torch.float32, device=grad_out.device)
    _launch("ptt_gather_grad_f32", grad_out.device, _ptr(grad_out), _ptr(idx), B, C, int(N), M, _ptr(out))
    return out


def select_centres(xyz, idx, npoint, want_idx64=True):
# ... 55 lines not shown
    return out


def group_points_grad(grad_out, idx, N):
    _chk(grad_out, "grad_out", torch.float32, 4)
    _chk(idx, "idx", torch.int32, 3)
    B, C, M, ns = grad_out.shape
    if M * ns > 0 and _det_grads(M * ns, N):
        return scatter_add_det(grad_out.view(B, C, M * ns), idx.view(B, M * ns), N)
    out = torch.empty((B, C, int(N)), dtype=torch.float32, device=grad_out.device)
    _launch("ptt_group_grad_f32", grad_out.device, _ptr(grad_out), _ptr(idx), B, C, int(N), M, ns, _ptr(out))
    return out


def _unreached(name):
    def fn(*a, **k):
        raise NotImplementedError("%s is never reached by PTT (SURVEY.md §2.1) and is not provided" % name)
    fn.__name__ = name
    return fn


three_nn = _unreached("three_nn")
three_interpolate = _unreached("three_interpolate")
three_interpolate_grad = _unreached("three_interpolate_grad")
furthest_point_sampling_with_dist = _unreached("furthest_point_sampling_with_dist")


def knn(xyz, k, want_rel=False):
    _chk(xyz, "xyz", torch.float32, 3)
    B, N, _ = xyz.shape
    out = torch.empty((B, N, int(k)), dtype=torch.int32, device=xyz.device)
    rel = torch.empty((B, N, int(k), 3), dtype=torch.float32, device=xyz.device) if want_rel else None
    _launch("ptt_knn_rel_f32", xyz.device, _ptr(xyz), B, N, int(k), _ptr(out), _ptr(rel), timed='ptt_knn_f32')
    return (out, rel) if want_rel else out


def pack_weight(weight, rot=0):
    w = weight.detach()
    w = w.reshape(w.shape[0], -1).contiguous().float()
    _chk(w, "weight", torch.float32, 2)
    Cout, K = w.shape
    n = _host("ptt_packed_weight_elems", Cout, K)
    out = torch.empty((n,), dtype=torch.float32, device=w.device)
    _launch("ptt_pack_weight_rot_f32", w.device, _ptr(w), Cout, K, int(rot), _ptr(out))
    return out


ONE_FRAME_MAX_SA_ROWS = 4096
ROW_JOB_MAX_ROWS = 1024
ONE_FRAME_MAX_POINTS = int(os.environ.get("PTT_PT_PER_LAYER_MAX", "512"))


def linear(x, wpacked, cout, scale=None, shift=None, relu=False, residual=None, out=None):
    if not x.is_cuda or x.dtype != torch.float32:
        raise RuntimeError("x must be a float32 device tensor")
    K = x.shape[-1]
    x2 = x.reshape(-1, K)
    if x2.stride(1) != 1:
        x2 = x2.contiguous()
    rows = x2.shape[0]
    if out is None:
        out = torch.empty(tuple(x.shape[:-1]) + (int(cout),), dtype=torch.float32, device=x.device)
    o2 = out.view(-1, int(cout))
    r2 = None
    if residual is not None:
        r2 = residual.reshape(-1, int(cout))
        if r2.stride(1) != 1:
            r2 = r2.contiguous()
    if (scale is None and (rows > 8192 or (rows >= 6144 and int(cout) == 256)) and x2.data_ptr() % 16 == 0 and o2.is_contiguous()
            and _host("ptt_rows_gemm_supported", rows, K, int(cout), x2.stride(0), int(cout))):
        _launch("ptt_rows_gemm_f32", x.device, _ptr(x2), rows, K, x2.stride(0), None, None, _ptr(wpacked), int(cout), _ptr(shift), 1 if relu else 0,
                _ptr(r2), r2.stride(0) if r2 is not None else int(cout), _ptr(o2), int(cout), None, 0, timed='ptt_linear_f32')
        return out
    if rows <= ROW_JOB_MAX_ROWS and 192 <= K <= 1024 and o2.stride(1) == 1:
        row_jobs([row_job(wpacked, cout, x=x2, scale=scale, shift=shift, act=1 if relu else 0, res=r2, out=o2)])
        return out
    _launch("ptt_linear_f32", x.device, _ptr(x2), rows, K, x2.stride(0) if rows > 1 else K, _ptr(wpacked), int(cout), _ptr(scale), _ptr(shift),
            1 if relu else 0, _ptr(r2), (r2.stride(0) if (r2 is not None and rows > 1) else int(cout)), _ptr(o2),
            o2.stride(0) if rows > 1 else int(cout), timed='ptt_linear_f32')
    return out


def sa_fused_forward(xyz, new_xyz, idx, features, layers, radius, use_xyz=True, normalize_xyz=False,
                     point_major_out=True, l0=None, compact=False):
    _chk(xyz, "xyz", torch.float32, 3)
    _chk(new_xyz, "new_xyz", torch.float32, 3)
    _chk(idx, "idx", torch.int32, 3)
    B, N, _ = xyz.shape
    _, M, ns = idx.shape
    d = SaDesc()
    d.xyz, d.new_xyz, d.idx = xyz.data_ptr(), new_xyz.data_ptr(), idx.data_ptr()
    if features is not None:
        if not features.is_cuda or features.dtype != torch.float32 or features.dim() != 3:
            raise RuntimeError("features must be a (B,C,N) float32 device tensor")
        d.feat = features.data_ptr()
        d.feat_sb, d.feat_sc, d.feat_sn = features.stride()
        d.C = features.shape[1]
    else:
        d.feat, d.C = None, 0
    cout = layers[-1][4]
    if point_major_out:
        store = torch.empty((B, M, cout), dtype=torch.float32, device=xyz.device)
        out = store.transpose(1, 2)
    else:
        out = torch.empty((B, cout, M), dtype=torch.float32, device=xyz.device)
    d.out = out.data_ptr()
    d.out_sb, d.out_sc, d.out_sm = out.stride()
    d.B, d.N, d.M, d.nsample = B, N, M, ns
    d.radius, d.use_xyz, d.normalize_xyz = float(radius), int(bool(use_xyz)), int(bool(normalize_xyz))
    d.n_layers = len(layers)
    for i, (wp, sc, sh, cin, co, relu) in enumerate(layers):
        L = d.layers[i]
        L.Wpacked = wp.data_ptr()
        L.scale = sc.data_ptr() if sc is not None else None
        L.shift = sh.data_ptr() if sh is not None else None
        L.Cin, L.Cout, L.relu = int(cin), int(co), int(bool(relu))
    if l0 is not None:
        term, wx, l0_relu = l0
        if features is not None:
            raise RuntimeError("with a hoisted layer 0 the point features are already inside l0[0]")
        _chk(term, "l0 point term", torch.float32, 3)
        _chk(wx, "l0 xyz weight", torch.float32, 2)
        if term.shape[0] != B or term.shape[1] != N or wx.shape[0] != 3 or wx.shape[1] != term.shape[2]:
            raise RuntimeError("l0 point term must be (B,N,C0) and the xyz weight (3,C0)")
        d.l0_point_term, d.l0_xyz_weight = term.data_ptr(), wx.data_ptr()
        d.l0_channels, d.l0_relu = term.shape[2], int(bool(l0_relu))
    if isinstance(compact, torch.Tensor):
        if not compact.is_cuda or compact.device != xyz.device or not compact.is_contiguous():
            raise RuntimeError("compact workspace must be a contiguous tensor on %s" % xyz.device)
        d.compact_ws, d.compact_ws_bytes = compact.data_ptr(), compact.numel() * compact.element_size()
    elif compact:
        ws, (_, d.compact_ws_bytes) = _workspace("ptt_sa_compact_workspace", xyz.device, B, M)
        d.compact_ws = ws.data_ptr()
    _launch("ptt_sa_fused_fwd_f32", xyz.device, ctypes.byref(d), timed='ptt_sa_fused_fwd_f32')
    return out


def cosine_map(search_feats, templ_feats, eps=1e-8):
    for t_, n_ in ((search_feats, "search_feats"), (templ_feats, "templ_feats")):
        if not isinstance(t_, torch.Tensor) or not t_.is_cuda or t_.dtype != torch.float32 or t_.dim() != 3:
            raise RuntimeError("%s must be a (B,C,N) float32 device tensor" % n_)
    if search_feats.shape[:2] != templ_feats.shape[:2] or search_feats.device != templ_feats.device:
        raise RuntimeError("search_feats and templ_feats must share batch size, channel count and device")
    B, C, Ns = search_feats.shape
    Nt = templ_feats.shape[2]
    out = torch.empty((B, Ns, Nt), dtype=torch.float32, device=search_feats.device)
    ssb, ssc, ssn = search_feats.stride()
    tsb, tsc, tsn = templ_feats.stride()
    _launch("ptt_cosine_map_f32", out.device, search_feats.data_ptr(), ssb, ssn, ssc, templ_feats.data_ptr(), tsb, tsn, tsc, B, Ns, Nt, C, float(eps),
            out.data_ptr(), timed='ptt_cosine_map_f32')
    return out


def rows_mlp(x, layers, residual=None):
    if not x.is_cuda or x.dtype != torch.float32 or x.stride(-1) != 1:
        raise RuntimeError("rows_mlp: x must be a float32 device tensor with contiguous rows")
    K = x.shape[-1]
    x2 = x.reshape(-1, K)
    rows = x2.shape[0]
    cout = int(layers[-1][4])
    out = torch.empty((rows, cout), dtype=torch.float32, device=x.device)
    res2 = None
    if residual is not None:
        res2 = residual.reshape(-1, cout)
        _chk(res2 if res2.is_contiguous() else res2.contiguous(), "residual", torch.float32, 2)
        res2 = res2 if res2.stride(1) == 1 else res2.contiguous()
    arr = (SaLayer * len(layers))()
    for i, (wp, sc, sh, cin, co, relu) in enumerate(layers):
        arr[i].Wpacked = wp.data_ptr()
        arr[i].scale = sc.data_ptr() if sc is not None else None
        arr[i].shift = sh.data_ptr() if sh is not None else None
        arr[i].Cin, arr[i].Cout, arr[i].relu = int(cin), int(co), int(bool(relu))
    _launch("ptt_rows_mlp_f32", x.device, _ptr(x2), rows, K, x2.stride(0), arr, len(layers), _ptr(res2), res2.stride(0) if res2 is not None else 0,
            _ptr(out), cout, timed='ptt_rows_mlp_f32')
    return out.view(*x.shape[:-1], cout)


def xcorr_fused(search_feats, templ_feats, P, w_sim, scale0, shift0, layers, eps=1e-8, want_sim=False, cos_t=None, split=False):
    for t_, n_ in ((search_feats, "search_feats"), (templ_feats, "templ_feats")):
        if not t_.is_cuda or t_.dtype != torch.float32 or t_.dim() != 3:
            raise RuntimeError("%s must be a (B,C,N) float32 device tensor" % n_)
    _chk(P, "P", torch.float32, 3)
    _chk(w_sim, "w_sim", torch.float32, 1)
    B, C, Ns = search_feats.shape
    Nt = templ_feats.shape[2]
    C0 = P.shape[2]
    if Nt <= 0 or Nt % 64:
        raise RuntimeError("xcorr_fused: Nt=%d (ptt_xcorr_fused_fwd_f32 walks the template seeds in chunks of 64)" % Nt)
    if P.shape[0] != B or P.shape[1] != Nt or w_sim.shape[0] != C0 or templ_feats.shape[:2] != search_feats.shape[:2]:
        raise RuntimeError("xcorr_fused: inconsistent shapes")
    cout = layers[-1][4]
    split = (split and not want_sim and search_feats.stride(1) == 1 and templ_feats.stride(1) == 1 and C % 4 == 0 and (B * Ns) % 8 == 0
             and all(st % 4 == 0 for st in (search_feats.stride(0), search_feats.stride(2), templ_feats.stride(0), templ_feats.stride(2)))
             and search_feats.data_ptr() % 16 == 0 and templ_feats.data_ptr() % 16 == 0 and bool(layers[-1][5]))
    if not split:
        if cos_t is None:
            cos_t = cosine_map(search_feats, templ_feats, eps=eps)
        _chk(cos_t, "cos_t", torch.float32, 3)
        if tuple(cos_t.shape) != (B, Ns, Nt):
            raise RuntimeError("xcorr_fused: cos_t must be (B,Ns,Nt)")
    store = torch.empty(((2, B, Ns, cout) if split else (B, Ns, cout)), dtype=torch.float32, device=P.device)
    out = store.transpose(-1, -2)
    sim = torch.empty((B, Nt, Ns), dtype=torch.float32, device=P.device) if want_sim else None
    d = XcorrDesc()
    if split:
        d.split, d.out_sh = 1, store.stride(0)
        d.search_feat, d.templ_feat = search_feats.data_ptr(), templ_feats.data_ptr()
        d.s_sb, d.s_sn, d.t_sb, d.t_sn = search_feats.stride(0), search_feats.stride(2), templ_feats.stride(0), templ_feats.stride(2)
        d.C, d.eps = int(C), float(eps)
    else:
        d.cos_t = cos_t.data_ptr()
    d.P, d.w_sim = P.data_ptr(), w_sim.data_ptr()
    d.scale0 = scale0.data_ptr() if scale0 is not None else None
    d.shift0 = shift0.data_ptr() if shift0 is not None else None
    d.out = out.data_ptr()
    d.out_sb, d.out_sc, d.out_sn = out.stride()[-3:]
# ... 1301 lines not shown
```

Baseline: 17410.

## Track live FPS centre counts and skip duplicate centres in SA kernels

A live-count variant of furthest point sampling stops once every remaining point has zero distance and records, per batch, how many distinct centres were found. The fused set-abstraction kernels (stream, compact, LDS) then process only the live centres, remapping tile-to-centre indexing through a prefix-sum seek. A small fill kernel copies the first centre's output into the skipped slots. The aim is to avoid recomputing duplicate centres for sparse point clouds, at the cost of extra seek logic, an extra launch and a runtime branch per block.

Result: no change. 17270 (-0.8%).

```diff
diff --git a/include/ptt_hip.h b/include/ptt_hip.h
--- a/include/ptt_hip.h
+++ b/include/ptt_hip.h
@@ -8,7 +8,7 @@
 extern "C" {
 #endif
 
-#define PTT_ABI_VERSION 31
+#define PTT_ABI_VERSION 32
 
 enum {
     PTT_OK = 0,
@@ -28,6 +28,8 @@
                 ptt_stream_t stream);
 int ptt_fps_ws_f32(const float* xyz, int B, int N, int npoint, int32_t* idx_out, float* workspace,
                    size_t workspace_elems, ptt_stream_t stream);
+int ptt_fps_live_f32(const float* xyz, int B, int N, int npoint, int32_t* idx_out, int32_t* live_out,
+                     ptt_stream_t stream);
 
 int ptt_ffps_f32(const float* xyz, const float* feat, int64_t feat_sb, int64_t feat_sc, int64_t feat_sn,
                  int B, int N, int C, int npoint, int32_t* idx_out, ptt_stream_t stream);
@@ -141,6 +143,7 @@
     int l0_relu;
     void* compact_ws;
     size_t compact_ws_bytes;
+    const int32_t* live;
 } ptt_sa_desc;
 
 int ptt_sa_fused_fwd_f32(const ptt_sa_desc* d, ptt_stream_t stream);
diff --git a/ptt_amd/_lib.py b/ptt_amd/_lib.py
--- a/ptt_amd/_lib.py
+++ b/ptt_amd/_lib.py
@@ -173,7 +173,7 @@
                 ("radius", c_float), ("use_xyz", c_int), ("normalize_xyz", c_int), ("n_layers", c_int),
                 ("layers", SaLayer * PTT_SA_MAX_LAYERS),
                 ("l0_point_term", c_void_p), ("l0_xyz_weight", c_void_p), ("l0_channels", c_int), ("l0_relu", c_int),
-                ("compact_ws", c_void_p), ("compact_ws_bytes", c_size_t)]
+                ("compact_ws", c_void_p), ("compact_ws_bytes", c_size_t), ("live", c_void_p)]
 
 
 class XcorrDesc(Structure):
diff --git a/ptt_amd/csrc/common.h b/ptt_amd/csrc/common.h
--- a/ptt_amd/csrc/common.h
+++ b/ptt_amd/csrc/common.h
@@ -25,6 +25,7 @@
     int pair_stagger = 0;
     int pair_lds_pad = 0;
     int sa_lds_chunk = 2;
+    int sa_live = 1;
     int fps_plain = 0;
     int ball_cpw = 0;
     int fps_t = 0;
diff --git a/ptt_amd/csrc/errors.hip b/ptt_amd/csrc/errors.hip
--- a/ptt_amd/csrc/errors.hip
+++ b/ptt_amd/csrc/errors.hip
@@ -43,6 +43,7 @@
     if (const char* e = getenv("PTT_BALL_CPW")) d.ball_cpw = atoi(e);
     if (const char* e = getenv("PTT_FPS_PLAIN")) d.fps_plain = atoi(e);
     if (const char* e = getenv("PTT_SA_LDS_CHUNK")) d.sa_lds_chunk = atoi(e);
+    if (const char* e = getenv("PTT_SA_LIVE")) d.sa_live = atoi(e) != 0;
     if (const char* e = getenv("PTT_FPS_T")) d.fps_t = atoi(e);
     if (const char* e = getenv("PTT_FFPS_STREAM")) d.ffps_stream = atoi(e);
     if (getenv("PTT_GROUP_GRAD_GLOBAL")) d.group_grad_global = 1;
diff --git a/ptt_amd/csrc/mfma_ops.hip b/ptt_amd/csrc/mfma_ops.hip
--- a/ptt_amd/csrc/mfma_ops.hip
+++ b/ptt_amd/csrc/mfma_ops.hip
@@ -446,6 +446,7 @@
     float radius;
     long long* dbg;
     int32_t* cws;
+    const int32_t* live;
     SaLayerDev L[PTT_SA_MAX_LAYERS];
 };
 
@@ -784,11 +785,66 @@
 
 struct SasCentre {
     int c, b, m;
+    int live;
     __device__ __forceinline__ void advance(int k, int M) {
         c += k; m += k;
         while (m >= M) { m -= M; ++b; }
     }
+    __device__ __forceinline__ void advance(int k, int M, int B, const int32_t* lv);
 };
+
+__device__ __forceinline__ int sas_live_count(const int32_t* lv, int b, int M) {
+    const int l = lv[b];
+    return l < 1 ? 1 : (l > M ? M : l);
+}
+
+__device__ __forceinline__ void SasCentre::advance(int k, int M, int B, const int32_t* lv) {
+    if (!lv) { advance(k, M); return; }
+    m += k;
+    while (b < B && m >= live) {
+        m -= live; ++b;
+        live = b < B ? sas_live_count(lv, b, M) : M;
+    }
+    c = b * M + m;
+}
+
+__device__ __forceinline__ void sas_live_seek(const int32_t* lv, int B, int M, int v, int lane, SasCentre& ce, int& tot) {
+    int base = 0;
+    bool found = false;
+    ce.b = B; ce.m = 0; ce.live = M;
+    for (int b0 = 0; b0 < B; b0 += 64) {
+        const int i = b0 + lane;
+        const int L = i < B ? sas_live_count(lv, i, M) : 0;
+        int inc = L;
+        for (int off = 1; off < 64; off <<= 1) {
+            const int o = __shfl_up(inc, off, 64);
+            if (lane >= off) inc += o;
+        }
+        inc += base;
+        const unsigned long long hit = __ballot(i < B && inc > v);
+        if (!found && hit != 0ull) {
+            const int src = __ffsll((long long)hit) - 1;
+            ce.live = __builtin_amdgcn_readlane(L, src);
+            ce.b = b0 + src;
+            ce.m = v - (__builtin_amdgcn_readlane(inc, src) - ce.live);
+            found = true;
+        }
+        base = __builtin_amdgcn_readlane(inc, 63);
+    }
+    if (!found) ce.m = v - base;
+    ce.c = ce.b * M + ce.m;
+    tot = base;
+}
+
+__device__ __forceinline__ bool sas_live_partial(const int32_t* lv, int B, int M, int lane) {
+    bool partial = false;
+    for (int b0 = 0; b0 < B; b0 += 64) {
+        const int i = b0 + lane;
+        const int L = i < B ? sas_live_count(lv, i, M) : M;
+        partial |= __ballot(L != M) != 0ull;
+    }
+    return partial;
+}
 
 __device__ __forceinline__ float sas_pool(const f32x16& a, float sh, int relu) {
     float mx = a[0];
@@ -804,8 +860,8 @@
 #ifndef PTT_SAS_EXP
 #define PTT_SAS_EXP 0
 #endif
-template <int NS>
-__global__ __launch_bounds__(256, 2) void sa_stream_kernel(SaParams p) {
+template <int NS, bool LIVE>
+__device__ __forceinline__ void sa_stream_body(const SaParams& p) {
     static_assert(NS == 32, "one centre per 32-row tile");
     extern __shared__ __attribute__((aligned(16))) float smem[];
     float* const P = smem;
@@ -813,10 +869,8 @@
     float* const meta = smem + 2 * SAS_TILE;
     const int t = threadIdx.x, lane = t & 63, half = lane >> 5, sub = half, q = lane & 31;
     const int w = __builtin_amdgcn_readfirstlane(t >> 6);
-    const int tile0 = logical_block() * p.chunk;
-    const int ntiles = min(p.chunk, p.tiles - tile0);
-    if (ntiles <= 0) return;
-    stagger_second_slot(p.first_wave, p.stagger);
+    const int tile0 = (LIVE ? (int)blockIdx.x : logical_block()) * p.chunk;
+    if (p.tiles <= tile0) return;
     const SaLayerDev& L1 = p.L[0];
     const SaLayerDev& L2 = p.L[1];
     const __amdgpu_buffer_rsrc_t rf = weight_rsrc(p.feat);
@@ -839,13 +893,26 @@
     const int M = p.M, N = p.N;
     const int osb = (int)p.osb, osm = (int)p.osm;
     const int ocol0 = (w * 32 + col) * (int)p.osc, ocol1 = ((w + 4) * 32 + col) * (int)p.osc;
-
-    SasCentre own, first;
+    const int32_t* const lv = LIVE ? p.live : nullptr;
+    SasCentre first{0, 0, 0, 0};
+    int tiles = p.tiles;
+    if constexpr (LIVE) {
+        int tot = 0;
+        sas_live_seek(lv, p.B, p.M, tile0 * 2, lane, first, tot);
+        tiles = (tot + 1) >> 1;
+    }
+    const int ntiles = min(p.chunk, tiles - tile0);
+    if (ntiles <= 0) return;
+    stagger_second_slot(p.first_wave, p.stagger);
+
+    SasCentre own;
     {
-        const int c0 = tile0 * 2;
-        first.c = c0; first.b = c0 / M; first.m = c0 - first.b * M;
+        if constexpr (!LIVE) {
+            const int c0 = tile0 * 2;
+            first.c = c0; first.b = c0 / M; first.m = c0 - first.b * M; first.live = M;
+        }
         own = first;
-        own.advance(w >> 1, M);
+        own.advance(w >> 1, M, p.B, lv);
     }
     auto meta_index = [&](const SasCentre& ce) -> int {
         const int c = ce.c < total_centres ? ce.c : total_centres - 1;
@@ -893,7 +960,7 @@
 
     auto store_pooled = [&](const SasCentre& f) {
         SasCentre c1 = f;
-        c1.advance(1, M);
+        c1.advance(1, M, p.B, lv);
         if (half == 0) {
             if (f.c < total_centres) {
                 float* o = p.out + (f.b * osb + f.m * osm);
@@ -909,7 +976,7 @@
     for (int it = 0; it < ntiles; ++it) {
         const bool more = it + 1 < ntiles;
         SasCentre own_next = own;
-        if (more) own_next.advance(2, M);
+        if (more) own_next.advance(2, M, p.B, lv);
         if (!(PTT_SAS_EXP & 1)) lds_barrier();
         const int nn = meta_index(own_next);
         MetaXyz mx;
@@ -1044,11 +1111,17 @@
 #undef SAS_A2
         }
         prev = first;
-        if (more) { first.advance(2, M); own = own_next; }
+        if (more) { first.advance(2, M, p.B, lv); own = own_next; }
     }
 #pragma unroll
     for (int i = 0; i < 4; ++i) pv[i >> 1][i & 1] = sas_pool(acc[i >> 1][i & 1], (i & 1) ? sh2b : sh2a, L2.relu);
     store_pooled(prev);
+}
+
+template <int NS>
+__global__ __launch_bounds__(256, 2) void sa_stream_kernel(SaParams p) {
+    if (p.live && sas_live_partial(p.live, p.B, p.M, threadIdx.x & 63)) sa_stream_body<NS, true>(p);
+    else sa_stream_body<NS, false>(p);
 }
 
 struct XcorrParams {
@@ -1291,7 +1364,7 @@
 
 template <bool XYZ>
 __global__ __launch_bounds__(256) void sa_compact_kernel(const float* __restrict__ xyz, const int32_t* __restrict__ idx, int N, int M,
-                                                         SacTable tab) {
+                                                         SacTable tab, const int32_t* __restrict__ live) {
     __shared__ int s_cnt[4], s_base[4], s_cls[32], s_pos[32], s_nd[32];
     __shared__ int s_row[32][32];
     const int t = threadIdx.x, lane = t & 63, half = lane >> 5, s = lane & 31, w = t >> 6;
@@ -1302,6 +1375,15 @@
     uint32_t x[SAC_PASSES], y[SAC_PASSES], z[SAC_PASSES];
 #pragma unroll
     for (int q = 0; q < SAC_PASSES; ++q) iv[q] = idx[(size_t)min(g0 + q * 8 + w * 2 + half, T - 1) * 32 + s];
+    int mrest[SAC_PASSES];
+#pragma unroll
+    for (int q = 0; q < SAC_PASSES; ++q) {
+        mrest[q] = 1;
+        if (live) {
+            const int g = min(g0 + q * 8 + w * 2 + half, T - 1), b = g / M;
+            mrest[q] = sas_live_count(live, b, M) - (g - b * M);
+        }
+    }
     if constexpr (XYZ) {
 #pragma unroll
         for (int q = 0; q < SAC_PASSES; ++q) {
@@ -1334,11 +1416,11 @@
         if (keep) s_row[lc][__popc(m & ((1u << s) - 1u))] = iv[q];
         if (s == 0) {
             const int k = nd <= 4 ? 0 : nd <= 8 ? 1 : nd <= 16 ? 2 : 3;
-            const bool valid = g0 + lc < T;
+            const bool valid = g0 + lc < T && mrest[q] > 0;
             s_cls[lc] = valid ? k : -1;
             s_nd[lc] = nd;
             s_pos[lc] = valid ? atomicAdd(&s_cnt[k], 1) : 0;
-            if (valid) tab.ndist()[g0 + lc] = nd;
+            if (g0 + lc < T) tab.ndist()[g0 + lc] = nd;
         }
     }
     __syncthreads();
@@ -1350,6 +1432,23 @@
         const int q = s_base[k] + s_pos[lc];
         tab.rows(k)[(size_t)q * (4 << k) + j] = s_row[lc][j < s_nd[lc] ? j : 0];
         if (j == 0) tab.list(k)[q] = g0 + lc;
+    }
+}
+
+constexpr int SALF_ROWS = 16;
+__global__ __launch_bounds__(256) void sa_live_fill_kernel(float* __restrict__ out, long long osb, long long osc, long long osm, int B,
+                                                           int M, int C, const int32_t* __restrict__ live) {
+    const int per = (M + SALF_ROWS - 1) / SALF_ROWS;
+    const int b = blockIdx.x / per, m0 = (blockIdx.x - b * per) * SALF_ROWS;
+    if (b >= B) return;
+    const int L = sas_live_count(live, b, M);
+    if (m0 + SALF_ROWS <= L) return;
+    float* const ob = out + (long long)b * osb;
+    const bool m_fast = osm == 1;
+    for (int e = threadIdx.x; e < SALF_ROWS * C; e += 256) {
+        const int r = m_fast ? e % SALF_ROWS : e / C, c = m_fast ? e / SALF_ROWS : e - (e / C) * C;
+        const int m = m0 + r;
+        if (m >= L && m < M) ob[(long long)c * osc + (long long)m * osm] = ob[(long long)c * osc];
     }
 }
 
@@ -1490,7 +1589,7 @@
     const float* b2p = W2 + lane * 4;
     const __amdgpu_buffer_rsrc_t rx = weight_rsrc(p.xyz);
 
-    SasCentre ce{0, 0, 0};
+    SasCentre ce{0, 0, 0, 0};
     SacTile tc{0, 0, 0};
     float px, py, pz, cx, cy, cz;
     int g_cur = 0;
@@ -2114,9 +2213,18 @@
     p.first_wave = 1024; p.stagger = dev_switches().sa_stagger;
     p.dbg = dev_switches().stamps;
     p.cws = nullptr;
+    p.live = dev_switches().sa_live ? d->live : nullptr;
     const int total_centres = d->B * d->M;
     hipStream_t s = as_stream(stream);
     int rc;
+    auto finish = [&](const char* what) -> int {
+        if (int r = check_launch(what)) return r;
+        if (!p.live) return PTT_OK;
+        const int cout = p.L[d->n_layers - 1].Cout;
+        hipLaunchKernelGGL(sa_live_fill_kernel, dim3(d->B * ((d->M + SALF_ROWS - 1) / SALF_ROWS)), dim3(256), 0, s, p.out, p.osb, p.osc,
+                           p.osm, d->B, d->M, cout, p.live);
+        return check_launch("sa_live_fill_kernel");
+    };
     if (d->C == 0 && d->use_xyz && !hoist && d->nsample == 32 && d->n_layers == 3 && p.L[0].Cout == 64 && p.L[1].Cout == 64 &&
         p.L[2].Cout == 128 && !p.L[0].scale && !p.L[1].scale && !p.L[2].scale && p.L[0].relu && p.L[1].relu &&
         dev_switches().sa_lds) {
@@ -2134,12 +2242,12 @@
             hipLaunchKernelGGL(sa_compact_zero_kernel, dim3(1), dim3(64), 0, s, p.cws);
             if ((rc = check_launch("sa_compact_zero_kernel"))) return rc;
             hipLaunchKernelGGL(sa_compact_kernel<true>, dim3((total_centres + 31) / 32), dim3(256), 0, s, d->xyz, d->idx, d->N, d->M,
-                               SacTable{p.cws, total_centres});
+                               SacTable{p.cws, total_centres}, p.live);
             if ((rc = check_launch("sa_compact_kernel"))) return rc;
             if (wgs > 256 * PTT_SAL_WGS) wgs = 256 * PTT_SAL_WGS;
             if ((rc = set_lds_limit(reinterpret_cast<const void*>(sa_lds_kernel<true>), lds))) return rc;
             hipLaunchKernelGGL(sa_lds_kernel<true>, dim3(wgs), dim3(64 * nw), lds, s, p);
-            return check_launch("sa_lds_kernel");
+            return finish("sa_lds_kernel");
         }
         if ((rc = set_lds_limit(reinterpret_cast<const void*>(sa_lds_kernel<false>), lds))) return rc;
         hipLaunchKernelGGL(sa_lds_kernel<false>, dim3(wgs), dim3(64 * nw), lds, s, p);
@@ -2181,17 +2289,17 @@
             hipLaunchKernelGGL(sa_compact_zero_kernel, dim3(1), dim3(64), 0, s, p.cws);
             if ((rc = check_launch("sa_compact_zero_kernel"))) return rc;
             hipLaunchKernelGGL(sa_compact_kernel<false>, dim3((total_centres + 31) / 32), dim3(256), 0, s, d->xyz, d->idx, d->N, d->M,
-                               SacTable{p.cws, total_centres});
+                               SacTable{p.cws, total_centres}, p.live);
             if ((rc = check_launch("sa_compact_kernel"))) return rc;
             const int lds = (2 * SAS_TILE + 64 * 4 + 64) * (int)sizeof(float);
             if ((rc = set_lds_limit(reinterpret_cast<const void*>(sa_stream_compact_kernel), lds))) return rc;
             hipLaunchKernelGGL(sa_stream_compact_kernel, dim3(p.tiles < 512 ? p.tiles : 512), dim3(256), lds, s, p);
-            return check_launch("sa_stream_compact_kernel");
+            return finish("sa_stream_compact_kernel");
         }
         const int lds = (2 * SAS_TILE + 4 * 16 * 4) * (int)sizeof(float);
         if ((rc = set_lds_limit(reinterpret_cast<const void*>(sa_stream_kernel<32>), lds))) return rc;
         hipLaunchKernelGGL((sa_stream_kernel<32>), dim3(wgs), dim3(256), lds, s, p);
-        return check_launch("sa_stream_kernel");
+        return finish("sa_stream_kernel");
     }
     int RT = dev_switches().sa_rt;
     if (d->nsample == 64) RT = 2;
diff --git a/ptt_amd/csrc/point_ops.hip b/ptt_amd/csrc/point_ops.hip
--- a/ptt_amd/csrc/point_ops.hip
+++ b/ptt_amd/csrc/point_ops.hip
@@ -23,9 +23,9 @@
 typedef float fps_f2 __attribute__((ext_vector_type(2)));
 
 
-template <int T, int P, bool LX, int ABL = 0>
+template <int T, int P, bool LX, int ABL = 0, bool LIVE = false>
 __global__ __launch_bounds__(T) void fps_kernel(const float* __restrict__ xyz, int N, int npoint,
-                                               int32_t* __restrict__ idx_out) {
+                                               int32_t* __restrict__ idx_out, int32_t* __restrict__ live_out) {
     constexpr int W = T / 64;
     const int b = blockIdx.x;
     const float* __restrict__ pts = xyz + (size_t)b * N * 3;
@@ -59,7 +59,10 @@
     if (t == 0 && npoint > 0) sel_lds[0] = 0;
     if (LX) __syncthreads();
 
-    for (int j = 1; j < npoint; ++j) {
+    float gdv = 1.0f;
+    int fillv = 0;
+    int j = 1;
+    for (; j < npoint && (!LIVE || __ballot(gdv > 0.f) != 0ull); ++j) {
         float best = -1.0f, bx = 0.f, by = 0.f, bz = 0.f;
         int besti = 0;
         if constexpr ((P % 2) == 0) {
@@ -112,6 +115,7 @@
         if constexpr (W == 1) {
             int widx = __builtin_amdgcn_readlane(besti, src);
             if (wmax < 0.f) widx = 0;
+            if constexpr (LIVE) { gdv = wmax; fillv = widx; }
             if constexpr ((ABL & 8) != 0) {
                 lx = (float)widx * 1e-3f; ly = lx; lz = lx;
             } else if constexpr (LX) {
@@ -181,6 +185,7 @@
             }
             if (gd < 0.f) gi = 0;
             if constexpr ((ABL & 16) != 0) gi &= 1023;
+            if constexpr (LIVE) { gdv = gd; fillv = gi; }
             if constexpr ((ABL & 8) != 0) {
                 lx = (float)gi * 1e-3f; ly = lx; lz = lx;
             } else if constexpr (LX) {
@@ -193,26 +198,35 @@
         }
     }
     __syncthreads();
-    for (int j = t; j < npoint; j += T) out[j] = sel_lds[j];
+    if constexpr (LIVE) {
+        const bool out_of_points = __ballot(gdv > 0.f) == 0ull;
+        const int fill = __builtin_amdgcn_readfirstlane(fillv);
+        for (int k = t; k < npoint; k += T) out[k] = k < j ? sel_lds[k] : fill;
+        if (t == 0) live_out[b] = (out_of_points && fill == 0) ? j - 1 : npoint;
+    } else {
+        for (int k = t; k < npoint; k += T) out[k] = sel_lds[k];
+    }
 }
 
 template <int T, int P>
-static int launch_fps(const float* xyz, int B, int N, int npoint, int32_t* idx, hipStream_t s) {
+static int launch_fps(const float* xyz, int B, int N, int npoint, int32_t* idx, int32_t* live, hipStream_t s) {
     const size_t sel_bytes = (size_t)((npoint + 3) & ~3) * sizeof(int);
     if (sel_bytes + (size_t)N * 12 + 1024 <= 65536 && !dev_switches().fps_plain) {
 #ifdef PTT_DEV
         if (const char* e = getenv("PTT_FPS_ABL")) {
             const int abl = atoi(e);
-#define PTT_FPS_ABL_CASE(A) if (abl == A) { hipLaunchKernelGGL((fps_kernel<T, P, true, A>), dim3(B), dim3(T), sel_bytes + (size_t)N * 12, s, xyz, N, npoint, idx); return check_launch("fps_kernel(abl)"); }
+#define PTT_FPS_ABL_CASE(A) if (abl == A) { hipLaunchKernelGGL((fps_kernel<T, P, true, A>), dim3(B), dim3(T), sel_bytes + (size_t)N * 12, s, xyz, N, npoint, idx, live); return check_launch("fps_kernel(abl)"); }
             PTT_FPS_ABL_CASE(1) PTT_FPS_ABL_CASE(2) PTT_FPS_ABL_CASE(3) PTT_FPS_ABL_CASE(4) PTT_FPS_ABL_CASE(8) PTT_FPS_ABL_CASE(12) PTT_FPS_ABL_CASE(15)
             PTT_FPS_ABL_CASE(16) PTT_FPS_ABL_CASE(32) PTT_FPS_ABL_CASE(47) PTT_FPS_ABL_CASE(7) PTT_FPS_ABL_CASE(24) PTT_FPS_ABL_CASE(40)
 #undef PTT_FPS_ABL_CASE
         }
 #endif
-        hipLaunchKernelGGL((fps_kernel<T, P, true>), dim3(B), dim3(T), sel_bytes + (size_t)N * 12, s, xyz, N, npoint, idx);
+        if (live) hipLaunchKernelGGL((fps_kernel<T, P, true, 0, true>), dim3(B), dim3(T), sel_bytes + (size_t)N * 12, s, xyz, N, npoint, idx, live);
+        else hipLaunchKernelGGL((fps_kernel<T, P, true>), dim3(B), dim3(T), sel_bytes + (size_t)N * 12, s, xyz, N, npoint, idx, live);
         return check_launch("fps_kernel");
     }
-    hipLaunchKernelGGL((fps_kernel<T, P, false>), dim3(B), dim3(T), sel_bytes, s, xyz, N, npoint, idx);
+    if (live) hipLaunchKernelGGL((fps_kernel<T, P, false, 0, true>), dim3(B), dim3(T), sel_bytes, s, xyz, N, npoint, idx, live);
+    else hipLaunchKernelGGL((fps_kernel<T, P, false>), dim3(B), dim3(T), sel_bytes, s, xyz, N, npoint, idx, live);
     return check_launch("fps_kernel");
 }
 
@@ -1153,43 +1167,52 @@
 
 using namespace ptt;
 
-extern "C" int ptt_fps_f32(const float* xyz, int B, int N, int npoint, int32_t* idx_out, ptt_stream_t stream) {
-    if (B < 0 || N <= 0 || npoint < 0) return fail(PTT_EINVAL, "ptt_fps_f32: B=%d N=%d npoint=%d", B, N, npoint);
+static int fps_dispatch(const char* who, const float* xyz, int B, int N, int npoint, int32_t* idx_out, int32_t* live_out, ptt_stream_t stream) {
+    if (B < 0 || N <= 0 || npoint < 0) return fail(PTT_EINVAL, "%s: B=%d N=%d npoint=%d", who, B, N, npoint);
     if (B == 0 || npoint == 0) return PTT_OK;
-    if (!xyz || !idx_out) return fail(PTT_EINVAL, "ptt_fps_f32: null pointer");
-    if (npoint > 15360) return fail(PTT_EUNSUPPORTED, "ptt_fps_f32: npoint=%d exceeds the LDS index buffer (15360)", npoint);
+    if (!xyz || !idx_out) return fail(PTT_EINVAL, "%s: null pointer", who);
+    if (npoint > 15360) return fail(PTT_EUNSUPPORTED, "%s: npoint=%d exceeds the LDS index buffer (15360)", who, npoint);
     hipStream_t s = as_stream(stream);
-    if (N <= 64) return launch_fps<64, 1>(xyz, B, N, npoint, idx_out, s);
-    if (N <= 128) return launch_fps<64, 2>(xyz, B, N, npoint, idx_out, s);
-    if (N <= 256) return launch_fps<64, 4>(xyz, B, N, npoint, idx_out, s);
+    if (N <= 64) return launch_fps<64, 1>(xyz, B, N, npoint, idx_out, live_out, s);
+    if (N <= 128) return launch_fps<64, 2>(xyz, B, N, npoint, idx_out, live_out, s);
+    if (N <= 256) return launch_fps<64, 4>(xyz, B, N, npoint, idx_out, live_out, s);
     if (N <= 512) {
         if (const int T = dev_switches().fps_t) {
-            if (T == 256) return launch_fps<256, 2>(xyz, B, N, npoint, idx_out, s);
-            if (T == 128) return launch_fps<128, 4>(xyz, B, N, npoint, idx_out, s);
-            if (T == 512) return launch_fps<512, 1>(xyz, B, N, npoint, idx_out, s);
-        }
-        return launch_fps<64, 8>(xyz, B, N, npoint, idx_out, s);
+            if (T == 256) return launch_fps<256, 2>(xyz, B, N, npoint, idx_out, live_out, s);
+            if (T == 128) return launch_fps<128, 4>(xyz, B, N, npoint, idx_out, live_out, s);
+            if (T == 512) return launch_fps<512, 1>(xyz, B, N, npoint, idx_out, live_out, s);
+        }
+        return launch_fps<64, 8>(xyz, B, N, npoint, idx_out, live_out, s);
     }
     if (N <= 1024) {
         if (const int T = dev_switches().fps_t) {
-            if (T == 64) return launch_fps<64, 16>(xyz, B, N, npoint, idx_out, s);
-            if (T == 128) return launch_fps<128, 8>(xyz, B, N, npoint, idx_out, s);
-            if (T == 512) return launch_fps<512, 2>(xyz, B, N, npoint, idx_out, s);
-        }
-        return launch_fps<256, 4>(xyz, B, N, npoint, idx_out, s);
+            if (T == 64) return launch_fps<64, 16>(xyz, B, N, npoint, idx_out, live_out, s);
+            if (T == 128) return launch_fps<128, 8>(xyz, B, N, npoint, idx_out, live_out, s);
+            if (T == 512) return launch_fps<512, 2>(xyz, B, N, npoint, idx_out, live_out, s);
+        }
+        return launch_fps<256, 4>(xyz, B, N, npoint, idx_out, live_out, s);
     }
     if (N <= 2048) {
         if (const int T = dev_switches().fps_t) {
-            if (T == 512) return launch_fps<512, 4>(xyz, B, N, npoint, idx_out, s);
-            if (T == 1024) return launch_fps<1024, 2>(xyz, B, N, npoint, idx_out, s);
-            if (T == 128) return launch_fps<128, 16>(xyz, B, N, npoint, idx_out, s);
-        }
-        return launch_fps<256, 8>(xyz, B, N, npoint, idx_out, s);
-    }
-    if (N <= 4096) return launch_fps<512, 8>(xyz, B, N, npoint, idx_out, s);
-    if (N <= 8192) return launch_fps<1024, 8>(xyz, B, N, npoint, idx_out, s);
-    if (N <= 16384) return launch_fps<1024, 16>(xyz, B, N, npoint, idx_out, s);
-    return fail(PTT_EUNSUPPORTED, "ptt_fps_f32: N=%d exceeds the register-resident limit 16384 (use ptt_fps_ws_f32)", N);
+            if (T == 512) return launch_fps<512, 4>(xyz, B, N, npoint, idx_out, live_out, s);
+            if (T == 1024) return launch_fps<1024, 2>(xyz, B, N, npoint, idx_out, live_out, s);
+            if (T == 128) return launch_fps<128, 16>(xyz, B, N, npoint, idx_out, live_out, s);
+        }
+        return launch_fps<256, 8>(xyz, B, N, npoint, idx_out, live_out, s);
+    }
+    if (N <= 4096) return launch_fps<512, 8>(xyz, B, N, npoint, idx_out, live_out, s);
+    if (N <= 8192) return launch_fps<1024, 8>(xyz, B, N, npoint, idx_out, live_out, s);
+    if (N <= 16384) return launch_fps<1024, 16>(xyz, B, N, npoint, idx_out, live_out, s);
+    return fail(PTT_EUNSUPPORTED, "%s: N=%d exceeds the register-resident limit 16384 (use ptt_fps_ws_f32)", who, N);
+}
+
+extern "C" int ptt_fps_f32(const float* xyz, int B, int N, int npoint, int32_t* idx_out, ptt_stream_t stream) {
+    return fps_dispatch("ptt_fps_f32", xyz, B, N, npoint, idx_out, nullptr, stream);
+}
+
+extern "C" int ptt_fps_live_f32(const float* xyz, int B, int N, int npoint, int32_t* idx_out, int32_t* live_out, ptt_stream_t stream) {
+    if (B > 0 && npoint > 0 && !live_out) return fail(PTT_EINVAL, "ptt_fps_live_f32: null pointer");
+    return fps_dispatch("ptt_fps_live_f32", xyz, B, N, npoint, idx_out, live_out, stream);
 }
 
 extern "C" int ptt_spatial_order_f32(const float* xyz, int B, int N, int32_t* order, ptt_stream_t stream) {
diff --git a/ptt_amd/models/backbones_3d/pointnet2/pointnet2_modules.py b/ptt_amd/models/backbones_3d/pointnet2/pointnet2_modules.py
--- a/ptt_amd/models/backbones_3d/pointnet2/pointnet2_modules.py
+++ b/ptt_amd/models/backbones_3d/pointnet2/pointnet2_modules.py
@@ -13,6 +13,10 @@
 
 STREAM_COMPACT_MIN_BALLS = 2048
 STREAM_COMPACT_MAX_POINTS = 1024
+
+
+def live_enabled():
+    return os.environ.get('PTT_SA_LIVE', '1') != '0'
 
 
 class PointnetSAModuleVotes(DropsCachesOnModeChange, nn.Module):
@@ -37,6 +41,7 @@
         self._fused_cache = ParamCache()
         self.centres_knn_k = 0
         self.centres_knn = None
+        self.live_out = None
 
     def _sample(self, xyz, features, npoint):
         if self.sample_method == 'fps':
@@ -95,13 +100,14 @@
         return layers, hoist
 
     def forward(self, xyz: torch.Tensor, features: torch.Tensor, npoint: int, inds: torch.Tensor = None, pre=None,
-                compact: bool = False):
+                compact: bool = False, live: torch.Tensor = None):
         self.centres_knn = None
+        self.live_out = None
         if self._fusable(xyz, features):
-            return self._forward_fused(xyz, features, npoint, inds, pre, compact)
+            return self._forward_fused(xyz, features, npoint, inds, pre, compact, live if live_enabled() else None)
         return self._forward_train(xyz, features, npoint, inds)
 
-    def _forward_fused(self, xyz, features, npoint, inds, pre, compact):
+    def _forward_fused(self, xyz, features, npoint, inds, pre, compact, live=None):
         if (pre is None and inds is None and self.sample_method == 'fps' and xyz.shape[1] <= 256 and npoint <= 128
                 and xyz.shape[0] * npoint * self.nsample <= ops.ONE_FRAME_MAX_SA_ROWS and self.centres_knn_k <= npoint):
             xyz = xyz.contiguous()
@@ -109,14 +115,22 @@
             pre = (new_xyz, idx, inds64)
         prefix = inds is None and self.sample_method in ('rs', 'sequence')
         if pre is not None:
+            live = None
+        elif not prefix and inds is None:
+            live = None
+        if pre is not None:
             pass
         elif prefix:
             inds64 = index_table(xyz.size(0), npoint, xyz.device, torch.int64)
         elif inds is None:
-            inds = self._sample(xyz, features, npoint)
+            if self.sample_method == 'fps' and live_enabled():
+                inds, live = ops.furthest_point_sampling_live(xyz.contiguous(), npoint)
+            else:
+                inds = self._sample(xyz, features, npoint)
         else:
             assert inds.shape[1] == npoint
             inds = inds.to(torch.int32)
+        self.live_out = live
 
         xyz = xyz.contiguous()
         if pre is not None:
@@ -144,11 +158,11 @@
             new_features = ops.sa_fused_forward(xyz, new_xyz, idx, None, layers[1:], self.radius, True,
                                                 self.normalize_xyz, point_major_out=True, l0=(term, wx, relu0),
                                                 compact=(bool(compact) and B * M >= STREAM_COMPACT_MIN_BALLS
-                                                         and xyz.shape[1] <= STREAM_COMPACT_MAX_POINTS))
+                                                         and xyz.shape[1] <= STREAM_COMPACT_MAX_POINTS), live=live)
         else:
             new_features = ops.sa_fused_forward(xyz, new_xyz, idx, features, layers, self.radius,
                                                 self.use_xyz, self.normalize_xyz, point_major_out=True,
-                                                compact=features is None)
+                                                compact=features is None, live=live)
         return new_xyz, new_features, inds64
 
     def _forward_train(self, xyz, features, npoint, inds):
diff --git a/ptt_amd/models/backbones_3d/pointnet2_backbone.py b/ptt_amd/models/backbones_3d/pointnet2_backbone.py
--- a/ptt_amd/models/backbones_3d/pointnet2_backbone.py
+++ b/ptt_amd/models/backbones_3d/pointnet2_backbone.py
@@ -53,7 +53,7 @@
         out = ops.linear(rows, wpacked, w.shape[0], None, bias)
         return out.transpose(1, 2)
 
-    def branch_forward(self, pts, npoints: List, inds0=None, want_knn=0, compact_levels=()):
+    def branch_forward(self, pts, npoints: List, inds0=None, want_knn=0, compact_levels=(), live0=None):
         xyz, features = self._break_up_pc(pts)
         sa = self.model_cfg.SA_CONFIG
         one_frame = (not self.training and xyz.is_cuda and features is None and len(self.SA_modules) == 3
@@ -79,9 +79,10 @@
             xyz, features, inds2 = self.SA_modules[2](xyz=xyz, features=features, npoint=npoints[2],
                                                       pre=(levels[2][0], levels[2][1], seq[2]))
         else:
-            xyz, features, inds0 = self.SA_modules[0](xyz=xyz, features=features, npoint=npoints[0], inds=inds0)
-            xyz, features, inds1 = self.SA_modules[1](xyz=xyz, features=features, npoint=npoints[1], compact=1 in compact_levels)
-            xyz, features, inds2 = self.SA_modules[2](xyz=xyz, features=features, npoint=npoints[2], compact=2 in compact_levels)
+            sa0, sa1, sa2 = self.SA_modules
+            xyz, features, inds0 = sa0(xyz=xyz, features=features, npoint=npoints[0], inds=inds0, live=live0)
+            xyz, features, inds1 = sa1(xyz=xyz, features=features, npoint=npoints[1], compact=1 in compact_levels, live=sa0.live_out)
+            xyz, features, inds2 = sa2(xyz=xyz, features=features, npoint=npoints[2], compact=2 in compact_levels, live=sa1.live_out)
         point_features = self._cov_final(features)
         assert inds1.dtype == inds2.dtype == torch.int64, 'index type must be int64, not {}'.format(inds2.dtype)
         if all(m.sample_method in ('rs', 'sequence') for m in self.SA_modules[1:]) and inds0.shape[1] >= npoints[2]:
@@ -96,24 +97,32 @@
         from .pointnet2 import pointnet2_utils
         sa = self.model_cfg.SA_CONFIG
         assert sa.SAMPLE_METHOD[0] == 'fps'
+        if search_points.is_cuda and not self.training and pointnet2_modules.live_enabled():
+            return (ops.furthest_point_sampling_live(search_points[..., 0:3].contiguous(), sa.NPOINTS_SEARCH[0], packed=True),
+                    ops.furthest_point_sampling_live(template_points[..., 0:3].contiguous(), sa.NPOINTS_TEMPLATE[0], packed=True))
         return (pointnet2_utils.furthest_point_sample(search_points[..., 0:3].contiguous(), sa.NPOINTS_SEARCH[0]),
                 pointnet2_utils.furthest_point_sample(template_points[..., 0:3].contiguous(), sa.NPOINTS_TEMPLATE[0]))
 
     def forward_branches(self, search_points, template_points, inds=None):
         sa = self.model_cfg.SA_CONFIG
         i_s, i_t = inds if inds is not None else (None, None)
+        l_s = l_t = None
+        if i_s is not None and i_s.dim() == 1:
+            i_s, l_s = ops.split_packed_live(i_s, sa.NPOINTS_SEARCH[0])
+        if i_t is not None and i_t.dim() == 1:
+            i_t, l_t = ops.split_packed_live(i_t, sa.NPOINTS_TEMPLATE[0])
         last = (len(self.SA_modules) - 1,) if (search_points.is_cuda and not self.training) else ()
         if not (self.overlap_branches and search_points.is_cuda and not self.training):
-            r = self.branch_forward(search_points, sa.NPOINTS_SEARCH, i_s, want_knn=self.seed_knn, compact_levels=last)
-            t_seeds, t_feats, t_inds = self.branch_forward(template_points, sa.NPOINTS_TEMPLATE, i_t)
+            r = self.branch_forward(search_points, sa.NPOINTS_SEARCH, i_s, want_knn=self.seed_knn, compact_levels=last, live0=l_s)
+            t_seeds, t_feats, t_inds = self.branch_forward(template_points, sa.NPOINTS_TEMPLATE, i_t, live0=l_t)
         else:
             if self._side_stream is None or self._side_stream.device != search_points.device:
                 self._side_stream = torch.cuda.Stream(device=search_points.device)
             main = torch.cuda.current_stream(search_points.device)
             side = graph_policy.branch(main, self._side_stream)
             with torch.cuda.stream(side):
-                t_seeds, t_feats, t_inds = self.branch_forward(template_points, sa.NPOINTS_TEMPLATE, i_t)
-            r = self.branch_forward(search_points, sa.NPOINTS_SEARCH, i_s, want_knn=self.seed_knn, compact_levels=last)
+                t_seeds, t_feats, t_inds = self.branch_forward(template_points, sa.NPOINTS_TEMPLATE, i_t, live0=l_t)
+            r = self.branch_forward(search_points, sa.NPOINTS_SEARCH, i_s, want_knn=self.seed_knn, compact_levels=last, live0=l_s)
             graph_policy.join(main, side)
             if side is not main:
                 for t in (t_seeds, t_feats, t_inds, template_points):
diff --git a/ptt_amd/ops.py b/ptt_amd/ops.py
--- a/ptt_amd/ops.py
+++ b/ptt_amd/ops.py
@@ -158,6 +158,24 @@
         ws = torch.empty((B * N,), dtype=torch.float32, device=xyz.device)
         _launch("ptt_fps_ws_f32", xyz.device, _ptr(xyz), B, N, int(npoint), _ptr(out), _ptr(ws), ws.numel(), timed='ptt_fps_f32')
     return out
+
+
+def furthest_point_sampling_live(xyz, npoint, packed=False):
+    _chk(xyz, "xyz", torch.float32, 3)
+    B, N, _ = xyz.shape
+    if N > FPS_RESIDENT_MAX_N or int(npoint) > FPS_RESIDENT_MAX_NPOINT:
+        buf = torch.cat((furthest_point_sampling(xyz, npoint).reshape(-1),
+                         torch.full((B,), int(npoint), dtype=torch.int32, device=xyz.device)))
+        return buf if packed else split_packed_live(buf, npoint)
+    buf = torch.empty((B * int(npoint) + B,), dtype=torch.int32, device=xyz.device)
+    out, live = split_packed_live(buf, npoint)
+    _launch("ptt_fps_live_f32", xyz.device, _ptr(xyz), B, N, int(npoint), _ptr(out), _ptr(live), timed='ptt_fps_f32')
+    return buf if packed else (out, live)
+
+
+def split_packed_live(buf, npoint):
+    B = buf.numel() // (int(npoint) + 1)
+    return buf[:B * int(npoint)].view(B, int(npoint)), buf[B * int(npoint):]
 
 
 FFPS_MAX_N, FFPS_MAX_C, FFPS_MAX_NPOINT = 16384, 1024, 15360
@@ -379,7 +397,7 @@
 
 
 def sa_fused_forward(xyz, new_xyz, idx, features, layers, radius, use_xyz=True, normalize_xyz=False,
-                     point_major_out=True, l0=None, compact=False):
+                     point_major_out=True, l0=None, compact=False, live=None, out=None):
     _chk(xyz, "xyz", torch.float32, 3)
     _chk(new_xyz, "new_xyz", torch.float32, 3)
     _chk(idx, "idx", torch.int32, 3)
@@ -396,7 +414,10 @@
     else:
         d.feat, d.C = None, 0
     cout = layers[-1][4]
-    if point_major_out:
+    if out is not None:
+        if not out.is_cuda or out.dtype != torch.float32 or tuple(out.shape) != (B, cout, M):
+            raise RuntimeError("out must be a (B,Cout,M) float32 device tensor")
+    elif point_major_out:
         store = torch.empty((B, M, cout), dtype=torch.float32, device=xyz.device)
         out = store.transpose(1, 2)
     else:
@@ -429,6 +450,10 @@
     elif compact:
         ws, (_, d.compact_ws_bytes) = _workspace("ptt_sa_compact_workspace", xyz.device, B, M)
         d.compact_ws = ws.data_ptr()
+    if live is not None:
+        if not live.is_cuda or live.device != xyz.device or live.dtype != torch.int32 or tuple(live.shape) != (B,) or not live.is_contiguous():
+            raise RuntimeError("live must be a contiguous (B) int32 tensor on %s" % xyz.device)
+        d.live = live.data_ptr()
     _launch("ptt_sa_fused_fwd_f32", xyz.device, ctypes.byref(d), timed='ptt_sa_fused_fwd_f32')
     return out
 
```
